# lab4d-org/lab4d

Hardware: AMD Instinct MI355X
Metric: rendered rays/sec (fwd+bwd) at 512² × 128 samples; PSNR vs ref (higher is better)
Workload: dtype bf16

## Files before the change

### include/lab4d_mlp.h

```cpp
#ifndef LAB4D_MLP_H
#define LAB4D_MLP_H

#include <stdint.h>

#define LAB4D_MLP_MAX_LAYERS 12

#define LAB4D_NET_FG_BASE 0
#define LAB4D_NET_FG_COLOR 1
#define LAB4D_NET_VIS 2
#define LAB4D_NET_FEAT 3
#define LAB4D_NET_SKIN 4
#define LAB4D_NET_DENSE 5
#define LAB4D_NET_BG_BASE 6
#define LAB4D_NET_BG_COLOR 7
#define LAB4D_NET_SKIN18 8
#define LAB4D_NET_HASH_GEO 9
#define LAB4D_NET_HASH_COLOR 10
#define LAB4D_NET_DENSE6 11
#define LAB4D_NET_SKIN_A 12
#define LAB4D_NET_SKIN18_A 13
#define LAB4D_NET_COUNT 14

#define LAB4D_PREC_F32 0
#define LAB4D_PREC_BF16 1

typedef struct {
  int ke;
  int kin;
  int mout;
  int mout_pad;
  int relu;
  int pf_bias;
  int add_ext;
  int ext_grad;
} lab4d_mlp_layer;

typedef struct {
  int n_layers;
  int emb_kind;
  int n_freq;
  int c_in;
  int emb_slots;
  int ke;
  int c_out;
  lab4d_mlp_layer layers[LAB4D_MLP_MAX_LAYERS];
} lab4d_mlp_desc;

int lab4d_mlp_describe(int net, lab4d_mlp_desc* out);

int64_t lab4d_mlp_packed_bytes(int net, int layer, int precision);

int lab4d_mlp_pack(int net, int layer, int precision, int transposed, const float* W_ref, int k_ref,
                   const int32_t* col_map, void* packed, void* stream);

typedef struct {
  int net, precision;
  int S;
  int S_pad;
  int ld;
  int spf;
  const float* x;
  const float* freq_w;
  const void* W[LAB4D_MLP_MAX_LAYERS];
  const float* bias[LAB4D_MLP_MAX_LAYERS];
  const float* pf_bias[LAB4D_MLP_MAX_LAYERS];
  void* act[LAB4D_MLP_MAX_LAYERS];
  void* mask[LAB4D_MLP_MAX_LAYERS];
  void* emb;
  const void* ext;
  float* out;
  const float* x2;
  const int32_t* S_dev;
  const int32_t* frame_idx;
  const float* aff;
} lab4d_mlp_fwd_args;
int lab4d_mlp_forward(const lab4d_mlp_fwd_args* a, void* stream);

typedef struct {
  int net, precision, S, spf;
  const float* x;
  const float* freq_w;
  const float* aff;
  const void* W[LAB4D_MLP_MAX_LAYERS];
  const void* WT[LAB4D_MLP_MAX_LAYERS];
  const float* bias[LAB4D_MLP_MAX_LAYERS];
  const float* pf_bias[LAB4D_MLP_MAX_LAYERS];
  const float* d_out;
  float* d_x;
  float* g_aff;
  float* dW[LAB4D_MLP_MAX_LAYERS];
  float* db[LAB4D_MLP_MAX_LAYERS];
  float* pf_db[LAB4D_MLP_MAX_LAYERS];
} lab4d_mlp_bwd_fused_args;
int lab4d_mlp_backward_fused(const lab4d_mlp_bwd_fused_args* a, void* stream);
int lab4d_mlp_fused_backward_supported(int net, int precision, int spf);

int lab4d_mlp_forward_tangent(const lab4d_mlp_fwd_args* a, void* stream);

typedef struct {
  int net, precision, S, S_pad, ld, spf;
  const void* WT[LAB4D_MLP_MAX_LAYERS];
  const void* act[LAB4D_MLP_MAX_LAYERS];
  const void* mask[LAB4D_MLP_MAX_LAYERS];
  const void* emb;
  const void* ext;
  const float* d_out;
  const void* ext_gin;
  void* ext_gout;
  void* dz[LAB4D_MLP_MAX_LAYERS];
  float* d_x;
  float* d_x2;
  const float* x;
  const float* aff;
  float* g_aff;
} lab4d_mlp_bwd_args;
int lab4d_mlp_backward(const lab4d_mlp_bwd_args* a, void* stream);

int lab4d_mlp_wgrad(int net, int layer, int precision, int S, int S_pad, int ld, int spf, const void* dz, const void* emb,
                    const void* act_prev, float* dW, float* db, float* pf_db, int M, void* stream);
int lab4d_mlp_wgrad_mapped(int net, int layer, int precision, int S, int S_pad, int ld, int spf, const void* dz, const void* emb,
                           const void* act_prev, float* dW_ref, int ld_ref, const int32_t* col_map, float* db, float* pf_db, int M,
                           void* stream);

#endif
```

### lab4d_amd/csrc/hd_math.hpp

```cpp
#pragma once
#include <math.h>
#include <stdint.h>

#if defined(__HIPCC__)
#define LAB4D_HD __host__ __device__ inline
#else
#define LAB4D_HD inline
#endif

namespace lab4d_rn {

#if defined(__HIP_DEVICE_COMPILE__)
template <typename T>
__device__ __forceinline__ void pin(T& v) { asm volatile("" : "+v"(v)); }
__device__ __forceinline__ float add_rn(float a, float b) { float p = a + b; asm volatile("" : "+v"(p)); return p; }
__device__ __forceinline__ float mul_rn(float a, float b) { float p = a * b; asm volatile("" : "+v"(p)); return p; }
__device__ __forceinline__ float div_rn(float a, float b) { return __fdiv_rn(a, b); }
__device__ __forceinline__ double dadd(double a, double b) { double p = a + b; asm volatile("" : "+v"(p)); return p; }
__device__ __forceinline__ double dmul(double a, double b) { double p = a * b; asm volatile("" : "+v"(p)); return p; }
#else
template <typename T>
LAB4D_HD void pin(T&) {}
LAB4D_HD float add_rn(float a, float b) { volatile float p = a + b; return p; }
LAB4D_HD float mul_rn(float a, float b) { volatile float p = a * b; return p; }
LAB4D_HD float div_rn(float a, float b) { volatile float p = a / b; return p; }
LAB4D_HD double dadd(double a, double b) { volatile double p = a + b; return p; }
LAB4D_HD double dmul(double a, double b) { volatile double p = a * b; return p; }
#endif

LAB4D_HD float sqrt_rn(float a) { return (float)sqrt((double)a); }
LAB4D_HD bool finite_f(float v) { return fabsf(v) <= 3.402823466e+38f; }
LAB4D_HD float inf_f() { return __builtin_huge_valf(); }
LAB4D_HD float nan_f() { return __builtin_nanf(""); }

}
```

### lab4d_amd/csrc/mlp.hip

```cpp
#include <cstdlib>
#include "mlp_kernels.hpp"
#include "mlp_fused_bwd.hpp"

namespace lab4d {

struct DwMap {
  const int* cmap;
  int ld, mout, db_rows;
};
__device__ __forceinline__ int dw_col(int k, const DwMap& wm) { return wm.cmap ? wm.cmap[k] : k; }
__device__ __forceinline__ void dw_add(float* dW, int o, int c, int K, const DwMap& wm, float v) {
  if (wm.cmap) {
    if (c >= 0 && o < wm.mout) atomicAdd(dW + (size_t)o * wm.ld + c, v);
  } else {
    atomicAdd(dW + (size_t)o * K + c, v);
  }
}

template <class P, int TM>
__global__ void __launch_bounds__(256) k_mlp_wgrad(const typename P::store_t* __restrict__ dz, const typename P::store_t* __restrict__ emb,
                                                    const typename P::store_t* __restrict__ actp, int mo_tiles, int ke, int kin,
                                                    int S_pad, int chunk, int spf, int cpf, float* __restrict__ dW, float* __restrict__ db, DwMap wm) {
  constexpr int TN = 4;
  constexpr int SPS = P::BF16 ? 16 : 8;
// ... 395 lines not shown
        });
      }
      __builtin_amdgcn_s_barrier();
      asm volatile("" ::: "memory");
      if (s + NSTAGE - 1 < N) issue(s + NSTAGE - 1, buf == 0 ? NSTAGE - 1 : buf - 1);
      compute(buf);
      buf = buf + 1 == NSTAGE ? 0 : buf + 1;
    }
  }
#pragma unroll
  for (int i = 0; i < TM; ++i) {
#pragma unroll
    for (int j = 0; j < TN; ++j) {
      if (!bv_[j]) continue;
      const int c = dw_col(k0 + 32 * (wc * TN + j) + row, wm);
#pragma unroll
      for (int r = 0; r < 16; ++r) {
        const int o = 32 * (wr * TM + i) + drow(r, h);
        dw_add(dW, o, c, K, wm, acc[i][j][r]);
      }
    }
    if (do_db) {
      const float v = rs[i] + __shfl_xor(rs[i], 32, 64);
      if (h == 0 && 32 * (wr * TM + i) + row < wm.db_rows) atomicAdd(db + 32 * (wr * TM + i) + row, v);
    }
  }
}

template <class P>
__global__ void __launch_bounds__(256) k_rowsum_pf(const typename P::store_t* __restrict__ dz, int mo_pad, int S, int ld, int spf,
                                                    int M, int nseg, float* __restrict__ pf_db) {
  constexpr int SEG = 4096;
  const int lane = threadIdx.x & 63;
  const long job = (long)blockIdx.x * 4 + (threadIdx.x >> 6);
  if (job >= (long)mo_pad * nseg) return;
  const int o = (int)(job / nseg), seg = (int)(job % nseg);
  const long b = (long)seg * SEG, e = min((long)S, b + SEG);
  const typename P::store_t* row = dz + (size_t)o * 64;
  long i = b;
  while (i < e) {
    const int m = (int)(i / spf);
    const long fe = min(e, (long)(m + 1) * spf);
    float s = 0.f;
    for (long k = i + lane; k < fe; k += 64) {
      const size_t idx = (size_t)(k >> 6) * block_stride(mo_pad) + (k & 63);
      if constexpr (P::BF16) s += bf2f(row[idx]);
      else s += row[idx];
    }
    s = wave_sum(s);
    if (lane == 0) atomicAdd(pf_db + (size_t)m * mo_pad + o, s);
    i = fe;
  }
}

template <class P>
__global__ void __launch_bounds__(256) k_pack(const float* __restrict__ Wref, int mout, int k_ref, const int32_t* __restrict__ col_map,
                                               int ke, int kin, int mo_pad, int transposed, typename P::store_t* __restrict__ out) {
  constexpr int EPL = P::BF16 ? 8 : 4;
  const int K = ke + kin;
  const int rows = transposed ? K : mo_pad;
  const int kdim = transposed ? mo_pad : K;
  const int G = kdim / P::FPG;
  const long total = (long)(rows / 32) * G * 64 * EPL;
  for (long e = (long)blockIdx.x * blockDim.x + threadIdx.x; e < total; e += (long)gridDim.x * blockDim.x) {
    const int j = (int)(e % EPL);
    const int lane = (int)((e / EPL) % 64);
    const int g = (int)((e / (EPL * 64)) % G);
    const int mt = (int)(e / ((long)EPL * 64 * G));
    const int row = 32 * mt + (lane & 31), h = lane >> 5;
    const int ge = transposed ? 0 : ke / P::FPG;
    int kk;
    if (g < ge) {
      kk = P::BF16 ? 16 * g + 8 * h + j : 2 * (4 * g + j) + h;
    } else {
      const int gg = g - ge;
      int b, r;
      if (P::BF16) { b = gg >> 1; r = 8 * (gg & 1) + j; }
      else { const int kap = 4 * gg + j; b = kap >> 4; r = kap & 15; }
      kk = (transposed ? 0 : ke) + 32 * b + drow(r, h);
    }
    const int o = transposed ? kk : row;
    const int c = transposed ? row : kk;
    float v = 0.f;
    if (o < mout && c < K) {
      const int cr = col_map[c];
      if (cr >= 0) v = Wref[(size_t)o * k_ref + cr];
    }
    if constexpr (P::BF16) out[e] = f2bf(v);
    else out[e] = v;
  }
}

}
using namespace lab4d;

namespace {

template <class F>
int with_net(int net, F&& f) {
  switch (net) {
    case LAB4D_NET_FG_BASE: return f(NetFgBase{});
    case LAB4D_NET_FG_COLOR: return f(NetFgColor{});
    case LAB4D_NET_VIS: return f(NetVis{});
    case LAB4D_NET_FEAT: return f(NetFeat{});
    case LAB4D_NET_SKIN: return f(NetSkin{});
    case LAB4D_NET_SKIN18: return f(NetSkin18{});
    case LAB4D_NET_SKIN_A: return f(NetSkinA{});
    case LAB4D_NET_SKIN18_A: return f(NetSkin18A{});
    case LAB4D_NET_DENSE: return f(NetDense{});
    case LAB4D_NET_DENSE6: return f(NetDense6{});
    case LAB4D_NET_BG_BASE: return f(NetBgBase{});
    case LAB4D_NET_BG_COLOR: return f(NetBgColor{});
    case LAB4D_NET_HASH_GEO: return f(NetHashGeo{});
    case LAB4D_NET_HASH_COLOR: return f(NetHashColor{});
    default: set_error("unknown net id %d", net); return LAB4D_EINVAL;
  }
}

}

extern "C" int lab4d_mlp_describe(int net, lab4d_mlp_desc* out) {
  LAB4D_REQUIRE(out, "mlp_describe: null out");
  memset(out, 0, sizeof(*out));
  return with_net(net, [&](auto n) { fill_desc<decltype(n)>(out); return LAB4D_OK; });
}

extern "C" int64_t lab4d_mlp_packed_bytes(int net, int layer, int precision) {
  lab4d_mlp_desc d;
  if (lab4d_mlp_describe(net, &d) != LAB4D_OK || layer < 0 || layer >= d.n_layers) return -1;
  const lab4d_mlp_layer& L = d.layers[layer];
  return (int64_t)L.mout_pad * (L.ke + L.kin) * (precision == LAB4D_PREC_BF16 ? 2 : 4);
}

extern "C" int lab4d_mlp_pack(int net, int layer, int precision, int transposed, const float* W_ref, int k_ref,
                              const int32_t* col_map, void* packed, void* stream) {
  lab4d_mlp_desc d;
  if (int e = lab4d_mlp_describe(net, &d)) return e;
  LAB4D_REQUIRE(layer >= 0 && layer < d.n_layers, "mlp_pack: bad layer %d", layer);
  LAB4D_REQUIRE(W_ref && col_map && packed, "mlp_pack: null pointer");
  const lab4d_mlp_layer& L = d.layers[layer];
  const long total = (long)L.mout_pad * (L.ke + L.kin);
  int grid = div_up(total, 256); if (grid > 2048) grid = 2048;
  if (precision == LAB4D_PREC_BF16)
    hipLaunchKernelGGL((k_pack<PBF16>), dim3(grid), dim3(256), 0, (hipStream_t)stream, W_ref, L.mout, k_ref, col_map, L.ke, L.kin,
                       L.mout_pad, transposed, (unsigned short*)packed);
  else if (precision == LAB4D_PREC_F32)
    hipLaunchKernelGGL((k_pack<PF32>), dim3(grid), dim3(256), 0, (hipStream_t)stream, W_ref, L.mout, k_ref, col_map, L.ke, L.kin,
                       L.mout_pad, transposed, (float*)packed);
  else { set_error("mlp_pack: bad precision %d", precision); return LAB4D_EINVAL; }
  return check_launch("mlp_pack");
}

extern "C" int lab4d_mlp_forward(const lab4d_mlp_fwd_args* a, void* stream) {
  LAB4D_REQUIRE(a, "mlp_forward: null args");
  LAB4D_REQUIRE(a->S >= 0 && a->S_pad >= a->S && a->S_pad % 256 == 0 && a->spf > 0 && a->ld >= a->S_pad && a->ld % 8 == 0,
                "mlp_forward: bad sizes (S_pad must be a multiple of 256) S=%d S_pad=%d ld=%d spf=%d", a->S, a->S_pad, a->ld, a->spf);
  LAB4D_REQUIRE(a->x && a->out, "mlp_forward: null x/out");
  if (a->S == 0) return LAB4D_OK;
  return with_net(a->net, [&](auto n) {
    using Net = decltype(n);
    FwdK k;
    memset(&k, 0, sizeof(k));
    k.S = a->S; k.S_pad = a->S_pad; k.ld = a->ld; k.spf = a->spf; k.x = a->x; k.freq_w = a->freq_w; k.emb = a->emb; k.ext = a->ext; k.out = a->out; k.x2 = a->x2;
    k.S_dev = a->S_dev; k.frame_idx = a->frame_idx; k.aff = a->aff;
    LAB4D_REQUIRE(!a->aff || Net::EMB != 0, "mlp_forward: aff is for the raw-input nets only");
    LAB4D_REQUIRE(Net::EMB != 2 || a->aff, "mlp_forward: this network needs the per-frame affine table aff (M, ke, 4)");
    LAB4D_REQUIRE(!Net::AUX3 || a->x2, "mlp_forward: this network needs the second input x2");
    LAB4D_REQUIRE(!(a->S_dev && a->emb), "mlp_forward: a device-side sample count is for the evaluation path (no stored activations)");
    for (int l = 0; l < Net::NL; ++l) {
      LAB4D_REQUIRE(a->W[l] && a->bias[l], "mlp_forward: layer %d weights/bias missing", l);
      LAB4D_REQUIRE(!Net::L[l].pf || a->pf_bias[l], "mlp_forward: layer %d needs a per-frame bias", l);
      LAB4D_REQUIRE(!Net::L[l].add_ext || a->ext, "mlp_forward: layer %d needs ext", l);
      if (a->emb && l + 1 < Net::NL) {
        LAB4D_REQUIRE(a->act[l] || (dx_only_ok<Net>() && !a->act[0]), "mlp_forward: training mode (emb != NULL) needs act[%d]", l);
        LAB4D_REQUIRE(!Net::L[l].relu || a->mask[l], "mlp_forward: training mode (emb != NULL) needs mask[%d]", l);
      }
      k.W[l] = a->W[l]; k.bias[l] = a->bias[l]; k.pf_bias[l] = a->pf_bias[l]; k.act[l] = a->act[l]; k.mask[l] = (unsigned int*)a->mask[l];
    }
    return launch_mlp_fwd<Net>(a->precision, k, a->S, (hipStream_t)stream);
  });
}

extern "C" int lab4d_mlp_backward(const lab4d_mlp_bwd_args* a, void* stream) {
  LAB4D_REQUIRE(a, "mlp_backward: null args");
  LAB4D_REQUIRE(a->S >= 0 && a->S_pad >= a->S && a->S_pad % 256 == 0 && a->spf > 0 && a->ld >= a->S_pad && a->ld % 8 == 0, "mlp_backward: bad sizes (S_pad must be a multiple of 256)");
  LAB4D_REQUIRE(a->d_out, "mlp_backward: null d_out");
  if (a->S == 0) return LAB4D_OK;
  return with_net(a->net, [&](auto n) {
    using Net = decltype(n);
    BwdK k;
    memset(&k, 0, sizeof(k));
    k.S = a->S; k.S_pad = a->S_pad; k.ld = a->ld; k.spf = a->spf; k.emb = a->emb; k.ext = a->ext; k.d_out = a->d_out; k.ext_gin = a->ext_gin;
    k.ext_gout = a->ext_gout; k.d_x = a->d_x; k.d_x2 = a->d_x2; k.x = a->x; k.aff = a->aff; k.g_aff = a->g_aff;
    if (Net::EMB == 2) {
      LAB4D_REQUIRE(a->x && a->aff && a->emb, "mlp_backward: this network needs x, aff and the stored embedding");
    } else {
      LAB4D_REQUIRE(!a->g_aff, "mlp_backward: g_aff is for the affine-first-layer nets only");
    }
    LAB4D_REQUIRE(!(a->d_x && Net::EMB == 0) || a->emb, "mlp_backward: d_x needs the stored embedding");
    for (int l = 0; l < Net::NL; ++l) {
      LAB4D_REQUIRE(a->WT[l], "mlp_backward: layer %d transposed weights missing", l);
      LAB4D_REQUIRE(!(Net::L[l].relu && l + 1 < Net::NL) || a->mask[l], "mlp_backward: layer %d ReLU mask missing", l);
      LAB4D_REQUIRE(!Net::L[l].ext_grad || a->ext_gin, "mlp_backward: layer %d needs ext_gin", l);
      LAB4D_REQUIRE(a->dz[l] || (dx_only_ok<Net>() && !a->dz[0] && a->d_x), "mlp_backward: dz[%d] missing (every layer's dZ is written, or none: point gradient only)", l);
      LAB4D_REQUIRE(!Net::L[l].add_ext || a->ext_gout, "mlp_backward: layer %d needs ext_gout", l);
      k.WT[l] = a->WT[l]; k.act[l] = a->act[l]; k.mask[l] = (const unsigned int*)a->mask[l]; k.dz[l] = a->dz[l];
    }
    return launch_mlp_bwd<Net>(a->precision, k, a->S, (hipStream_t)stream);
  });
}

extern "C" int lab4d_mlp_fused_backward_supported(int net, int precision, int spf) {
  if (precision != LAB4D_PREC_BF16 || spf <= 0 || spf % 64 != 0) return 0;
  static const int vis_env = getenv("LAB4D_FUSED_VIS") ? atoi(getenv("LAB4D_FUSED_VIS")) : 0;
  return net == LAB4D_NET_SKIN_A || net == LAB4D_NET_SKIN18_A || (net == LAB4D_NET_VIS && vis_env != 0);
}

extern "C" int lab4d_mlp_backward_fused(const lab4d_mlp_bwd_fused_args* a, void* stream) {
  LAB4D_REQUIRE(a, "mlp_backward_fused: null args");
  LAB4D_REQUIRE(lab4d_mlp_fused_backward_supported(a->net, a->precision, a->spf), "mlp_backward_fused: net %d / precision %d / spf %d not supported (bf16, narrow nets, spf %% 64 == 0)",
                a->net, a->precision, a->spf);
  LAB4D_REQUIRE(a->S >= 0 && a->x && a->d_out, "mlp_backward_fused: null x / d_out");
  if (a->S == 0) return LAB4D_OK;
  auto run = [&](auto n) {
    using Net = decltype(n);
    FusedK k;
    memset(&k, 0, sizeof(k));
    k.S = a->S; k.spf = a->spf; k.ntiles = (a->S + 63) / 64; k.x = a->x; k.freq_w = a->freq_w; k.aff = a->aff; k.d_out = a->d_out; k.d_x = a->d_x; k.g_aff = a->g_aff;
    LAB4D_REQUIRE(Net::EMB != 2 || a->aff, "mlp_backward_fused: this network needs the per-frame affine table aff");
    for (int l = 0; l < Net::NL; ++l) {
      LAB4D_REQUIRE(a->WT[l] && a->dW[l], "mlp_backward_fused: layer %d transposed weights / dW missing", l);
      LAB4D_REQUIRE(l + 1 == Net::NL || (a->W[l] && (Net::L[l].pf ? (const void*)a->pf_bias[l] : (const void*)a->bias[l])), "mlp_backward_fused: layer %d forward weights / bias missing", l);
      LAB4D_REQUIRE((((uintptr_t)a->W[l] | (uintptr_t)a->WT[l]) & 15) == 0, "mlp_backward_fused: packed weights must be 16-byte aligned");
      k.W[l] = a->W[l]; k.WT[l] = a->WT[l]; k.bias[l] = a->bias[l]; k.pf_bias[l] = a->pf_bias[l]; k.dW[l] = a->dW[l]; k.db[l] = a->db[l]; k.pf_db[l] = a->pf_db[l];
    }
    return launch_mlp_bwd_fused<Net>(k, (hipStream_t)stream);
  };
  switch (a->net) {
    case LAB4D_NET_VIS: return run(NetVis{});
    case LAB4D_NET_SKIN_A: return run(NetSkinA{});
    default: return run(NetSkin18A{});
  }
}

extern "C" int lab4d_mlp_wgrad(int net, int layer, int precision, int S, int S_pad, int ld, int spf, const void* dz, const void* emb,
                               const void* act_prev, float* dW, float* db, float* pf_db, int M, void* stream) {
  return lab4d_mlp_wgrad_mapped(net, layer, precision, S, S_pad, ld, spf, dz, emb, act_prev, dW, 0, nullptr, db, pf_db, M, stream);
}

extern "C" int lab4d_mlp_wgrad_mapped(int net, int layer, int precision, int S, int S_pad, int ld, int spf, const void* dz, const void* emb,
                                      const void* act_prev, float* dW, int ld_ref, const int32_t* col_map, float* db, float* pf_db, int M,
                                      void* stream) {
  lab4d_mlp_desc d;
  if (int e = lab4d_mlp_describe(net, &d)) return e;
  LAB4D_REQUIRE(layer >= 0 && layer < d.n_layers, "mlp_wgrad: bad layer %d", layer);
  const lab4d_mlp_layer& L = d.layers[layer];
  LAB4D_REQUIRE(dz && dW, "mlp_wgrad: null dz/dW");
  LAB4D_REQUIRE(col_map == nullptr || ld_ref > 0, "mlp_wgrad_mapped: a column map needs the reference row stride");
  LAB4D_REQUIRE(L.ke == 0 || emb, "mlp_wgrad: layer %d needs the stored embedding", layer);
  LAB4D_REQUIRE(L.kin == 0 || act_prev, "mlp_wgrad: layer %d needs the previous activation", layer);
  LAB4D_REQUIRE(S_pad % 64 == 0 && S_pad >= S && ld >= S_pad && ld % 8 == 0, "mlp_wgrad: bad S_pad/ld");
  if (S == 0) return LAB4D_OK;
  const int mo_tiles = L.mout_pad / 32, nk_tiles = (L.ke + L.kin) / 32;
  const bool big = mo_tiles >= 8;
  const int Kt = L.ke + L.kin;
  static const int head_dma = getenv("LAB4D_WGRAD_HEAD_DMA") ? atoi(getenv("LAB4D_WGRAD_HEAD_DMA")) : 1;
  const bool dma = precision == LAB4D_PREC_BF16 && (mo_tiles == 8 || mo_tiles == 4 || mo_tiles == 2 || (mo_tiles == 1 && head_dma && Kt <= 256));
  const int nbw = (dma && mo_tiles == 1) ? (Kt <= 128 ? 2 : 4)
                  : Kt <= 64 ? 1 : (Kt <= 128 ? 2 : (Kt <= 192 ? 3 : (Kt <= 256 ? 4 : (mo_tiles == 8 && Kt <= 320 ? 5 : 3))));
  const int TM = mo_tiles >= 4 ? 4 : (mo_tiles >= 2 ? 2 : 1);
  const int ob_n = dma ? 1 : (big ? div_up(mo_tiles, 8) : div_up(mo_tiles, TM));
  const int kb_n = dma ? div_up(Kt, 64 * nbw) : (big ? div_up(nk_tiles, 8) : div_up(nk_tiles, 4));
  static const int jobs_env = getenv("LAB4D_WGRAD_JOBS") ? atoi(getenv("LAB4D_WGRAD_JOBS")) : 0;
  const int jobs_target = jobs_env > 0 ? jobs_env : ((dma && mo_tiles < 8) ? 512 : 256);
  int nchunks = jobs_target / (ob_n * kb_n); if (nchunks < 1) nchunks = 1;
  int chunk = div_up(div_up(S_pad, nchunks), 256) * 256; if (chunk < 1024) chunk = 1024;
  const bool fold_pf = pf_db != nullptr && spf % 256 == 0 && M > 0 && (long)M * spf >= S;
  LAB4D_REQUIRE(pf_db == nullptr || fold_pf || (M > 0 && spf > 0 && (long)M * spf >= S), "mlp_wgrad: pf_db needs M and spf, with M * spf >= S");
  int cpf = 0;
  if (fold_pf) {
    if (chunk > spf) chunk = spf;
    cpf = div_up(spf, chunk);
    nchunks = cpf * M;
  } else {
    nchunks = div_up(S_pad, chunk);
  }
  const int jobs = ob_n * kb_n * nchunks;
  const dim3 grid(jobs), block(256), block8(512);
  float* db_arg = fold_pf ? pf_db : db;
  const DwMap wm = {col_map, ld_ref, L.mout, (col_map && !fold_pf) ? L.mout : L.mout_pad};
  hipStream_t st = (hipStream_t)stream;
#define WG(P, TMV) hipLaunchKernelGGL((k_mlp_wgrad<P, TMV>), grid, block, 0, st, (const typename P::store_t*)dz, (const typename P::store_t*)emb, \
                                      (const typename P::store_t*)act_prev, mo_tiles, L.ke, L.kin, S_pad, chunk, spf, cpf, dW, db_arg, wm)
#define WGB(P) hipLaunchKernelGGL((k_mlp_wgrad_big<P>), grid, block, 0, st, (const typename P::store_t*)dz, (const typename P::store_t*)emb, \
                                  (const typename P::store_t*)act_prev, mo_tiles, L.ke, L.kin, S_pad, chunk, spf, cpf, dW, db_arg, wm)
#define WGD(MTV, NBV) hipLaunchKernelGGL((k_mlp_wgrad_dma<MTV, NBV>), grid, block, 0, st, (const unsigned short*)dz, (const unsigned short*)emb, \
                                         (const unsigned short*)act_prev, L.ke, L.kin, S_pad, chunk, spf, cpf, dW, db_arg, wm)
#define WGD8(NBV) hipLaunchKernelGGL((k_mlp_wgrad_dma<8, NBV, 8>), grid, block8, 0, st, (const unsigned short*)dz, (const unsigned short*)emb, \
                                     (const unsigned short*)act_prev, L.ke, L.kin, S_pad, chunk, spf, cpf, dW, db_arg, wm)
#define WGD_NB(MTV) do { if (nbw == 1) WGD(MTV, 1); else if (nbw == 2) WGD(MTV, 2); else if (nbw == 3) WGD(MTV, 3); else WGD(MTV, 4); } while (0)
  if (dma) {
    if (mo_tiles == 8) {
      if (nbw == 1) WGD8(1); else if (nbw == 2) WGD8(2); else if (nbw == 3) WGD8(3); else if (nbw == 4) WGD8(4); else WGD8(5);
    } else if (mo_tiles == 4) WGD_NB(4); else if (mo_tiles == 2) WGD_NB(2);
    else if (nbw == 2) hipLaunchKernelGGL((k_mlp_wgrad_dma<1, 2, 4, 4>), grid, block, 0, st, (const unsigned short*)dz, (const unsigned short*)emb,
                                          (const unsigned short*)act_prev, L.ke, L.kin, S_pad, chunk, spf, cpf, dW, db_arg, wm);
    else hipLaunchKernelGGL((k_mlp_wgrad_dma<1, 4, 4, 4>), grid, block, 0, st, (const unsigned short*)dz, (const unsigned short*)emb,
                            (const unsigned short*)act_prev, L.ke, L.kin, S_pad, chunk, spf, cpf, dW, db_arg, wm);
  }
#undef WGD_NB
#undef WGD8
#undef WGD
  else if (precision == LAB4D_PREC_BF16) { if (big) WGB(PBF16); else if (TM == 4) WG(PBF16, 4); else if (TM == 2) WG(PBF16, 2); else WG(PBF16, 1); }
  else if (precision == LAB4D_PREC_F32) { if (big) WGB(PF32); else if (TM == 4) WG(PF32, 4); else if (TM == 2) WG(PF32, 2); else WG(PF32, 1); }
  else { set_error("mlp_wgrad: bad precision %d", precision); return LAB4D_EINVAL; }
#undef WGB
#undef WG
  if (int e = check_launch("mlp_wgrad")) return e;
  if (pf_db && !fold_pf) {
    const int nseg = div_up(S, 4096);
    const long jobs2 = (long)L.mout_pad * nseg;
    if (precision == LAB4D_PREC_BF16)
      hipLaunchKernelGGL((k_rowsum_pf<PBF16>), dim3(div_up(jobs2, 4)), dim3(256), 0, st, (const unsigned short*)dz, L.mout_pad, S, ld, spf, M, nseg, pf_db);
    else
      hipLaunchKernelGGL((k_rowsum_pf<PF32>), dim3(div_up(jobs2, 4)), dim3(256), 0, st, (const float*)dz, L.mout_pad, S, ld, spf, M, nseg, pf_db);
    return check_launch("mlp_rowsum_pf");
  }
  return LAB4D_OK;
}

namespace {
template <class Net>
int forward_tangent_impl(const lab4d_mlp_fwd_args* a, void* stream) {
  FwdK k;
  memset(&k, 0, sizeof(k));
  k.S = a->S; k.S_pad = a->S_pad; k.ld = a->ld; k.spf = a->spf; k.x = a->x; k.emb = a->emb; k.out = a->out;
  for (int l = 0; l < Net::NL; ++l) {
    LAB4D_REQUIRE(a->W[l], "mlp_forward_tangent: layer %d weights missing", l);
    LAB4D_REQUIRE(!(Net::L[l].relu) || a->mask[l], "mlp_forward_tangent: layer %d primal ReLU mask missing", l);
    LAB4D_REQUIRE(l + 1 == Net::NL || a->act[l], "mlp_forward_tangent: act[%d] missing", l);
    k.W[l] = a->W[l]; k.bias[l] = a->bias[l] ? a->bias[l] : (const float*)a->W[l]; k.act[l] = a->act[l]; k.mask[l] = (unsigned int*)a->mask[l];
  }
  return launch_mlp_fwd_tangent<Net>(a->precision, k, a->S, (hipStream_t)stream);
}
}

// ... 11 lines not shown
```

### lab4d_amd/csrc/mlp_kernels.hpp

```cpp
#pragma once
#include <cstddef>
#include <cstdlib>
#include <type_traits>

#include "common.hpp"
#include "mlp_nets.hpp"

namespace lab4d {

typedef __attribute__((ext_vector_type(8))) short bf16x8_t;
typedef __attribute__((ext_vector_type(16))) float f32x16_t;

struct PBF16 {
  static constexpr bool BF16 = true;
  static constexpr int NT = 2, TILE = 64, FPG = 16, UPT = 2;
  using store_t = unsigned short;
};
struct PF32 {
  static constexpr bool BF16 = false;
  static constexpr int NT = 1, TILE = 32, FPG = 8, UPT = 4;
  using store_t = float;
};

__device__ __forceinline__ unsigned short f2bf(float x) {
// ... 169 lines not shown
               "v_cndmask_b32_dpp %[t02], %[d21], %[d20], vcc" LAB4D_QP1 "v_cndmask_b32_dpp %[t22], %[d23], %[d22], vcc" LAB4D_QP1
               "v_cndmask_b32_dpp %[t03], %[d31], %[d30], vcc" LAB4D_QP1 "v_cndmask_b32_dpp %[t23], %[d33], %[d32], vcc quad_perm:[1,0,3,2] row_mask:0xf bank_mask:0xf"
               : [t00] "=&v"(t0[0]), [t01] "=&v"(t0[1]), [t02] "=&v"(t0[2]), [t03] "=&v"(t0[3]), [t20] "=&v"(t2[0]), [t21] "=&v"(t2[1]),
                 [t22] "=&v"(t2[2]), [t23] "=&v"(t2[3])
               : [m] "s"(mE), [d00] "v"(d[0][0]), [d01] "v"(d[0][1]), [d02] "v"(d[0][2]), [d03] "v"(d[0][3]), [d10] "v"(d[1][0]), [d11] "v"(d[1][1]),
                 [d12] "v"(d[1][2]), [d13] "v"(d[1][3]), [d20] "v"(d[2][0]), [d21] "v"(d[2][1]), [d22] "v"(d[2][2]), [d23] "v"(d[2][3]),
                 [d30] "v"(d[3][0]), [d31] "v"(d[3][1]), [d32] "v"(d[3][2]), [d33] "v"(d[3][3])
               : "vcc");
  asm volatile("s_mov_b64 vcc, %[m]\n\t"
               "v_cndmask_b32_dpp %[d01], %[d00], %[d01], vcc" LAB4D_QP1 "v_cndmask_b32_dpp %[d03], %[d02], %[d03], vcc" LAB4D_QP1
               "v_cndmask_b32_dpp %[d11], %[d10], %[d11], vcc" LAB4D_QP1 "v_cndmask_b32_dpp %[d13], %[d12], %[d13], vcc" LAB4D_QP1
               "v_cndmask_b32_dpp %[d21], %[d20], %[d21], vcc" LAB4D_QP1 "v_cndmask_b32_dpp %[d23], %[d22], %[d23], vcc" LAB4D_QP1
               "v_cndmask_b32_dpp %[d31], %[d30], %[d31], vcc" LAB4D_QP1 "v_cndmask_b32_dpp %[d33], %[d32], %[d33], vcc quad_perm:[1,0,3,2] row_mask:0xf bank_mask:0xf"
               : [d01] "+v"(d[0][1]), [d03] "+v"(d[0][3]), [d11] "+v"(d[1][1]), [d13] "+v"(d[1][3]), [d21] "+v"(d[2][1]), [d23] "+v"(d[2][3]),
                 [d31] "+v"(d[3][1]), [d33] "+v"(d[3][3])
               : [m] "s"(mO), [d00] "v"(d[0][0]), [d02] "v"(d[0][2]), [d10] "v"(d[1][0]), [d12] "v"(d[1][2]), [d20] "v"(d[2][0]), [d22] "v"(d[2][2]),
                 [d30] "v"(d[3][0]), [d32] "v"(d[3][2])
               : "vcc");
  unsigned int c0[4], c1[4];
  asm volatile("s_mov_b64 vcc, %[m]\n\t"
               "v_cndmask_b32_dpp %[c00], %[t20], %[t00], vcc" LAB4D_QP2 "v_cndmask_b32_dpp %[c10], %[d03], %[d01], vcc" LAB4D_QP2
               "v_cndmask_b32_dpp %[c01], %[t21], %[t01], vcc" LAB4D_QP2 "v_cndmask_b32_dpp %[c11], %[d13], %[d11], vcc" LAB4D_QP2
               "v_cndmask_b32_dpp %[c02], %[t22], %[t02], vcc" LAB4D_QP2 "v_cndmask_b32_dpp %[c12], %[d23], %[d21], vcc" LAB4D_QP2
               "v_cndmask_b32_dpp %[c03], %[t23], %[t03], vcc" LAB4D_QP2 "v_cndmask_b32_dpp %[c13], %[d33], %[d31], vcc quad_perm:[2,3,0,1] row_mask:0xf bank_mask:0xf"
               : [c00] "=&v"(c0[0]), [c01] "=&v"(c0[1]), [c02] "=&v"(c0[2]), [c03] "=&v"(c0[3]), [c10] "=&v"(c1[0]), [c11] "=&v"(c1[1]),
                 [c12] "=&v"(c1[2]), [c13] "=&v"(c1[3])
               : [m] "s"(mL), [t00] "v"(t0[0]), [t01] "v"(t0[1]), [t02] "v"(t0[2]), [t03] "v"(t0[3]), [t20] "v"(t2[0]), [t21] "v"(t2[1]), [t22] "v"(t2[2]),
                 [t23] "v"(t2[3]), [d01] "v"(d[0][1]), [d03] "v"(d[0][3]), [d11] "v"(d[1][1]), [d13] "v"(d[1][3]), [d21] "v"(d[2][1]), [d23] "v"(d[2][3]),
                 [d31] "v"(d[3][1]), [d33] "v"(d[3][3])
               : "vcc");
  asm volatile("s_mov_b64 vcc, %[m]\n\t"
               "v_cndmask_b32_dpp %[t20], %[t00], %[t20], vcc" LAB4D_QP2 "v_cndmask_b32_dpp %[d03], %[d01], %[d03], vcc" LAB4D_QP2
               "v_cndmask_b32_dpp %[t21], %[t01], %[t21], vcc" LAB4D_QP2 "v_cndmask_b32_dpp %[d13], %[d11], %[d13], vcc" LAB4D_QP2
               "v_cndmask_b32_dpp %[t22], %[t02], %[t22], vcc" LAB4D_QP2 "v_cndmask_b32_dpp %[d23], %[d21], %[d23], vcc" LAB4D_QP2
               "v_cndmask_b32_dpp %[t23], %[t03], %[t23], vcc" LAB4D_QP2 "v_cndmask_b32_dpp %[d33], %[d31], %[d33], vcc quad_perm:[2,3,0,1] row_mask:0xf bank_mask:0xf"
               : [t20] "+v"(t2[0]), [t21] "+v"(t2[1]), [t22] "+v"(t2[2]), [t23] "+v"(t2[3]), [d03] "+v"(d[0][3]), [d13] "+v"(d[1][3]), [d23] "+v"(d[2][3]),
                 [d33] "+v"(d[3][3])
               : [m] "s"(mH), [t00] "v"(t0[0]), [t01] "v"(t0[1]), [t02] "v"(t0[2]), [t03] "v"(t0[3]), [d01] "v"(d[0][1]), [d11] "v"(d[1][1]), [d21] "v"(d[2][1]),
                 [d31] "v"(d[3][1])
               : "vcc");
#undef LAB4D_QP1
#undef LAB4D_QP2
#pragma unroll
  for (int i = 0; i < 4; ++i) {
    out[i][0] = c0[i];
    out[i][1] = c1[i];
    out[i][2] = t2[i];
    out[i][3] = d[i][3];
  }
}

__device__ __forceinline__ void store_tile_packed(GLOBAL_AS void* buf, int F, int s0, int mt, int lane, const unsigned int (&w)[2][8]) {
  const int n = lane & 31, h = lane >> 5, q = n & 3, k = n >> 2;
  GLOBAL_AS char* base = (GLOBAL_AS char*)buf + tile_base_offset<PBF16>(F, s0, 32 * mt);
  const unsigned lo = tile_lane_offset<PBF16>(4 * h + q, k);
  unsigned int d[4][4], c[4][4];
#pragma unroll
  for (int i = 0; i < 4; ++i)
#pragma unroll
    for (int j = 0; j < 4; ++j) {
      const int r = 4 * i + j;
      d[i][j] = __builtin_amdgcn_perm(w[1][r >> 1], w[0][r >> 1], (r & 1) ? 0x07060302u : 0x05040100u);
    }
  quad_transpose4(d, c);
#pragma unroll
  for (int i = 0; i < 4; ++i) gst16(base + (lo + tile_lane_offset<PBF16>(8 * i, 0)), c[i][0], c[i][1], c[i][2], c[i][3]);
}


struct TrTile {
  unsigned long long a[4], b[4];
};
__device__ __forceinline__ void tr_wait(TrTile& r) {
  asm volatile("s_waitcnt lgkmcnt(0)"
               : "+v"(r.a[0]), "+v"(r.a[1]), "+v"(r.a[2]), "+v"(r.a[3]), "+v"(r.b[0]), "+v"(r.b[1]), "+v"(r.b[2]), "+v"(r.b[3]));
}
__device__ __forceinline__ void tr_store(GLOBAL_AS void* buf, int F, int s0, int mt, int lane, const TrTile& r) {
  const int i = lane & 15, G = lane >> 4, h = G & 1, S = G >> 1;
  GLOBAL_AS char* base = (GLOBAL_AS char*)buf + tile_base_offset<PBF16>(F, s0, 32 * mt);
  const unsigned lo = (unsigned)((4 * h + (i & 3)) * 128 + (32 * S + 8 * (i >> 2)) * 2);
#pragma unroll
  for (int qa = 0; qa < 4; ++qa) {
    const unsigned long long A = r.a[qa], B = r.b[qa];
    gst16(base + (lo + (unsigned)((16 * (qa >> 1) + 8 * (qa & 1)) * 128)), (unsigned)A, (unsigned)(A >> 32), (unsigned)B, (unsigned)(B >> 32));
  }
}

template <class P>
__device__ __forceinline__ void store_tile(GLOBAL_AS void* buf, int F, int s0, int mt, int lane, const f32x16_t* c ) {
  const int n = lane & 31, h = lane >> 5, q = n & 3, k = n >> 2;
  GLOBAL_AS char* base = (GLOBAL_AS char*)buf + tile_base_offset<P>(F, s0, 32 * mt);
  const unsigned lo = tile_lane_offset<P>(4 * h + q, k);
#pragma unroll
  for (int i = 0; i < 4; ++i) {
    unsigned int d[4];
#pragma unroll
    for (int j = 0; j < 4; ++j) {
      if constexpr (P::BF16) d[j] = pack2bf(c[0][4 * i + j], c[1][4 * i + j]);
      else d[j] = __float_as_uint(c[0][4 * i + j]);
    }
    quad_transpose(d, q);
    gst16(base + (lo + tile_lane_offset<P>(8 * i, 0)), d[0], d[1], d[2], d[3]);
  }
}
template <class P>
__device__ __forceinline__ void load_tile_raw(const GLOBAL_AS void* buf, int F, int s0, int mt, int lane, uint4 (&raw)[4]) {
  const int n = lane & 31, h = lane >> 5, q = n & 3, k = n >> 2;
  const GLOBAL_AS char* base = (const GLOBAL_AS char*)buf + tile_base_offset<P>(F, s0, 32 * mt);
  const unsigned lo = tile_lane_offset<P>(4 * h + q, k);
#pragma unroll
  for (int i = 0; i < 4; ++i) raw[i] = gld16(base + (lo + tile_lane_offset<P>(8 * i, 0)));
}
template <class P>
__device__ __forceinline__ void tile_from_raw(const uint4 (&raw)[4], int lane, f32x16_t* c ) {
  const int q = lane & 3;
#pragma unroll
  for (int i = 0; i < 4; ++i) {
    unsigned int d[4] = {raw[i].x, raw[i].y, raw[i].z, raw[i].w};
    quad_transpose(d, q);
#pragma unroll
    for (int j = 0; j < 4; ++j) {
      if constexpr (P::BF16) {
        c[0][4 * i + j] = bf2f((unsigned short)(d[j] & 0xffffu));
        c[1][4 * i + j] = bf2f((unsigned short)(d[j] >> 16));
      } else {
        c[0][4 * i + j] = __uint_as_float(d[j]);
      }
    }
  }
}
template <class P>
__device__ __forceinline__ void load_tile(const GLOBAL_AS void* buf, int F, int s0, int mt, int lane, f32x16_t* c ) {
  uint4 raw[4];
  load_tile_raw<P>(buf, F, s0, mt, lane, raw);
  tile_from_raw<P>(raw, lane, c);
}

struct FwdK {
  int S, S_pad, ld, spf, ntiles;
  const float* x;
  const float* freq_w;
  const void* W[LAB4D_MLP_MAX_LAYERS];
  const float* bias[LAB4D_MLP_MAX_LAYERS];
  const float* pf_bias[LAB4D_MLP_MAX_LAYERS];
  void* act[LAB4D_MLP_MAX_LAYERS];
  unsigned int* mask[LAB4D_MLP_MAX_LAYERS];
  void* emb;
  const void* ext;
  float* out;
  const float* x2;
  const int* S_dev;
  const int* frame_idx;
  const float* aff;
};
struct BwdK {
  int S, S_pad, ld, spf, ntiles;
  const void* WT[LAB4D_MLP_MAX_LAYERS];
  const void* act[LAB4D_MLP_MAX_LAYERS];
  const unsigned int* mask[LAB4D_MLP_MAX_LAYERS];
  const void* emb;
  const void* ext;
  const float* d_out;
  const void* ext_gin;
  void* ext_gout;
  void* dz[LAB4D_MLP_MAX_LAYERS];
  float* d_x;
  float* d_x2;
  const float* x;
  const float* aff;
  float* g_aff;
};

template <class Net>
__device__ __forceinline__ void emb_pair(int pair, const float* x , const float* freq_w, float& v0, float& v1) {
  constexpr int L = Net::NFREQ;
  if (pair < 3 * L) {
    const int f = pair / 3, a = pair - 3 * f;
    const float xa = a == 0 ? x[0] : (a == 1 ? x[1] : x[2]);
    const float ang = ldexpf(xa, f);
    float s, c;
    sincosf(ang, &s, &c);
    const float w = freq_w ? freq_w[f] : 1.0f;
    v0 = s * w;
    v1 = c * w;
  } else {
    const int s0 = 2 * pair - 6 * L;
    constexpr int NR = Net::AUX3 ? 6 : 3;
    v0 = s0 < NR ? x[s0 < NR ? s0 : 0] : 0.f;
    v1 = s0 + 1 < NR ? x[s0 + 1 < NR ? s0 + 1 : 0] : 0.f;
  }
}

constexpr int ACACHE_G = 14;
template <class Net, class P, bool BWD = false>
constexpr int want_occ() {
  return (P::BF16 && (Net::ID == LAB4D_NET_FEAT || Net::ID == LAB4D_NET_VIS)) ? 2 : 1;
}
template <class Net, class P>
constexpr int acache_g() {
  return want_occ<Net, P>() == 2 ? 7 : ACACHE_G;
}
__device__ __forceinline__ void wg_step_barrier() {
  asm volatile("s_waitcnt lgkmcnt(0)\n\ts_barrier" ::: "memory");
}

template <class Net>
constexpr bool fwd_same(int a, int b) {
  const LS x = Net::L[a], y = Net::L[b];
  return x.ke == y.ke && x.kin == y.kin && x.mout == y.mout && x.relu == y.relu && x.pf == y.pf && x.add_ext == y.add_ext &&
         ((a == Net::NL - 1) == (b == Net::NL - 1));
}
template <class Net>
constexpr int fwd_rep(int l) {
  for (int j = 0; j < l; ++j)
    if (fwd_same<Net>(j, l)) return j;
  return l;
}
template <class Net>
constexpr unsigned fwd_members(int r) {
  unsigned m = 0;
  for (int l = 0; l < Net::NL; ++l)
    if (fwd_rep<Net>(l) == r) m |= 1u << l;
  return m;
}
template <class Net>
constexpr bool fwd_any_export(int r) {
  for (int l = 0; l < Net::NL; ++l)
    if (fwd_rep<Net>(l) == r && Net::L[l].ext_grad) return true;
  return false;
}
template <class Net>
constexpr bool bwd_same(int a, int b) {
  if ((a == 0) != (b == 0)) return false;
  const LS x = Net::L[a], y = Net::L[b];
  if (!(x.ke == y.ke && x.kin == y.kin && x.mout == y.mout)) return false;
  if (a == 0) return true;
  const LS xp = Net::L[a - 1], yp = Net::L[b - 1];
  return xp.relu == yp.relu && xp.ext_grad == yp.ext_grad && xp.add_ext == yp.add_ext && xp.mout == yp.mout;
}
template <class Net>
constexpr int bwd_rep(int l) {
  for (int j = Net::NL - 1; j > l; --j)
    if (bwd_same<Net>(j, l)) return j;
  return l;
}
template <class Net>
constexpr unsigned bwd_members(int r) {
  unsigned m = 0;
  for (int l = 0; l < Net::NL; ++l)
    if (bwd_rep<Net>(l) == r) m |= 1u << l;
  return m;
}

template <class Net>
constexpr bool head_staged() { return Net::COUT > 16; }

template <class Net, class P>
struct Slab {
  static constexpr int W = net_wmax<Net>();
  static constexpr int UW = W / P::FPG;
  static constexpr int STAGE_C = Net::EMB == 1 ? Net::CIN : Net::KE;
  static constexpr bool STAGES = Net::EMB == 1 || Net::ID == LAB4D_NET_FG_BASE || Net::ID == LAB4D_NET_BG_BASE;
  static constexpr int UNITS_STAGE = STAGES ? (P::TILE * STAGE_C * 4 + 15) / 16 : 0;
  static constexpr int UNITS_LAYER = P::NT * UW * 64;
  static constexpr int UNITS_PER_WAVE = UNITS_LAYER > UNITS_STAGE ? UNITS_LAYER : UNITS_STAGE;
};

template <int COUNT>
__device__ __forceinline__ void stage_in(float* __restrict__ stage, const float* __restrict__ x, long e0, long e_last, int lane) {
  const GLOBAL_AS float* gx = (const GLOBAL_AS float*)x;
  if (e0 + COUNT - 1 <= e_last && (((size_t)(x + e0)) & 15) == 0 && (COUNT & 3) == 0) {
    constexpr int N4 = COUNT / 4, TRIPS = (N4 + 63) / 64;
    f32x4_t v[TRIPS];
#pragma unroll
    for (int i = 0; i < TRIPS; ++i) {
      const int e = lane + 64 * i;
      if (e < N4) v[i] = *(const GLOBAL_AS f32x4_t*)(gx + e0 + 4 * e);
    }
#pragma unroll
    for (int i = 0; i < TRIPS; ++i) {
      const int e = lane + 64 * i;
      if (e < N4) reinterpret_cast<float4*>(stage)[e] = make_float4(v[i].x, v[i].y, v[i].z, v[i].w);
    }
  } else {
    for (int e = lane; e < COUNT; e += 64) {
      const long ge = e0 + e;
      stage[e] = gx[ge <= e_last ? ge : e_last];
    }
  }
}
__device__ __forceinline__ void stage_out(const float* __restrict__ stage, float* __restrict__ y, long e0, int count, long e_last, int lane) {
  GLOBAL_AS float* gy = (GLOBAL_AS float*)y;
  if (e0 + count - 1 <= e_last && (((size_t)(y + e0)) & 15) == 0 && (count & 3) == 0) {
    for (int e = lane; e < count / 4; e += 64) {
      const float4 v = reinterpret_cast<const float4*>(stage)[e];
      f32x4_t o = {v.x, v.y, v.z, v.w};
      *(GLOBAL_AS f32x4_t*)(gy + e0 + 4 * e) = o;
    }
  } else {
    for (int e = lane; e < count; e += 64) {
      const long ge = e0 + e;
      if (ge <= e_last) gy[ge] = stage[e];
    }
  }
}

template <class Net, class P, bool TAN = false, bool ST = false, bool ACTS = true>
__global__ void __launch_bounds__(256, (want_occ<Net, P>())) k_mlp_fwd(FwdK a) {
  constexpr int NT = P::NT, TILE = P::TILE, KE = Net::KE, UE = KE / P::FPG, UW = Slab<Net, P>::UW;
  constexpr int ACG = acache_g<Net, P>();
  __shared__ uint4 slab_all[4 * Slab<Net, P>::UNITS_PER_WAVE];
  __shared__ uint4 abuf[2 * ACG * 64];
  __shared__ float4 afftab[(Net::EMB != 0 && !TAN) ? 4 * 96 : 1];
  const int lane = threadIdx.x & 63, n = lane & 31, h = lane >> 5;
  const int wid = __builtin_amdgcn_readfirstlane((int)(threadIdx.x >> 6));
  uint4* slab = slab_all + wid * Slab<Net, P>::UNITS_PER_WAVE + lane;
  const int wave = blockIdx.x * 4 + wid, nwaves = gridDim.x * 4;

  int S_eff = a.S, ntiles = a.ntiles;
  if (a.S_dev) {
    const int sd = *(const GLOBAL_AS int*)a.S_dev;
    S_eff = sd < a.S ? sd : a.S;
    const int nt = ((S_eff + TILE - 1) / TILE + 3) & ~3;
    ntiles = nt < a.ntiles ? nt : a.ntiles;
  }
  for (int tile = wave; tile < ntiles; tile += nwaves) {
    const int s0 = tile * TILE;
    int sidx[NT], frame[NT];
#pragma unroll
    for (int t = 0; t < NT; ++t) {
      const int s = s0 + NT * n + t;
      sidx[t] = s;
      const int sc = s < S_eff ? s : S_eff - 1;
      frame[t] = a.frame_idx ? ((const GLOBAL_AS int*)a.frame_idx)[sc] : sc / a.spf;
    }
    uint4 emb[NT][UE];
    constexpr bool RAW = (Net::EMB == 1) || TAN;
    constexpr int CINR = TAN ? KE : Net::CIN;
    float* stagef = reinterpret_cast<float*>(slab_all + wid * Slab<Net, P>::UNITS_PER_WAVE);
    if constexpr (RAW) {
      bool staged = false;
      if constexpr (Net::EMB == 1 && !TAN) {
        if (a.aff != nullptr) {
          static_assert(Net::CIN <= 96, "affine table");
          constexpr int HALF = (Net::CIN + 1) / 2;
          const GLOBAL_AS float4* tabg = (const GLOBAL_AS float4*)a.aff;
          float4* ltab = afftab + wid * 96;
          const bool uni = (a.spf % TILE) == 0 && a.frame_idx == nullptr;
          if (uni) {
            const int m = __builtin_amdgcn_readfirstlane(frame[0]);
            for (int e = lane; e < Net::CIN; e += 64) {
              const f32x4_t r = *(const GLOBAL_AS f32x4_t*)(tabg + (size_t)m * Net::CIN + e);
              ltab[e] = make_float4(r.x, r.y, r.z, r.w);
            }
          }
          __builtin_amdgcn_wave_barrier();
#pragma unroll
          for (int t = 0; t < NT; ++t) {
            const int s = sidx[t] < S_eff ? sidx[t] : S_eff - 1;
            const float x0 = a.x[(size_t)s * 3], x1 = a.x[(size_t)s * 3 + 1], x2_ = a.x[(size_t)s * 3 + 2];
            float* row = stagef + (NT * n + t) * Net::CIN;
            for (int i = 0; i < HALF; ++i) {
              const int c = i + h * HALF;
              if (c < Net::CIN) {
                float4 r;
                if (uni) r = ltab[c];
                else {
                  const f32x4_t g = *(const GLOBAL_AS f32x4_t*)(tabg + (size_t)frame[t] * Net::CIN + c);
                  r = make_float4(g.x, g.y, g.z, g.w);
                }
                row[c] = r.x * x0 + r.y * x1 + r.z * x2_ + r.w;
              }
            }
          }
          __builtin_amdgcn_wave_barrier();
          staged = true;
        }
      }
      if (!staged) stage_in<TILE * CINR>(stagef, a.x, (long)s0 * CINR, (long)S_eff * CINR - 1, lane);
    }
    if constexpr (Net::EMB == 2 && !TAN) {
      static_assert(KE <= 96, "affine table");
      const GLOBAL_AS float4* tabg = (const GLOBAL_AS float4*)a.aff;
      float4* ltab = afftab + wid * 96;
      const bool uni = (a.spf % TILE) == 0 && a.frame_idx == nullptr;
      if (uni) {
        const int m = __builtin_amdgcn_readfirstlane(frame[0]);
        for (int e = lane; e < KE; e += 64) {
          const f32x4_t r = *(const GLOBAL_AS f32x4_t*)(tabg + (size_t)m * KE + e);
          ltab[e] = make_float4(r.x, r.y, r.z, r.w);
        }
      }
      __builtin_amdgcn_wave_barrier();
#pragma unroll
      for (int t = 0; t < NT; ++t) {
        const int s = sidx[t] < S_eff ? sidx[t] : S_eff - 1;
        const float x0 = a.x[(size_t)s * 3], x1 = a.x[(size_t)s * 3 + 1], x2_ = a.x[(size_t)s * 3 + 2];
        auto slot_val = [&](int slot) {
          float4 r;
          if (uni) r = ltab[slot];
          else {
            const f32x4_t g4 = *(const GLOBAL_AS f32x4_t*)(tabg + (size_t)frame[t] * KE + slot);
            r = make_float4(g4.x, g4.y, g4.z, g4.w);
          }
          return relu1(r.x * x0 + r.y * x1 + r.z * x2_ + r.w);
        };
#pragma unroll
        for (int g = 0; g < UE; ++g) {
// ... 128 lines not shown
      if constexpr (fwd_rep<Net>(R) != R) return;
      constexpr unsigned MEMBERS = fwd_members<Net>(R);
      if (!((MEMBERS >> l) & 1u)) return;
      constexpr LS ls = Net::L[R];
      constexpr bool LAST = (R == Net::NL - 1);
      constexpr int MT = pad32(ls.mout) / 32;
      constexpr int GE = ls.ke / P::FPG, GA = ls.kin / P::FPG, G = GE + GA;
      constexpr int GL = G < ACG ? G : ACG, NQ = (GL + 3) / 4;
      const GLOBAL_AS void* Wl = KARG_PTR(FwdK, const void*, W, l);
      const GLOBAL_AS float* bl = KARG_PTR(FwdK, const float*, bias, l);
      const GLOBAL_AS float* pfl = KARG_PTR(FwdK, const float*, pf_bias, l);
      GLOBAL_AS unsigned int* maskl = KARG_PTR(FwdK, unsigned int*, mask, l);
      GLOBAL_AS void* actl = KARG_PTR(FwdK, void*, act, l);
      uint4 bin[NT][GA > 0 ? GA : 1];
#pragma unroll
      for (int t = 0; t < NT; ++t)
#pragma unroll
        for (int u = 0; u < GA; ++u) bin[t][u] = slab[(t * UW + u) * 64];
      constexpr int NB = (ls.pf != 0 && !TAN) ? NT : 1;
      auto load_bias = [&](int mt, f32x16_t (&bv)[NB]) {
        if constexpr (TAN) {
#pragma unroll
          for (int r = 0; r < 16; ++r) bv[0][r] = 0.f;
        } else {
#pragma unroll
          for (int t = 0; t < NB; ++t)
#pragma unroll
            for (int i = 0; i < 4; ++i) {
              const GLOBAL_AS float* src = (ls.pf != 0) ? pfl + (size_t)frame[t] * (32 * MT) : bl;
              const f32x4_t v = *(const GLOBAL_AS f32x4_t*)(src + 32 * mt + 8 * i + 4 * h);
              bv[t][4 * i + 0] = v.x; bv[t][4 * i + 1] = v.y; bv[t][4 * i + 2] = v.z; bv[t][4 * i + 3] = v.w;
            }
        }
      };
      auto mfma_tile = [&](auto has_pre, int pre, int rbuf, uint4 (&A)[G], f32x16_t (&bv)[NB], f32x16_t (&acc)[NT]) {
        constexpr bool PRE = decltype(has_pre)::value;
#pragma unroll
        for (int t = 0; t < NT; ++t) acc[t] = bv[NB == 1 ? 0 : t];
#pragma unroll
        for (int g = 0; g < G; ++g) {
#pragma unroll
          for (int t = 0; t < NT; ++t) mma_unit<P>(acc[t], A[g], g < GE ? emb[t][g < GE ? g : 0] : bin[t][g >= GE ? g - GE : 0]);
          if constexpr (PRE) {
            if (g >= GL) A[g] = load_a(Wl, G, pre, g, lane);
            else if (rbuf >= 0) A[g] = abuf[(rbuf * ACG + g) * 64 + lane];
          }
        }
        if constexpr (PRE) load_bias(pre, bv);
      };
      auto a_fetch = [&](int mt, uint4 (&stg)[NQ]) {
#pragma unroll
        for (int i = 0; i < NQ; ++i) {
          const int g = wid + 4 * i < GL ? wid + 4 * i : GL - 1;
          stg[i] = load_a(Wl, G, mt, g, lane);
        }
      };
      auto a_stash = [&](int buf, const uint4 (&stg)[NQ]) {
#pragma unroll
        for (int i = 0; i < NQ; ++i) {
          const int g = wid + 4 * i < GL ? wid + 4 * i : GL - 1;
          abuf[(buf * ACG + g) * 64 + lane] = stg[i];
        }
      };
      auto a_grab = [&](int buf, uint4 (&A)[G]) {
#pragma unroll
        for (int g = 0; g < GL; ++g) A[g] = abuf[(buf * ACG + g) * 64 + lane];
      };
      unsigned int tan_bits = 0;
      uint4 ext_raw[4];
      auto prefetch = [&](int mt) {
        if constexpr (TAN && ls.relu != 0) tan_bits = maskl[((size_t)tile * MT + mt) * 64 + lane];
        if constexpr (ls.add_ext != 0 && !TAN) load_tile_raw<P>((const GLOBAL_AS void*)a.ext, 32 * MT, s0, mt, lane, ext_raw);
      };
      constexpr bool PACKED = P::BF16 && !TAN && ls.add_ext == 0 && !LAST;
      auto epilogue = [&](int mt, f32x16_t (&acc)[NT], unsigned int (&w)[2][8], unsigned int& wbits) {
        if constexpr (PACKED) {
#pragma unroll
          for (int t = 0; t < NT; ++t) acc_fence_if<(want_occ<Net, P>() == 2)>(acc[t]);
#pragma unroll
          for (int t = 0; t < 2; ++t)
#pragma unroll
            for (int k = 0; k < 8; ++k) w[t][k] = pack2bf_op(acc[t][2 * k], acc[t][2 * k + 1]);
          if constexpr (ls.relu != 0) {
            if constexpr (ST) wbits = pk_alive_bits(w);
#pragma unroll
            for (int t = 0; t < 2; ++t)
#pragma unroll
              for (int k = 0; k < 8; ++k) w[t][k] = pk_relu_bf16(w[t][k]);
          }
#pragma unroll
          for (int t = 0; t < 2; ++t)
#pragma unroll
            for (int q = 0; q < 2; ++q) slab[(t * UW + 2 * mt + q) * 64] = make_uint4(w[t][4 * q], w[t][4 * q + 1], w[t][4 * q + 2], w[t][4 * q + 3]);
          return;
        }
        if constexpr (ls.relu != 0) {
          if constexpr (TAN) {
            const unsigned int bits = tan_bits;
#pragma unroll
            for (int t = 0; t < NT; ++t)
#pragma unroll
              for (int r = 0; r < 16; ++r)
                acc[t][r] = __uint_as_float(__float_as_uint(acc[t][r]) & (unsigned int)__builtin_amdgcn_sbfe((int)bits, mask_bit<P>(t, r), 1));
          } else {
            if constexpr (ST && !LAST) {
              unsigned int bits = 0;
#pragma unroll
              for (int t = 0; t < NT; ++t)
#pragma unroll
                for (int r = 0; r < 16; ++r) bits |= (acc[t][r] > 0.f ? 1u : 0u) << mask_bit<P>(t, r);
              maskl[((size_t)tile * MT + mt) * 64 + lane] = bits;
            }
#pragma unroll
            for (int t = 0; t < NT; ++t)
#pragma unroll
              for (int r = 0; r < 16; ++r) acc[t][r] = relu1(acc[t][r]);
          }
        }
        if constexpr (ls.add_ext != 0 && !TAN) {
          f32x16_t e[NT];
          tile_from_raw<P>(ext_raw, lane, e);
#pragma unroll
          for (int t = 0; t < NT; ++t)
#pragma unroll
            for (int r = 0; r < 16; ++r) acc[t][r] += e[t][r];
        }
        if constexpr (ST) {
          if constexpr (!LAST && ACTS) store_tile<P>(actl, 32 * MT, s0, mt, lane, acc);
        } else if constexpr (fwd_any_export<Net>(R)) {
          if (actl) store_tile<P>(actl, 32 * MT, s0, mt, lane, acc);
        }
        if constexpr (!LAST) {
#pragma unroll
          for (int t = 0; t < NT; ++t) {
            uint4 u[P::UPT];
            tile_to_units<P>(acc[t], u);
#pragma unroll
            for (int q = 0; q < P::UPT; ++q) slab[(t * UW + P::UPT * mt + q) * 64] = u[q];
          }
        } else if constexpr (head_staged<Net>() && !TAN) {
          static_assert(pad32(Net::COUT) == 32, "one row tile");
          __builtin_amdgcn_wave_barrier();
#pragma unroll
          for (int t = 0; t < NT; ++t)
#pragma unroll
            for (int r = 0; r < 16; ++r) {
              const int f = drow(r, h);
              if (f < Net::COUT) stagef[(NT * n + t) * Net::COUT + f] = acc[t][r];
            }
          __builtin_amdgcn_wave_barrier();
          if (a.out) stage_out(stagef, a.out, (long)s0 * Net::COUT, TILE * Net::COUT, (long)S_eff * Net::COUT - 1, lane);
          __builtin_amdgcn_wave_barrier();
        } else {
#pragma unroll
          for (int t = 0; t < NT; ++t)
#pragma unroll
            for (int r = 0; r < 16; ++r) {
              const int f = 32 * mt + drow(r, h);
              if (f < Net::COUT && sidx[t] < S_eff && a.out) a.out[(size_t)sidx[t] * Net::COUT + f] = acc[t][r];
            }
        }
      };
      auto flush = [&](int mt, const unsigned int (&w)[2][8], unsigned int wbits) {
        if constexpr (PACKED) {
          if constexpr (ST) {
            if constexpr (ls.relu != 0) maskl[((size_t)tile * MT + mt) * 64 + lane] = wbits;
            if constexpr (ACTS) store_tile_packed(actl, 32 * MT, s0, mt, lane, w);
          } else if constexpr (fwd_any_export<Net>(R)) {
            if (actl) store_tile_packed(actl, 32 * MT, s0, mt, lane, w);
          }
        }
      };
      uint4 A[G], stg[NQ];
      f32x16_t bv[NB];
      f32x16_t acc0[NT], acc1[NT];
      unsigned int pw[2][8], pbits = 0;
      wg_step_barrier();
      a_fetch(0, stg);
      a_stash(0, stg);
      if constexpr (MT > 1) {
        a_fetch(1, stg);
        a_stash(1, stg);
      }
      a_fetch(MT > 2 ? 2 : MT - 1, stg);
#pragma unroll
      for (int g = GL; g < G; ++g) A[g] = load_a(Wl, G, 0, g, lane);
      load_bias(0, bv);
      prefetch(0);
      wg_step_barrier();
      a_grab(0, A);
      constexpr int NSTEP = MT - 1, NPAIR = NSTEP / 2;
      mfma_tile(std::bool_constant<(MT > 1)>{}, 1, -1, A, bv, acc0);
      if constexpr (NPAIR > 0) {
#pragma nounroll
        for (int k = 0; k < 2 * NPAIR; k += 2) {
          wg_step_barrier();
          a_grab(1, A);
          mfma_tile(std::true_type{}, k + 2 < MT ? k + 2 : MT - 1, -1, A, bv, acc1);
          epilogue(k, acc0, pw, pbits);
          prefetch(k + 1);
          a_stash(0, stg);
          a_fetch(k + 3 < MT ? k + 3 : MT - 1, stg);
          flush(k, pw, pbits);
          wg_step_barrier();
          a_grab(0, A);
          mfma_tile(std::true_type{}, k + 3 < MT ? k + 3 : MT - 1, -1, A, bv, acc0);
          epilogue(k + 1, acc1, pw, pbits);
          prefetch(k + 2 < MT ? k + 2 : MT - 1);
          a_stash(1, stg);
          a_fetch(k + 4 < MT ? k + 4 : MT - 1, stg);
          flush(k + 1, pw, pbits);
        }
      }
      if constexpr (NSTEP % 2 == 1) {
        wg_step_barrier();
        a_grab(1, A);
        mfma_tile(std::false_type{}, 0, -1, A, bv, acc1);
        epilogue(MT - 2, acc0, pw, pbits);
        flush(MT - 2, pw, pbits);
        prefetch(MT - 1);
        epilogue(MT - 1, acc1, pw, pbits);
        flush(MT - 1, pw, pbits);
      } else {
        epilogue(MT - 1, acc0, pw, pbits);
        flush(MT - 1, pw, pbits);
      }
    });
  }
}

template <class Net>
constexpr int emb_layer_count() {
  int c = 0;
  for (int l = 0; l < Net::NL; ++l) c += Net::L[l].ke ? 1 : 0;
  return c;
}

template <class Net, class P, bool AU = true, bool DZ = true>
__global__ void __launch_bounds__(256, (want_occ<Net, P, true>())) k_mlp_bwd(BwdK a) {
  static_assert(Net::EMB == 0 || emb_layer_count<Net>() == 1, "raw-input nets may use the input in one layer only");
  constexpr int NT = P::NT, TILE = P::TILE, NL = Net::NL, UW = Slab<Net, P>::UW;
  constexpr int ACG = acache_g<Net, P>();
  __shared__ uint4 slab_all[4 * Slab<Net, P>::UNITS_PER_WAVE];
  __shared__ uint4 abuf0[ACG * 64];
  __shared__ uint4 abuf1[ACG * 64];
#define LAB4D_ABUF(buf) ((buf) ? abuf1 : abuf0)
  __shared__ float4 afftab[Net::EMB == 2 ? 4 * 96 : 1];
  constexpr int NGA = (Net::EMB == 2 && AU) ? (Net::KE / 32) * 16 * 4 : 1;
  float gacc[NGA];
#pragma unroll
  for (int i = 0; i < NGA; ++i) gacc[i] = 0.f;
  int gframe = -1;
  auto gram_flush = [&]() {
    if constexpr (Net::EMB == 2 && AU) {
      if (gframe >= 0 && a.g_aff != nullptr) {
#pragma unroll
        for (int i = 0; i < NGA; ++i) {
          float v = gacc[i];
#pragma unroll
          for (int off = 1; off < 32; off <<= 1) v += __shfl_xor(v, off, 64);
          const int mt = i / 64, r = (i >> 2) & 15, j = i & 3;
          if ((threadIdx.x & 31) == 0) atomicAdd(a.g_aff + ((size_t)gframe * Net::KE + 32 * mt + drow(r, (int)((threadIdx.x & 63) >> 5))) * 4 + j, v);
          gacc[i] = 0.f;
        }
      }
    }
  };
  const int lane = threadIdx.x & 63, n = lane & 31, h = lane >> 5;
  const int wid = __builtin_amdgcn_readfirstlane((int)(threadIdx.x >> 6));
  uint4* slab = slab_all + wid * Slab<Net, P>::UNITS_PER_WAVE + lane;
  float* stagef = reinterpret_cast<float*>(slab_all + wid * Slab<Net, P>::UNITS_PER_WAVE);
  const int wave = blockIdx.x * 4 + wid, nwaves = gridDim.x * 4;

  for (int tile = wave; tile < a.ntiles; tile += nwaves) {
    const int s0 = tile * TILE;
    int sidx[NT];
#pragma unroll
    for (int t = 0; t < NT; ++t) sidx[t] = s0 + NT * n + t;
    float dx[NT][3];
    float dx2[NT][3];
#pragma unroll
    for (int t = 0; t < NT; ++t) { dx[t][0] = dx[t][1] = dx[t][2] = 0.f; dx2[t][0] = dx2[t][1] = dx2[t][2] = 0.f; }
    float xs[NT][3];
    int frm[NT];
    float4* ltab = afftab + wid * 96;
    constexpr bool uni = AU;
    if constexpr (Net::EMB == 2) {
#pragma unroll
      for (int t = 0; t < NT; ++t) {
        const int sc = sidx[t] < a.S ? sidx[t] : a.S - 1;
        frm[t] = sc / a.spf;
#pragma unroll
        for (int k = 0; k < 3; ++k) xs[t][k] = ((const GLOBAL_AS float*)a.x)[(size_t)sc * 3 + k];
      }
      if constexpr (uni) {
        const int m = __builtin_amdgcn_readfirstlane(frm[0]);
        if (m != gframe) {
          gram_flush();
          gframe = m;
        }
        for (int e = lane; e < Net::KE; e += 64) {
          const f32x4_t r4 = *(const GLOBAL_AS f32x4_t*)((const GLOBAL_AS float4*)a.aff + (size_t)m * Net::KE + e);
          ltab[e] = make_float4(r4.x, r4.y, r4.z, r4.w);
        }
      }
      __builtin_amdgcn_wave_barrier();
    }

    {
      f32x16_t g[NT];
      if constexpr (head_staged<Net>()) {
        __builtin_amdgcn_wave_barrier();
        stage_in<TILE * Net::COUT>(stagef, a.d_out, (long)s0 * Net::COUT, (long)a.S * Net::COUT - 1, lane);
        __builtin_amdgcn_wave_barrier();
#pragma unroll
        for (int t = 0; t < NT; ++t)
#pragma unroll
          for (int r = 0; r < 16; ++r) {
            const int f = drow(r, h);
            g[t][r] = (f < Net::COUT && sidx[t] < a.S) ? stagef[(NT * n + t) * Net::COUT + (f < Net::COUT ? f : 0)] : 0.f;
          }
        __builtin_amdgcn_wave_barrier();
      } else {
#pragma unroll
      for (int t = 0; t < NT; ++t)
#pragma unroll
        for (int r = 0; r < 16; ++r) {
          const int f = drow(r, h);
          g[t][r] = (f < Net::COUT && sidx[t] < a.S) ? a.d_out[(size_t)sidx[t] * Net::COUT + f] : 0.f;
        }
      }
      if constexpr (DZ) store_tile<P>((GLOBAL_AS void*)a.dz[NL - 1], pad32(Net::L[NL - 1].mout), s0, 0, lane, g);
#pragma unroll
      for (int t = 0; t < NT; ++t) {
        uint4 u[P::UPT];
        tile_to_units<P>(g[t], u);
#pragma unroll
        for (int q = 0; q < P::UPT; ++q) slab[(t * UW + q) * 64] = u[q];
      }
    }

#pragma nounroll
    for (int l = NL - 1; l >= 0; --l)
    sfor<0, NL>([&](auto ri) {
      constexpr int R = NL - 1 - decltype(ri)::value;
      if constexpr (bwd_rep<Net>(R) != R) return;
      constexpr unsigned MEMBERS = bwd_members<Net>(R);
      if (!((MEMBERS >> l) & 1u)) return;
      constexpr LS ls = Net::L[R];
      constexpr LS lp = Net::L[R > 0 ? R - 1 : 0];
      constexpr int GK = pad32(ls.mout) / P::FPG;
      constexpr int GL = GK < ACG ? GK : ACG, NQ = (GL + 3) / 4;
      constexpr int MTE = ls.ke / 32, MTA = ls.kin / 32;
      constexpr bool DO_ACT = (R > 0 && MTA > 0);
      const int lm1 = l > 0 ? l - 1 : 0;
      const GLOBAL_AS void* Wt = KARG_PTR(BwdK, const void*, WT, l);
      const GLOBAL_AS unsigned int* maskp = KARG_PTR(BwdK, const unsigned int*, mask, lm1);
      GLOBAL_AS void* dzp = KARG_PTR(BwdK, void*, dz, lm1);
      uint4 bin[NT][GK];
#pragma unroll
      for (int t = 0; t < NT; ++t)
#pragma unroll
        for (int u = 0; u < GK; ++u) bin[t][u] = slab[(t * UW + u) * 64];

      auto mfma_tile = [&](auto has_pre, int pre, int rbuf, uint4 (&A)[GK], f32x16_t (&acc)[NT]) {
        constexpr bool PRE = decltype(has_pre)::value;
#pragma unroll
        for (int t = 0; t < NT; ++t)
#pragma unroll
          for (int r = 0; r < 16; ++r) acc[t][r] = 0.f;
        sfor<0, GK>([&](auto gc) {
          constexpr int g = decltype(gc)::value;
#pragma unroll
          for (int t = 0; t < NT; ++t) mma_unit<P>(acc[t], A[g], bin[t][g]);
          if constexpr (PRE) {
            if (g >= GL) A[g] = load_a(Wt, GK, pre, g, lane);
            else if (rbuf >= 0) A[g] = LAB4D_ABUF(rbuf)[g * 64 + lane];
          }
        });
      };
      auto a_fetch = [&](int mt, uint4 (&stg)[NQ]) {
#pragma unroll
        for (int i = 0; i < NQ; ++i) {
          const int g = wid + 4 * i < GL ? wid + 4 * i : GL - 1;
          stg[i] = load_a(Wt, GK, mt, g, lane);
        }
      };
      auto a_stash = [&](int buf, const uint4 (&stg)[NQ]) {
#pragma unroll
        for (int i = 0; i < NQ; ++i) {
          const int g = wid + 4 * i < GL ? wid + 4 * i : GL - 1;
          LAB4D_ABUF(buf)[g * 64 + lane] = stg[i];
        }
      };
      auto a_grab = [&](int buf, uint4 (&A)[GK]) {
#pragma unroll
        for (int g = 0; g < GL; ++g) A[g] = LAB4D_ABUF(buf)[g * 64 + lane];
      };
      auto pipeline = [&](auto n_c, int tile0, auto&& pre, auto&& epi, auto&& fl, auto&& prem) {
        constexpr int N = decltype(n_c)::value;
        if constexpr (N > 0) {
          uint4 A[GK], stg[NQ];
          f32x16_t acc0[NT], acc1[NT];
          unsigned int pw[2][8];
          wg_step_barrier();
          a_fetch(tile0, stg);
          a_stash(0, stg);
          if constexpr (N > 1) {
            a_fetch(tile0 + 1, stg);
            a_stash(1, stg);
          }
          a_fetch(tile0 + (N > 2 ? 2 : N - 1), stg);
#pragma unroll
          for (int g = GL; g < GK; ++g) A[g] = load_a(Wt, GK, tile0, g, lane);
          pre(0);
          prem(std::integral_constant<int, 0>{}, 0);
          prem(std::integral_constant<int, 1>{}, N > 1 ? 1 : 0);
          wg_step_barrier();
          a_grab(0, A);
          constexpr int NSTEP = N - 1, NPAIR = NSTEP / 2;
          mfma_tile(std::bool_constant<(N > 1)>{}, tile0 + 1, 1, A, acc0);
          if constexpr (N > 1) {
            wg_step_barrier();
            a_stash(0, stg);
            a_fetch(tile0 + (N > 3 ? 3 : N - 1), stg);
          }
          if constexpr (NPAIR > 0) {
#pragma nounroll
            for (int k = 0; k < 2 * NPAIR; k += 2) {
              wg_step_barrier();
              mfma_tile(std::true_type{}, tile0 + (k + 2 < N ? k + 2 : N - 1), 0, A, acc1);
              epi(k, acc0, pw);
              pre(k + 1);
              prem(std::integral_constant<int, 0>{}, k + 2 < N ? k + 2 : N - 1);
              a_stash(1, stg);
              a_fetch(tile0 + (k + 4 < N ? k + 4 : N - 1), stg);
              fl(k, pw);
              wg_step_barrier();
              mfma_tile(std::true_type{}, tile0 + (k + 3 < N ? k + 3 : N - 1), 1, A, acc0);
              epi(k + 1, acc1, pw);
              pre(k + 2 < N ? k + 2 : N - 1);
              prem(std::integral_constant<int, 1>{}, k + 3 < N ? k + 3 : N - 1);
              a_stash(0, stg);
              a_fetch(tile0 + (k + 5 < N ? k + 5 : N - 1), stg);
              fl(k + 1, pw);
            }
          }
          if constexpr (NSTEP % 2 == 1) {
            wg_step_barrier();
            mfma_tile(std::false_type{}, 0, -1, A, acc1);
            epi(N - 2, acc0, pw);
            fl(N - 2, pw);
            pre(N - 1);
            epi(N - 1, acc1, pw);
            fl(N - 1, pw);
          } else {
            epi(N - 1, acc0, pw);
            fl(N - 1, pw);
          }
        }
      };
      uint4 raw[4];
      unsigned int mb0 = 0, mb1 = 0;
      auto no_prem = [&](auto, int) {};
      auto pre_mask = [&](auto par_c, int j) {
        if constexpr (lp.relu != 0) {
          const unsigned int v = maskp[((size_t)tile * (pad32(lp.mout) / 32) + j) * 64 + lane];
          if constexpr (decltype(par_c)::value == 0) mb0 = v; else mb1 = v;
        }
      };
      auto pre_emb = [&](int mt) {
        if constexpr (Net::EMB != 1) load_tile_raw<P>((const GLOBAL_AS void*)a.emb, Net::KE, s0, mt, lane, raw);
      };
      auto pre_act = [&](int j) {
        if constexpr (lp.ext_grad != 0) load_tile_raw<P>((const GLOBAL_AS void*)a.ext_gin, pad32(lp.mout), s0, j, lane, raw);
      };
      auto no_flush = [&](int, const unsigned int (&)[2][8]) {};
      auto epi_emb = [&](int mt, f32x16_t (&acc)[NT], unsigned int (&)[2][8]) {
        if constexpr (Net::EMB == 0) {
          f32x16_t e[NT];
          tile_from_raw<P>(raw, lane, e);
          constexpr int L = Net::NFREQ;
#pragma unroll
// ... 297 lines not shown
```

### lab4d_amd/csrc/mlp_kernels_ws.hpp

```cpp
#pragma once
#include "mlp_kernels.hpp"

namespace lab4d {

template <class Net>
constexpr bool ws_ok() {
  if (!(Net::EMB == 0 && Net::AUX3 == 0 && net_wmax<Net>() == 256 && Net::KE % 32 == 0)) return false;
  for (int l = 0; l < Net::NL; ++l) {
    const int mt = pad32(Net::L[l].mout) / 32;
    if (!(mt == 1 || mt == 2 || mt == 4 || mt == 8)) return false;
    if (Net::L[l].kin % 32 != 0 || Net::L[l].kin > 256) return false;
    if (Net::L[l].ke != 0 && Net::L[l].ke != Net::KE) return false;
  }
  return true;
}
template <class Net>
constexpr int ws_g(int l) { return (Net::L[l].ke + Net::L[l].kin) / 16; }
template <class Net>
constexpr int ws_mt(int l) { return pad32(Net::L[l].mout) / 32; }
template <class Net>
constexpr int ws_gmax() {
  int g = 0;
  for (int l = 0; l < Net::NL; ++l) g = ws_g<Net>(l) > g ? ws_g<Net>(l) : g;
  return g;
// ... 396 lines not shown
      GLOBAL_AS void* actp = act_c;
      GLOBAL_AS unsigned int* maskp = mask_c;
      const GLOBAL_AS void* Wn_n = KARG_PTR(FwdK, const void*, W, (ln + 1 < NL ? ln + 1 : 0));
      GLOBAL_AS void* act_n = KARG_PTR(FwdK, void*, act, l);
      GLOBAL_AS unsigned int* mask_n = KARG_PTR(FwdK, unsigned int*, mask, l);
      const int mtp = ITp::mt(w);
      if constexpr (R > 0 && !SPREAD) {
        auto flush_prev = [&]() {
#pragma unroll
          for (int k = 0; k < ITp::IPW; ++k) {
            const int b = ITp::blk(w, k);
            if constexpr (ACTS) {
              {
                const unsigned tb_ = xbuf_lds + (unsigned)(ib * WS_BUF * 16 + b * 2 * 16 * 1024 + mtp * 2048);
                ws_tr_issue(tb_ + trl, tb_ + trl2, trt);
              }
              tr_wait(trt);
              tr_store(actp, 32 * MTp, s0 + 64 * b, mtp, lane, trt);
            }
            if constexpr (ST && !TAN && Net::L[R > 0 ? R - 1 : 0].relu != 0) maskp[((size_t)(2 * tile + b) * MTp + mtp) * 64 + lane] = pbits[k];
          }
        };
        if constexpr (ST) {
          if (ITp::active(w)) flush_prev();
        } else {
          if (actp != nullptr && ITp::active(w)) flush_prev();
        }
      }
      WsPiece tp;

      if (active) {
        sfor<0, IT::IPW>([&](auto kc) {
          constexpr int k = decltype(kc)::value;
          const int b = IT::blk(w, k);
          constexpr int KL = IT::IPW - 1;
          f32x16_t acc[2];
          constexpr int BD = G < WS_BD ? G : WS_BD;
          u32x4_t bq[BD][2];
          const unsigned pe_a = ebuf_lds + (unsigned)((2 * b * UE) * 1024 + lane * 16), px_a = xbuf_lds + (unsigned)(ib * WS_BUF * 16 + (2 * b * 16) * 1024 + lane_s * 16);
          auto b_read = [&](auto gc, u32x4_t (&dst)[2]) {
            constexpr int g = decltype(gc)::value;
            if constexpr (g < GE) {
              ws_lds_read<g * 1024>(dst[0], pe_a);
              ws_lds_read<(UE + g) * 1024>(dst[1], pe_a);
            } else {
              ws_lds_read<(g - GE) * 1024>(dst[0], px_a);
              ws_lds_read<(16 + g - GE) * 1024>(dst[1], px_a);
            }
          };
          sfor<0, BD>([&](auto gc) { b_read(gc, bq[decltype(gc)::value]); });
          if constexpr (k == 0) {
            if (bias_lds_path) {
              ws_lds_wait4<2 * BD>(br);
#pragma unroll
              for (int i = 0; i < 4; ++i) {
                bv[0][4 * i + 0] = __uint_as_float(br[i].x); bv[0][4 * i + 1] = __uint_as_float(br[i].y);
                bv[0][4 * i + 2] = __uint_as_float(br[i].z); bv[0][4 * i + 3] = __uint_as_float(br[i].w);
              }
              bv[1] = bv[0];
            }
          }
          acc[0] = bv[0];
          acc[1] = bv[1];
          sfor<0, G>([&](auto gc) {
            constexpr int g = decltype(gc)::value;
            constexpr int NEWER = 2 * ((G - 1 - g) < (BD - 1) ? (G - 1 - g) : (BD - 1));
            ws_lds_wait<NEWER>(bq[g % BD][0], bq[g % BD][1]);
            mma_b(acc[0], A[g], bq[g % BD][0]);
            mma_b(acc[1], A[g], bq[g % BD][1]);
            if constexpr (SPREAD && k < NHOST) {
              using SP = WsSpread<G, (NPI > 0 ? NPI : 1)>;
              sfor<0, (SPREAD ? NPI : 0)>([&](auto ic) {
                constexpr int i = decltype(ic)::value, pi = k * NPI + i, kp = pi / 4, qa = pi % 4;
                if constexpr (SP::issue_at(i) == g) {
                  const unsigned tb_ = xbuf_lds + (unsigned)(ib * WS_BUF * 16 + ITp::blk(w, kp) * 2 * 16 * 1024 + mtp * 2048);
                  ws_trp_issue<qa>(tb_ + trl, tb_ + trl2, tp);
                }
              });
            }
            if constexpr (g + BD < G) b_read(std::integral_constant<int, g + BD>{}, bq[g % BD]);
            if constexpr (SPREAD && k < NHOST) {
              using SP = WsSpread<G, (NPI > 0 ? NPI : 1)>;
              sfor<0, (SPREAD ? NPI : 0)>([&](auto ic) {
                constexpr int i = decltype(ic)::value, pi = k * NPI + i, kp = pi / 4, qa = pi % 4;
                if constexpr (SP::perm_at(i) == g) ws_trp_perm<SP::newer(SP::issue_at(i), true, g, BD)>(tp);
                if constexpr (SP::store_at(i) == g) {
                  ws_trp_store<qa, SP::newer(SP::perm_at(i), false, g, BD)>(actp, 32 * MTp, s0 + 64 * ITp::blk(w, kp), mtp, lane, tp);
                  if constexpr (!TAN && qa == 3 && Net::L[R > 0 ? R - 1 : 0].relu != 0) maskp[((size_t)(2 * tile + ITp::blk(w, kp)) * MTp + mtp) * 64 + lane] = pbits[kp];
                }
              });
            }
            if (k == KL && g < Gn) A[g] = load_a(Wn, Gn, mtn, g, lane);
          });
          if (k < KL) {
            if constexpr (ls.pf != 0) load_bias(IT::blk(w, k + 1), bv);
          }
          if constexpr (!LAST && ls.add_ext == 0) {
#pragma unroll
            for (int t = 0; t < 2; ++t) acc_fence(acc[t]);
            unsigned int pw[2][8];
#pragma unroll
            for (int t = 0; t < 2; ++t)
#pragma unroll
              for (int kk = 0; kk < 8; ++kk) pw[t][kk] = pack2bf_op(acc[t][2 * kk], acc[t][2 * kk + 1]);
            if constexpr (ls.relu != 0 && TAN) {
#pragma unroll
              for (int t = 0; t < 2; ++t)
#pragma unroll
                for (int kk = 0; kk < 8; ++kk) pw[t][kk] = pk_mask_bf16(pw[t][kk], pk_m01(tbits[k], t, kk));
            } else if constexpr (ls.relu != 0) {
              if constexpr (ST) pbits[k] = pk_alive_bits(pw);
#pragma unroll
              for (int t = 0; t < 2; ++t)
#pragma unroll
                for (int kk = 0; kk < 8; ++kk) pw[t][kk] = pk_relu_bf16(pw[t][kk]);
            }
#pragma unroll
            for (int t = 0; t < 2; ++t)
#pragma unroll
              for (int q = 0; q < 2; ++q)
                xout[((2 * b + t) * 16 + 2 * mt + q) * 64 + lane_s] = make_uint4(pw[t][4 * q], pw[t][4 * q + 1], pw[t][4 * q + 2], pw[t][4 * q + 3]);
          } else if constexpr (!LAST) {
            if constexpr (ls.relu != 0) {
              if constexpr (ST) {
                unsigned int bits = 0;
#pragma unroll
                for (int t = 0; t < 2; ++t)
#pragma unroll
                  for (int r = 0; r < 16; ++r) bits |= (acc[t][r] > 0.f ? 1u : 0u) << mask_bit<P>(t, r);
                pbits[k] = bits;
              }
#pragma unroll
              for (int t = 0; t < 2; ++t)
#pragma unroll
                for (int r = 0; r < 16; ++r) acc[t][r] = relu1(acc[t][r]);
            }
            {
              f32x16_t e[2];
              tile_from_raw<P>(ext_raw, lane, e);
#pragma unroll
              for (int t = 0; t < 2; ++t)
#pragma unroll
                for (int r = 0; r < 16; ++r) acc[t][r] += e[t][r];
            }
            if (k < KL) load_ext(IT::blk(w, k + 1));
#pragma unroll
            for (int t = 0; t < 2; ++t) {
              uint4 u[2];
              tile_to_units<P>(acc[t], u);
#pragma unroll
              for (int q = 0; q < 2; ++q) xout[((2 * b + t) * 16 + 2 * mt + q) * 64 + lane_s] = u[q];
            }
          } else {
#pragma unroll
            for (int t = 0; t < 2; ++t) {
              const int s = s0 + 64 * b + 2 * n + t;
#pragma unroll
              for (int r = 0; r < 16; ++r) {
                const int f = 32 * mt + drow(r, h);
                if (f < Net::COUT && s < S_eff && a.out) a.out[(size_t)s * Net::COUT + f] = acc[t][r];
              }
            }
          }
        });
      } else {
        a_load(std::integral_constant<int, 0>{}, std::integral_constant<int, (Gn < G ? Gn : G)>{}, Wn, Gn, mtn);
      }
      ws_layer_barrier();
      Wn_c = Wn_n;
      act_c = act_n;
      mask_c = mask_n;
      ws_pin_sgpr(Wn_c);
      ws_pin_sgpr(act_c);
      ws_pin_sgpr(mask_c);
    });
    xcur = xnext;
  }
}

template <class Net>
constexpr int wsb_gk(int l) { return pad32(Net::L[l].mout) / 16; }
template <class Net>
constexpr bool wsb_same(int a, int b) {
  if (!bwd_same<Net>(a, b)) return false;
  if ((a == Net::NL - 1) != (b == Net::NL - 1)) return false;
  const int an = a > 0 ? a - 1 : Net::NL - 1, bn = b > 0 ? b - 1 : Net::NL - 1;
  return wsb_gk<Net>(an) == wsb_gk<Net>(bn);
}
template <class Net>
constexpr int wsb_rep(int l) {
  for (int j = Net::NL - 1; j > l; --j)
    if (wsb_same<Net>(j, l)) return j;
  return l;
}
template <class Net>
constexpr unsigned wsb_members(int r) {
  unsigned m = 0;
  for (int l = 0; l < Net::NL; ++l)
    if (wsb_rep<Net>(l) == r) m |= 1u << l;
  return m;
}
template <class Net>
__device__ __forceinline__ int wsb_first_tile(int l, int w, bool want_dx) {
  int v = 0;
  sfor<0, Net::NL>([&](auto ic) {
    constexpr int i = decltype(ic)::value;
    constexpr int MTE = Net::L[i].ke / 32, MTA = Net::L[i].kin / 32;
    if (l == i) {
      if (MTE > 0 && want_dx && w < 2 * MTE) v = w % (MTE > 0 ? MTE : 1);
      else v = (i > 0 && MTA > 0) ? MTE + (w & ((MTA > 0 ? MTA : 1) - 1)) : 0;
    }
  });
  return v;
}
template <class Net>
__device__ __forceinline__ int wsb_mta_rt(int l) {
  int v = 0;
  sfor<0, Net::NL>([&](auto ic) {
    constexpr int i = decltype(ic)::value;
    if (l == i) v = i > 0 ? Net::L[i].kin / 32 : 0;
  });
  return v;
}

template <class Net, bool DZ = true>
__global__ void __launch_bounds__(512) k_mlp_bwd_ws(BwdK a) {
  static_assert(ws_ok<Net>(), "weights-stationary chain: 256-wide posenc nets only");
  using P = PBF16;
  constexpr int NL = Net::NL, KE = Net::KE, GMAX = 16;
  constexpr int MTE_ANY = KE / 32;
  __shared__ uint4 xbuf[2 * WS_BUF];
  __shared__ float red[8 * 2 * 3 * 32];
  const int tid = threadIdx.x, lane = tid & 63, n = lane & 31, h = lane >> 5;
  const int w = __builtin_amdgcn_readfirstlane((int)(threadIdx.x >> 6));
  const unsigned xbuf_lds = lds_addr(xbuf);
  const unsigned trl = ws_tr_lane(lane), trl2 = trl ^ 32u;
  const int lane_s = ws_slot(lane);
  const int ntw = a.S_pad / WS_TILE;
  const bool want_dx = a.d_x != nullptr;

  uint4 A[GMAX];
  auto a_load = [&](auto g1c, const GLOBAL_AS void* Wp, int G, int rt) {
    constexpr int G1 = decltype(g1c)::value;
#pragma unroll
    for (int g = 0; g < G1; ++g) A[g] = load_a(Wp, G, rt, g, lane);
  };
  if ((int)blockIdx.x < ntw) {
    constexpr int GK0 = wsb_gk<Net>(NL - 1);
    a_load(std::integral_constant<int, GK0>{}, KARG_PTR(BwdK, const void*, WT, NL - 1), GK0, wsb_first_tile<Net>(NL - 1, w, want_dx));
  }
  TrTile trt;
  auto mask_slot_after = [](int ln_) { const int q = ln_ > 0 ? ln_ - 1 : 0; return q >= 1 ? q - 1 : 0; };
  const GLOBAL_AS void* Wn_c = KARG_PTR(BwdK, const void*, WT, (NL >= 2 ? NL - 2 : 0));
  GLOBAL_AS void* dz_c = KARG_PTR(BwdK, void*, dz, NL - 1);
  const GLOBAL_AS unsigned int* maskq_c = KARG_PTR(BwdK, const unsigned int*, mask, mask_slot_after(NL - 1));
  auto mask_req = [&](int lq , int tile, unsigned int (&m)[2], const GLOBAL_AS unsigned int* mp) {
    int mta = wsb_mta_rt<Net>(lq >= 1 ? lq : 1);
    mta = mta > 0 ? mta : 8;
    const int j = w & (mta - 1);
#pragma unroll
    for (int k = 0; k < 2; ++k) {
      const int b = mta >= 8 ? k : ((w / mta) & 1);
      m[k] = mp[((size_t)(2 * tile + b) * mta + j) * 64 + lane];
    }
  };

  constexpr bool DPRE = Net::COUT <= 4;
  constexpr int DN = DPRE ? Net::COUT : 1;
  auto d_fetch = [&](int tile_, float (&d)[2][DN]) {
    if constexpr (DPRE) {
      if (w < 2 && tile_ < ntw) {
#pragma unroll
        for (int t = 0; t < 2; ++t) {
          const int s = tile_ * WS_TILE + 64 * w + 2 * n + t;
#pragma unroll
          for (int r = 0; r < DN; ++r) {
            const int f = drow(r, h);
            d[t][r] = (f < Net::COUT && s < a.S) ? a.d_out[(size_t)s * Net::COUT + f] : 0.f;
          }
        }
      }
    }
  };
  float dcur[2][DN], dnext[2][DN];
#pragma unroll
  for (int t = 0; t < 2; ++t)
#pragma unroll
    for (int r = 0; r < DN; ++r) dcur[t][r] = dnext[t][r] = 0.f;
  d_fetch((int)blockIdx.x, dcur);
  for (int tile = blockIdx.x; tile < ntw; tile += gridDim.x) {
    const int s0 = tile * WS_TILE;
    d_fetch(tile + (int)gridDim.x, dnext);
    float dx[2][3];
#pragma unroll
    for (int t = 0; t < 2; ++t) dx[t][0] = dx[t][1] = dx[t][2] = 0.f;
    unsigned int mcur[2], mnext[2];
    mask_req(NL - 1, tile, mcur, KARG_PTR(BwdK, const unsigned int*, mask, (NL >= 2 ? NL - 2 : 0)));

    if (w < 2) {
      const int b = w;
      f32x16_t g[2];
#pragma unroll
      for (int t = 0; t < 2; ++t) {
        const int s = s0 + 64 * b + 2 * n + t;
#pragma unroll
        for (int r = 0; r < 16; ++r) {
          const int f = drow(r, h);
          if constexpr (DPRE) g[t][r] = r < DN ? dcur[t][r < DN ? r : 0] : 0.f;
          else g[t][r] = (f < Net::COUT && s < a.S) ? a.d_out[(size_t)s * Net::COUT + f] : 0.f;
        }
      }
      if constexpr (DZ) store_tile<P>((GLOBAL_AS void*)a.dz[NL - 1], pad32(Net::L[NL - 1].mout), s0 + 64 * b, 0, lane, g);
#pragma unroll
      for (int t = 0; t < 2; ++t) {
        uint4 u[2];
        tile_to_units<P>(g[t], u);
#pragma unroll
        for (int q = 0; q < 2; ++q) xbuf[((2 * b + t) * 16 + q) * 64 + lane_s] = u[q];
      }
    }
    wg_step_barrier();

#pragma nounroll
    for (int l = NL - 1; l >= 0; --l)
    sfor<0, NL>([&](auto ri) {
      constexpr int R = NL - 1 - decltype(ri)::value;
      if constexpr (wsb_rep<Net>(R) != R) return;
      constexpr unsigned MEMBERS = wsb_members<Net>(R);
      if (!((MEMBERS >> l) & 1u)) return;
      constexpr LS ls = Net::L[R];
      constexpr LS lp = Net::L[R > 0 ? R - 1 : 0];
      constexpr int GK = wsb_gk<Net>(R);
      constexpr int MTE = ls.ke / 32, MTA = ls.kin / 32;
      constexpr bool DO_ACT = (R > 0 && MTA > 0);
      constexpr int GKn = wsb_gk<Net>(R > 0 ? R - 1 : NL - 1);
      using IT = WsItems<(DO_ACT ? MTA : 1)>;
      const int lm1 = l > 0 ? l - 1 : 0;
      const int ln = l > 0 ? l - 1 : NL - 1;
      const GLOBAL_AS void* Wn = Wn_c;
      const GLOBAL_AS void* Wn_n = KARG_PTR(BwdK, const void*, WT, (ln > 0 ? ln - 1 : NL - 1));
      GLOBAL_AS void* dz_n = KARG_PTR(BwdK, void*, dz, ln);
      const GLOBAL_AS unsigned int* maskq_n = KARG_PTR(BwdK, const unsigned int*, mask, mask_slot_after(ln));
      const int rtn = wsb_first_tile<Net>(ln, w, want_dx);
      const int ib = (NL - 1 - l) & 1;
      uint4* xout = xbuf + (ib ^ 1) * WS_BUF;
      const bool act_on = DO_ACT && IT::active(w);
      const bool emb_on = MTE > 0 && want_dx && w < 2 * MTE;
      const int j = IT::mt(w);
      const int me = MTE > 0 ? w % (MTE > 0 ? MTE : 1) : 0, be = MTE > 0 ? (w / (MTE > 0 ? MTE : 1)) & 1 : 0;

#pragma unroll
      for (int g = GK; g < GKn; ++g) A[g] = load_a(Wn, GKn, rtn, g, lane);
      mask_req(lm1, tile, mnext, maskq_c);
      uint4 raw[4];
      if constexpr (MTE > 0) {
        if (emb_on) load_tile_raw<P>((const GLOBAL_AS void*)a.emb, KE, s0 + 64 * be, me, lane, raw);
      }
      if constexpr (DO_ACT && lp.ext_grad != 0) {
        if (act_on && !emb_on) load_tile_raw<P>((const GLOBAL_AS void*)a.ext_gin, pad32(lp.mout), s0 + 64 * IT::blk(w, 0), j, lane, raw);
      }
      static_assert(!(MTE > 0 && DO_ACT && lp.ext_grad != 0), "one prefetched tile per layer");
      constexpr int MTp = GK / 2;
      using ITp = WsItems<MTp>;
      constexpr int NP = (DZ && R < NL - 1) ? 4 * ITp::IPW : 0;
      constexpr int NHOST = IT::IPW;
      constexpr int NPI = NP / NHOST;
      constexpr bool SPREAD = NP > 0 && DO_ACT && IT::ITEMS >= 8 && ITp::ITEMS >= 8 && NP % NHOST == 0 && WsSpread<GK, (NPI > 0 ? NPI : 1)>::OK;
      GLOBAL_AS void* dzl = dz_c;
      const int jp = ITp::mt(w);
      if constexpr (NP > 0 && !SPREAD) {
        if (ITp::active(w)) {
#pragma unroll
          for (int k = 0; k < ITp::IPW; ++k) {
            const int b = ITp::blk(w, k);
            {
              const unsigned tb_ = xbuf_lds + (unsigned)(ib * WS_BUF * 16 + b * 2 * 16 * 1024 + jp * 2048);
              ws_tr_issue(tb_ + trl, tb_ + trl2, trt);
            }
            tr_wait(trt);
            tr_store(dzl, 32 * MTp, s0 + 64 * b, jp, lane, trt);
          }
        }
      }
      WsPiece tp;

      auto mfma_item = [&](int b, f32x16_t (&acc)[2], auto pf_c, auto gp_c, const GLOBAL_AS void* Wp, int rt, auto host_c) {
        constexpr bool PF = decltype(pf_c)::value;
        constexpr int GP = decltype(gp_c)::value;
        constexpr int HK = decltype(host_c)::value;
#pragma unroll
        for (int t = 0; t < 2; ++t)
#pragma unroll
          for (int r = 0; r < 16; ++r) acc[t][r] = 0.f;
        constexpr int BD = GK < WS_BD ? GK : WS_BD;
        u32x4_t bq[BD][2];
        const unsigned px_a = xbuf_lds + (unsigned)(ib * WS_BUF * 16 + (2 * b * 16) * 1024 + lane_s * 16);
        auto b_read = [&](auto gc, u32x4_t (&dst)[2]) {
          constexpr int g = decltype(gc)::value;
          ws_lds_read<g * 1024>(dst[0], px_a);
          ws_lds_read<(16 + g) * 1024>(dst[1], px_a);
        };
        sfor<0, BD>([&](auto gc) { b_read(gc, bq[decltype(gc)::value]); });
        sfor<0, GK>([&](auto gc) {
          constexpr int g = decltype(gc)::value;
          constexpr int NEWER = 2 * ((GK - 1 - g) < (BD - 1) ? (GK - 1 - g) : (BD - 1));
          ws_lds_wait<NEWER>(bq[g % BD][0], bq[g % BD][1]);
          mma_b(acc[0], A[g], bq[g % BD][0]);
          mma_b(acc[1], A[g], bq[g % BD][1]);
          if constexpr (SPREAD && HK >= 0 && HK < NHOST) {
            using SP = WsSpread<GK, (NPI > 0 ? NPI : 1)>;
            sfor<0, (SPREAD ? NPI : 0)>([&](auto ic) {
              constexpr int i = decltype(ic)::value, pi = (HK >= 0 ? HK : 0) * NPI + i, kp = pi / 4, qa = pi % 4;
              if constexpr (SP::issue_at(i) == g) {
                const unsigned tb_ = xbuf_lds + (unsigned)(ib * WS_BUF * 16 + ITp::blk(w, kp) * 2 * 16 * 1024 + jp * 2048);
                ws_trp_issue<qa>(tb_ + trl, tb_ + trl2, tp);
              }
            });
          }
          if constexpr (g + BD < GK) b_read(std::integral_constant<int, g + BD>{}, bq[g % BD]);
          if constexpr (SPREAD && HK >= 0 && HK < NHOST) {
            using SP = WsSpread<GK, (NPI > 0 ? NPI : 1)>;
            sfor<0, (SPREAD ? NPI : 0)>([&](auto ic) {
              constexpr int i = decltype(ic)::value, pi = (HK >= 0 ? HK : 0) * NPI + i, kp = pi / 4, qa = pi % 4;
              if constexpr (SP::perm_at(i) == g) ws_trp_perm<SP::newer(SP::issue_at(i), true, g, BD)>(tp);
              if constexpr (SP::store_at(i) == g) ws_trp_store<qa, SP::newer(SP::perm_at(i), false, g, BD)>(dzl, 32 * MTp, s0 + 64 * ITp::blk(w, kp), jp, lane, tp);
            });
          }
          if constexpr (PF && g < GP) A[g] = load_a(Wp, GP, rt, g, lane);
        });
      };

      bool loaded_next = false;
      if constexpr (MTE > 0) {
        if (emb_on) {
          f32x16_t acc[2];
          if constexpr (DO_ACT) mfma_item(be, acc, std::true_type{}, std::integral_constant<int, GK>{}, KARG_PTR(BwdK, const void*, WT, l), MTE + j, std::integral_constant<int, -1>{});
          else { mfma_item(be, acc, std::true_type{}, std::integral_constant<int, GKn>{}, Wn, rtn, std::integral_constant<int, -1>{}); loaded_next = true; }
          f32x16_t e[2];
          tile_from_raw<P>(raw, lane, e);
          constexpr int L = Net::NFREQ;
          sfor<0, (MTE > 0 ? MTE : 1)>([&](auto mc) {
            constexpr int MEc = decltype(mc)::value;
            if (me != MEc) return;
            sfor<0, 16>([&](auto rc) {
              constexpr int r = decltype(rc)::value;
              constexpr int S0 = 32 * MEc + (r & 3) + 8 * (r >> 2), S1 = S0 + 4;
              constexpr int K0 = S0 < 6 * L ? 1 : (S0 < 6 * L + 3 ? 2 : 0), K1 = S1 < 6 * L ? 1 : (S1 < 6 * L + 3 ? 2 : 0);
              if constexpr (K0 != 0 || K1 != 0) {
                constexpr int F0 = (S0 >> 1) / 3, F1 = (S1 >> 1) / 3;
                constexpr int A0 = K0 == 1 ? (S0 >> 1) % 3 : (K0 == 2 ? S0 - 6 * L : -1), A1 = K1 == 1 ? (S1 >> 1) % 3 : (K1 == 2 ? S1 - 6 * L : -1);
#pragma unroll
                for (int t = 0; t < 2; ++t) {
                  const float gv = acc[t][r];
                  const float partner = e[t][r ^ 1];
                  const float sp = (r & 1) ? -partner : partner;
                  float c;
                  if constexpr (K0 == 1 && K1 == 1) {
                    c = ldexpf(sp, h ? F1 : F0) * gv;
                  } else {
                    const float c0 = K0 == 1 ? ldexpf(sp, F0) * gv : (K0 == 2 ? gv : 0.f);
                    const float c1 = K1 == 1 ? ldexpf(sp, F1) * gv : (K1 == 2 ? gv : 0.f);
                    c = h ? c1 : c0;
                  }
#pragma unroll
                  for (int k = 0; k < 3; ++k) {
                    if (A0 == k && A1 == k) dx[t][k] += c;
                    else if (A0 == k) dx[t][k] += h ? 0.f : c;
                    else if (A1 == k) dx[t][k] += h ? c : 0.f;
                  }
                }
              }
            });
          });
        }
      }
      if constexpr (DO_ACT) {
        if (act_on) {
          sfor<0, IT::IPW>([&](auto kc) {
            constexpr int k = decltype(kc)::value;
            const int b = IT::blk(w, k);
            constexpr int KL = IT::IPW - 1;
              f32x16_t acc[2];
            if constexpr (k == KL) mfma_item(b, acc, std::true_type{}, std::integral_constant<int, GKn>{}, Wn, rtn, kc);
            else mfma_item(b, acc, std::false_type{}, std::integral_constant<int, 0>{}, Wn, rtn, kc);
            if constexpr (lp.ext_grad != 0) {
              f32x16_t eg[2];
              tile_from_raw<P>(raw, lane, eg);
#pragma unroll
              for (int t = 0; t < 2; ++t)
#pragma unroll
                for (int r = 0; r < 16; ++r) acc[t][r] += eg[t][r];
              if (k < KL) load_tile_raw<P>((const GLOBAL_AS void*)a.ext_gin, pad32(lp.mout), s0 + 64 * IT::blk(w, k + 1), j, lane, raw);
            }
            if constexpr (lp.add_ext != 0) store_tile<P>((GLOBAL_AS void*)a.ext_gout, pad32(lp.mout), s0 + 64 * b, j, lane, acc);
#pragma unroll
            for (int t = 0; t < 2; ++t) acc_fence(acc[t]);
            unsigned int pw[2][8];
#pragma unroll
            for (int t = 0; t < 2; ++t)
#pragma unroll
              for (int kk = 0; kk < 8; ++kk) pw[t][kk] = pack2bf_op(acc[t][2 * kk], acc[t][2 * kk + 1]);
            {
              unsigned int alive = lp.relu != 0 ? mcur[k] : 0xffffffffu;
#pragma unroll
              for (int t = 0; t < 2; ++t)
                if (s0 + 64 * b + 2 * n + t >= a.S) alive &= ~(0x00ff00ffu << (8 * t));
#pragma unroll
              for (int t = 0; t < 2; ++t)
#pragma unroll
                for (int kk = 0; kk < 8; ++kk) pw[t][kk] = pk_mask_bf16(pw[t][kk], pk_m01(alive, t, kk));
            }
#pragma unroll
            for (int t = 0; t < 2; ++t)
#pragma unroll
              for (int q = 0; q < 2; ++q)
                xout[((2 * b + t) * 16 + 2 * j + q) * 64 + lane_s] = make_uint4(pw[t][4 * q], pw[t][4 * q + 1], pw[t][4 * q + 2], pw[t][4 * q + 3]);
          });
          loaded_next = true;
        }
      }
      if (!loaded_next) a_load(std::integral_constant<int, (GKn < GK ? GKn : GK)>{}, Wn, GKn, rtn);
      mcur[0] = mnext[0];
      mcur[1] = mnext[1];
      ws_layer_barrier();
      Wn_c = Wn_n;
      dz_c = dz_n;
      maskq_c = maskq_n;
      ws_pin_sgpr(Wn_c);
      ws_pin_sgpr(dz_c);
      ws_pin_sgpr(maskq_c);
    });

#pragma unroll
    for (int t = 0; t < 2; ++t)
#pragma unroll
      for (int r = 0; r < DN; ++r) dcur[t][r] = dnext[t][r];
    if (want_dx) {
      if (w < 2 * MTE_ANY) {
#pragma unroll
        for (int t = 0; t < 2; ++t)
#pragma unroll
          for (int k = 0; k < 3; ++k) {
            const float v = dx[t][k] + __shfl_xor(dx[t][k], 32, 64);
            if (h == 0) red[((w * 2 + t) * 3 + k) * 32 + n] = v;
          }
      }
      wg_step_barrier();
      if (w < 2 && h == 0) {
        const int b = w;
#pragma unroll
        for (int t = 0; t < 2; ++t) {
          const int s = s0 + 64 * b + 2 * n + t;
          float v[3] = {0.f, 0.f, 0.f};
#pragma unroll
          for (int m = 0; m < MTE_ANY; ++m)
#pragma unroll
            for (int k = 0; k < 3; ++k) v[k] += red[(((b * MTE_ANY + m) * 2 + t) * 3 + k) * 32 + n];
          if (s < a.S) {
            a.d_x[(size_t)s * 3 + 0] = v[0];
            a.d_x[(size_t)s * 3 + 1] = v[1];
            a.d_x[(size_t)s * 3 + 2] = v[2];
          }
        }
      }
    }
  }
}

inline int mlp_grid_ws(int ntiles) {
  static int n_cu = 0;
  if (n_cu == 0) {
    int dev = 0;
    hipDeviceProp_t prop;
    if (hipGetDevice(&dev) != hipSuccess || hipGetDeviceProperties(&prop, dev) != hipSuccess) prop.multiProcessorCount = 256;
    n_cu = prop.multiProcessorCount > 0 ? prop.multiProcessorCount : 256;
  }
  const char* ge = getenv("LAB4D_CHAIN_GRID");
  const int grid_env = ge ? atoi(ge) : 0;
  int g = ntiles < n_cu ? ntiles : n_cu;
  if (grid_env > 0 && g > grid_env) g = grid_env;
  return g < 1 ? 1 : g;
}

inline bool ws_enabled() {
  const char* e = getenv("LAB4D_WS");
  return e == nullptr || atoi(e) != 0;
}

}
```

### lab4d_amd/csrc/pointwise.hip

```cpp
#include "common.hpp"

namespace lab4d {

template <int C>
__global__ void __launch_bounds__(256) k_l2norm_fwd(const float* __restrict__ x, long S, float* __restrict__ y) {
  for (long s = (long)blockIdx.x * blockDim.x + threadIdx.x; s < S; s += (long)gridDim.x * blockDim.x) {
    float v[C];
    float q = 0.f;
#pragma unroll
    for (int c = 0; c < C; ++c) { v[c] = x[s * C + c]; q += v[c] * v[c]; }
    const float inv = 1.f / sqrtf(q);
#pragma unroll
    for (int c = 0; c < C; ++c) y[s * C + c] = v[c] * inv;
  }
}
template <int C>
__global__ void __launch_bounds__(256) k_l2norm_bwd(const float* __restrict__ x, const float* __restrict__ g, long S, float* __restrict__ gx) {
  for (long s = (long)blockIdx.x * blockDim.x + threadIdx.x; s < S; s += (long)gridDim.x * blockDim.x) {
    float v[C], gv[C];
    float q = 0.f, d = 0.f;
#pragma unroll
    for (int c = 0; c < C; ++c) { v[c] = x[s * C + c]; gv[c] = g[s * C + c]; q += v[c] * v[c]; d += v[c] * gv[c]; }
    const float inv = 1.f / sqrtf(q);
    const float k = d * inv * inv;
#pragma unroll
    for (int c = 0; c < C; ++c) gx[s * C + c] = (gv[c] - v[c] * k) * inv;
  }
}

__global__ void __launch_bounds__(256) k_eik_tangent_input(const float* __restrict__ x, const float* __restrict__ g, const float* __restrict__ ge,
                                                           const float* __restrict__ freq_w, long S, int L, int KE, float* __restrict__ u) {
  for (long s = (long)blockIdx.x * blockDim.x + threadIdx.x; s < S; s += (long)gridDim.x * blockDim.x) {
    const float g0 = g[s * 3], g1 = g[s * 3 + 1], g2 = g[s * 3 + 2];
    const float gn = sqrtf(g0 * g0 + g1 * g1 + g2 * g2);
    const float k = gn > 0.f ? ge[s] * (2.f * (gn - 1.f) / fmaxf(gn, 1e-38f)) : 0.f;
    const float d[3] = {k * g0, k * g1, k * g2};
    const float xv[3] = {x[s * 3], x[s * 3 + 1], x[s * 3 + 2]};
    float* row = u + s * KE;
    for (int f = 0; f < L; ++f) {
      const float fr = ldexpf(1.f, f);
      const float wf = freq_w ? fr * freq_w[f] : fr;
#pragma unroll
      for (int a = 0; a < 3; ++a) {
        float sn, cs;
        sincosf(xv[a] * fr, &sn, &cs);
        row[2 * (3 * f + a)] = wf * cs * d[a];
        row[2 * (3 * f + a) + 1] = -wf * sn * d[a];
      }
    }
    row[6 * L] = d[0]; row[6 * L + 1] = d[1]; row[6 * L + 2] = d[2];
    for (int c = 6 * L + 3; c < KE; ++c) row[c] = 0.f;
  }
}

}
using namespace lab4d;

extern "C" int lab4d_l2_normalize_forward(const float* x, int S, int C, float* y, void* stream) {
  LAB4D_REQUIRE(x && y, "l2_normalize_forward: null pointer");
  LAB4D_REQUIRE(C == 16 || C == 3, "l2_normalize_forward: C must be 16 (feature field) or 3 (got %d)", C);
  if (S == 0) return LAB4D_OK;
  if (C == 16) hipLaunchKernelGGL((k_l2norm_fwd<16>), dim3(grid_1d(S, 256, 16384)), dim3(256), 0, (hipStream_t)stream, x, (long)S, y);
  else hipLaunchKernelGGL((k_l2norm_fwd<3>), dim3(grid_1d(S, 256, 16384)), dim3(256), 0, (hipStream_t)stream, x, (long)S, y);
  return check_launch("l2_normalize_forward");
}

extern "C" int lab4d_l2_normalize_backward(const float* x, const float* g, int S, int C, float* g_x, void* stream) {
  LAB4D_REQUIRE(x && g && g_x, "l2_normalize_backward: null pointer");
  LAB4D_REQUIRE(C == 16 || C == 3, "l2_normalize_backward: C must be 16 or 3 (got %d)", C);
  if (S == 0) return LAB4D_OK;
  if (C == 16) hipLaunchKernelGGL((k_l2norm_bwd<16>), dim3(grid_1d(S, 256, 16384)), dim3(256), 0, (hipStream_t)stream, x, g, (long)S, g_x);
  else hipLaunchKernelGGL((k_l2norm_bwd<3>), dim3(grid_1d(S, 256, 16384)), dim3(256), 0, (hipStream_t)stream, x, g, (long)S, g_x);
  return check_launch("l2_normalize_backward");
}

extern "C" int lab4d_eikonal_tangent_input(const float* x, const float* g, const float* ge, const float* freq_w, int S, int L, int KE, float* u,
                                           void* stream) {
  LAB4D_REQUIRE(x && g && ge && u, "eikonal_tangent_input: null pointer");
  LAB4D_REQUIRE(L >= 0 && KE >= 6 * L + 3, "eikonal_tangent_input: KE = %d is too small for %d bands", KE, L);
  if (S == 0) return LAB4D_OK;
  hipLaunchKernelGGL(k_eik_tangent_input, dim3(grid_1d(S, 256, 16384)), dim3(256), 0, (hipStream_t)stream, x, g, ge, freq_w, (long)S, L, KE, u);
  return check_launch("eikonal_tangent_input");
}
```

### lab4d_amd/deformable.py

```python
import ctypes
import os

import torch
import torch.nn.functional as F
from torch.autograd import Function
from torch.autograd.function import once_differentiable

from . import _lib, mlp
from . import quat_utils as Q
from . import render_utils as RU
from .warping import composed_warp, dense_warp, skinning_warp, skinning_warp_forward_multi

vp, ci, cf = ctypes.c_void_p, ctypes.c_int, ctypes.c_float


def flip_pair(x):
    if torch.is_tensor(x):
        if len(x) < 2:
            return x
        return x.view(x.shape[0] // 2, 2, -1).flip(1).view(x.shape)
    if isinstance(x, tuple):
        return tuple(flip_pair(t) for t in x)
    if isinstance(x, dict):
        return {k: flip_pair(v) for k, v in x.items()}
    return x


def _spf(x):
    n = 1
    for d in x.shape[1:-1]:
        n *= d
    return n


def rigid_apply(q, t, x):
    shp = (x.shape[0],) + (1,) * (x.dim() - 2)
    w = q[:, 0].view(shp + (1,))
    v = q[:, 1:].view(shp + (3,))
    out = (w * w - (v * v).sum(-1, keepdim=True)) * x + 2 * (v * x).sum(-1, keepdim=True) * v + 2 * w * torch.linalg.cross(v.expand_as(x), x)
    return out + t.view(shp + (3,))


def pinhole_projection(Kmat, xyz_cam):
    shp = (xyz_cam.shape[0],) + (1,) * (xyz_cam.dim() - 2)
    K = Kmat.view(shp + (3, 3))
    hxy = (K * xyz_cam.unsqueeze(-2)).sum(-1)
    return hxy / (hxy[..., -1:] + 1e-6)


class GaussDensity(Function):
    @staticmethod
    def forward(ctx, xyz, centres, ibeta):
        xyz, centres = xyz.contiguous(), centres.contiguous()
        _lib.require_device(xyz, centres)
        S, B = xyz.shape[0], centres.shape[0]
        out = torch.empty(S, 1, device=xyz.device)
        best = torch.empty(S, dtype=torch.int32, device=xyz.device)
        ib = ibeta.detach().reshape(1).float().contiguous()
        _lib.call("gauss_density_forward", xyz, centres, B, ib, S, out, best)
        ctx.save_for_backward(xyz, centres, best, ib)
        return out

    @staticmethod
    @once_differentiable
    def backward(ctx, g):
        xyz, centres, best, ib = ctx.saved_tensors
        g = g.contiguous()
        gx = torch.empty_like(xyz)
        gc = torch.zeros_like(centres)
        gi = torch.zeros(1, device=xyz.device)
        _lib.call("gauss_density_backward", xyz, centres, centres.shape[0], ib, best, g, xyz.shape[0], gx, gc, gi)
        return gx, gc, gi


def gauss_density(P, xyz, rest_articulation, ft=None):
    if ft is not None:
        centre, ibeta = ft["gauss_centre"], ft["gauss_ibeta"]
    else:
        _, centre = Q.dual_quaternion_to_quaternion_translation((rest_articulation[0][:1], rest_articulation[1][:1]))
        ibeta = P["warp.logibeta"].exp()
    out = GaussDensity.apply(xyz.reshape(-1, 3), centre[0], ibeta)
    return out.view(xyz.shape[:-1] + (1,))


def _flip_yz(n):
    return torch.cat([n[..., :1], -n[..., 1:]], -1)


class FlowCyc(Function):

    @staticmethod
    def forward(ctx, xyz_next, q, t, Kmat, hxy, xyz_cyc, xyz_t, flow_thresh):
        xyz_next, q, t, Kmat, hxy = [x.contiguous().float() for x in (xyz_next, q, t, Kmat, hxy)]
        has_cyc = xyz_cyc is not None
        if has_cyc:
            xyz_cyc, xyz_t = xyz_cyc.contiguous().float(), xyz_t.contiguous().float()
        _lib.require_device(xyz_next, q, t, Kmat, hxy, xyz_cyc, xyz_t)
        M, N, D = xyz_next.shape[:3]
        S = M * N * D
        flow = torch.empty(M, N, D, 3, device=xyz_next.device)
        cyc = torch.empty(M, N, D, 1, device=xyz_next.device) if has_cyc else None
        _lib.call("flow_cyc_forward", xyz_next, q, t, Kmat, hxy, xyz_cyc, xyz_t, S, N * D, D, -1.0 if flow_thresh is None else float(flow_thresh), flow, cyc)
        ctx.save_for_backward(xyz_next, q, t, Kmat, xyz_cyc, xyz_t)
        ctx.dims = (M, N, D)
        return (flow, cyc) if has_cyc else (flow, None)

    @staticmethod
    @once_differentiable
    def backward(ctx, g_flow, g_cyc):
        xyz_next, q, t, Kmat, xyz_cyc, xyz_t = ctx.saved_tensors
        M, N, D = ctx.dims
        S = M * N * D
        has_cyc = xyz_cyc is not None
        g_flow = g_flow.contiguous()
        if has_cyc:
            g_cyc = torch.zeros(M, N, D, 1, device=g_flow.device) if g_cyc is None else g_cyc.contiguous()
        g_next = torch.empty_like(xyz_next)
        g_pf = torch.empty(M, 16, device=g_flow.device)
        g_xc = torch.empty_like(xyz_cyc) if has_cyc else None
        g_xt = torch.empty_like(xyz_t) if has_cyc else None
        _lib.call("flow_cyc_backward", xyz_next, q, t, Kmat, xyz_cyc, xyz_t, g_flow, g_cyc if has_cyc else None, S, N * D, M, g_next, g_pf, g_xc, g_xt)
        return g_next, g_pf[:, :4], g_pf[:, 4:7], g_pf[:, 7:].reshape(M, 3, 3), None, g_xc, g_xt, None


class VolSdfDensity(Function):

    @staticmethod
    def forward(ctx, sdf, ibeta):
        sdf_c, ib = sdf.contiguous().float(), ibeta.reshape(1).contiguous().float()
        _lib.require_device(sdf_c, ib)
        out = torch.empty_like(sdf_c)
        _lib.call("volsdf_forward", sdf_c, ib, sdf_c.numel(), out)
        ctx.save_for_backward(sdf_c, ib)
        ctx.ib_shape = ibeta.shape
        return out

    @staticmethod
    @once_differentiable
    def backward(ctx, g):
        sdf, ib = ctx.saved_tensors
        g = g.contiguous()
        g_sdf = torch.empty_like(sdf)
        g_ib = torch.empty(1, device=sdf.device) if ctx.needs_input_grad[1] else None
        _lib.call("volsdf_backward", sdf, ib, g, sdf.numel(), g_sdf, g_ib)
        return g_sdf, None if g_ib is None else g_ib.view(ctx.ib_shape)


def volsdf_density(sdf, logibeta):
    return VolSdfDensity.apply(sdf, logibeta.exp())


EIK_REUSE = os.environ.get("LAB4D_EIK_REUSE", "1") != "0"


def posenc_window(alpha, n_freq, device):
    if alpha is None:
        return None
    w = torch.clamp(alpha * n_freq - torch.arange(n_freq, dtype=torch.float32, device=device), 0.0, 1.0)
    return 0.5 * (1 + torch.cos(torch.pi * w + torch.pi))


def nerf_forward(P, xyz, fr, prec, with_color=True, get_density=True, alpha=None, ft=None, tap=None):
    shape = xyz.shape
    spf = _spf(xyz)
    x = xyz.reshape(-1, 3)
    dev = x.device
    r = mlp.run_chain(mlp.NET_FG_BASE, prec, P, x, spf, conds={0: fr["code_base"], 4: fr["code_base"]}, export_layer=8 if with_color else None,
                      freq_w=posenc_window(alpha, 10, dev), pfs_pre=None if ft is None else {0: ft["pf.base0"], 4: ft["pf.base4"]}, tap=tap)
    sdf, feat = r if with_color else (r, None)
    sdf = sdf.view(shape[:-1] + (1,))
    if get_density:
        out = volsdf_density(sdf, P["logibeta"])
    else:
        out = sdf
    if not with_color:
        return out
    rgb = mlp.run_chain(mlp.NET_FG_COLOR, prec, P, x, spf, conds={0: fr["code_color"], 3: fr["appr_code"]}, ext=feat,
                        freq_w=posenc_window(alpha, 12, dev), pfs_pre=None if ft is None else {0: ft["pf.color0"], 3: ft["pf.color3"]})
    return torch.sigmoid(rgb).view(shape[:-1] + (3,)), out


def nerf_forward_bg(P, xyz, dir, codes, prec, get_density=True, alpha=None, prefix="", tap=None):
    shape = xyz.shape
    spf = _spf(xyz)
    x = xyz.reshape(-1, 3)
    dev = x.device
    r = mlp.run_chain(mlp.NET_BG_BASE, prec, P, x, spf, conds={0: codes["basefield"], 4: codes["basefield"]}, export_layer=5 if dir is not None else None,
                      freq_w=posenc_window(alpha, 6, dev), prefix=prefix, tap=tap)
    sdf, feat = r if dir is not None else (r, None)
    sdf = sdf.view(shape[:-1] + (1,))
    if get_density:
        out = volsdf_density(sdf, P[prefix + "logibeta"])
    else:
        out = sdf
    if dir is None:
        return out
    rgb = mlp.run_chain(mlp.NET_BG_COLOR, prec, P, x, spf, conds={0: codes["colorfield"]}, ext=feat, freq_w=posenc_window(alpha, 8, dev),
                        prefix=prefix, x2=dir.reshape(-1, 3))
    return torch.sigmoid(rgb).view(shape[:-1] + (3,)), out


def vis_field(P, xyz, fr, prec, ft=None):
    out = mlp.run_chain(mlp.NET_VIS, prec, P, xyz.reshape(-1, 3), _spf(xyz), conds={0: fr["code_vis"]},
                        pfs_pre=None if ft is None else {0: ft["pf.vis0"]})
    return out.view(xyz.shape[:-1] + (1,))


class L2Normalize(Function):

    @staticmethod
    def forward(ctx, x):
        x = x.contiguous()
        _lib.require_device(x)
        S, C = x.shape
        y = torch.empty_like(x)
        _lib.call("l2_normalize_forward", x, S, C, y)
        ctx.save_for_backward(x)
        return y

    @staticmethod
    @once_differentiable
    def backward(ctx, g):
        (x,) = ctx.saved_tensors
        g = g.contiguous()
        gx = torch.empty_like(x)
        _lib.call("l2_normalize_backward", x, g, x.shape[0], x.shape[1], gx)
        return gx


def compute_feat(P, xyz, prec):
    f = mlp.run_chain(mlp.NET_FEAT, prec, P, xyz.reshape(-1, 3), _spf(xyz))
    return L2Normalize.apply(f).view(xyz.shape[:-1] + (16,))


class GlobalMatch(Function):

    @staticmethod
    def forward(ctx, feat_px, feat_c, xyz_c, logsigma):
        feat_px, feat_c, xyz_c, logsigma = [t.detach().contiguous().float() for t in (feat_px, feat_c, xyz_c, logsigma)]
        _lib.require_device(feat_px, feat_c, xyz_c, logsigma)
        R, C = feat_px.shape
        K = feat_c.shape[0]
        out = torch.empty(R, 3, device=feat_px.device)
        stats = torch.empty(R, 2, device=feat_px.device)
        with _lib.timed("k_match_fwd", (2.0 * R * K * (C + 3), 4.0 * (R * (C + 5) + K * (C + 3)))):
            _lib.call("global_match_forward", feat_px, feat_c, xyz_c, logsigma, R, C, K, out, stats)
        ctx.save_for_backward(feat_px, feat_c, xyz_c, logsigma, out, stats)
        return out

    @staticmethod
    @once_differentiable
    def backward(ctx, g):
        if ctx.needs_input_grad[0]:
            raise NotImplementedError("GlobalMatch: the pixel features are data (samples_dict['feature'], feature.py:127): no gradient path")
        feat_px, feat_c, xyz_c, logsigma, out, stats = ctx.saved_tensors
        R, C = feat_px.shape
        K = feat_c.shape[0]
        g = g.contiguous().float()
        g_fc, g_xc, g_ls = torch.empty_like(feat_c), torch.empty_like(xyz_c), torch.empty_like(logsigma)
        work = torch.empty(_lib.lib().lab4d_global_match_workspace_floats(K), device=g.device)
        with _lib.timed("k_match_bwd", (2.0 * R * K * (2 * C + 8), 4.0 * (R * (C + 8) + 2 * K * (C + 3)))):
            _lib.call("global_match_backward", feat_px, feat_c, xyz_c, logsigma, out, stats, g, R, C, K, g_fc, g_xc, g_ls, work)
        return None, g_fc, g_xc, g_ls


class RowTap(Function):

    @staticmethod
    def forward(ctx, x, idx):
        ctx.save_for_backward(idx)
        ctx.x_shape = x.shape
        return x.view_as(x), x.detach()[idx]

    @staticmethod
    @once_differentiable
    def backward(ctx, g_dense, g_rows):
        (idx,) = ctx.saved_tensors
        if g_dense is None:
            g_dense = torch.zeros(ctx.x_shape, device=idx.device)
        elif not g_dense.is_contiguous():
            g_dense = g_dense.contiguous()
        elif g_rows is not None and (g_dense._use_count() > 2 or g_dense._is_view()):
            g_dense = g_dense.clone()
        if g_rows is not None:
            g_dense.index_add_(0, idx, g_rows.to(g_dense.dtype))
        return g_dense, None


def global_match(P, feat_px, feat_rows, xyz_rows):
    shape = feat_px.shape
    out = GlobalMatch.apply(feat_px.reshape(-1, shape[-1]), feat_rows, xyz_rows, P["logsigma"].reshape(1))
    return out.view(shape[:-1] + (3,))


def eikonal_subsample(P, xyz, code, rand_inds, alpha=None, prec=mlp.PREC_F32, net=mlp.NET_FG_BASE, prefix="", pf_tables=None, tap=None):
    M, N, D, _ = xyz.shape
    pts = xyz.reshape(M * N, D, 3)
    out = torch.zeros(M * N, D, device=xyz.device)
    if rand_inds is None:
        rand_inds = torch.arange(M * N, device=xyz.device)
    ray_frame = torch.div(rand_inds, N, rounding_mode="floor")
    x = pts[rand_inds].detach().reshape(-1, 3)
    if pf_tables is not None:
        ray_code, pf_rows = None, (pf_tables[0].index_select(0, ray_frame), pf_tables[1].index_select(0, ray_frame))
    else:
        ray_code, pf_rows = code[ray_frame], None
    eik_tap = None
    if tap and D % 64 == 0:
        eik_tap = (tap, (rand_inds[:, None] * (D // 64) + torch.arange(D // 64, device=xyz.device)).reshape(-1))
    e = mlp.eikonal_sdf(P, x, ray_code, D, prec, freq_w=posenc_window(alpha, mlp.describe(net).n_freq, xyz.device), prefix=prefix, net=net,
                        pf_rows=pf_rows, tap=eik_tap)
    out = out.index_put((rand_inds,), e.view(-1, D))
    return out.reshape(M, N, D, 1)


def frame_terms(P, fr):
    from .warping import SKIN_AFFINE, get_gauss, skin_affine_table, skin_cond
    ft = {}
    M = fr["field2cam"][0].shape[0]
    ft["cam2field.q"], ft["cam2field.t"] = Q.quaternion_translation_inverse(fr["field2cam"][0], fr["field2cam"][1])
    nxt = flip_pair({k: fr.get(k) for k in ["Kinv", "field2cam", "t_articulation"]})
    ft["Kmat"], ft["Kmat_next"] = Q.kmatinv(fr["Kinv"]), Q.kmatinv(nxt["Kinv"])
    ft["field2cam_next.q"], ft["field2cam_next.t"] = nxt["field2cam"][0].contiguous(), nxt["field2cam"][1].contiguous()
    ft["scale"] = P["logscale"].exp()
    motion = fr.get("motion", "skinning")
    if motion not in ("rigid", "dense"):
        _, centre = Q.dual_quaternion_to_quaternion_translation((fr["rest_articulation"][0][:1], fr["rest_articulation"][1][:1]))
        ft["gauss_centre"], ft["gauss_ibeta"] = centre, P["warp.logibeta"].exp()
    W = lambda net, l: P[mlp.bindings(net)[l].wname]
    ft["pf.base0"] = mlp.pf_bias_of(mlp.NET_FG_BASE, 0, W(mlp.NET_FG_BASE, 0), fr["code_base"])
    ft["pf.base4"] = mlp.pf_bias_of(mlp.NET_FG_BASE, 4, W(mlp.NET_FG_BASE, 4), fr["code_base"])
    ft["pf.color0"] = mlp.pf_bias_of(mlp.NET_FG_COLOR, 0, W(mlp.NET_FG_COLOR, 0), fr["code_color"])
    ft["pf.color3"] = mlp.pf_bias_of(mlp.NET_FG_COLOR, 3, W(mlp.NET_FG_COLOR, 3), fr["appr_code"])
    ft["pf.vis0"] = mlp.pf_bias_of(mlp.NET_VIS, 0, W(mlp.NET_VIS, 0), fr["code_vis"])
    if fr.get("dense") is None and motion == "skinning":
        t_art, rest = fr["t_articulation"], fr["rest_articulation"]
        skin = mlp.skin_net_for(t_art[0].shape[1])
        ft["gauss"] = get_gauss(P)
        ft["se3_bw.r"], ft["se3_bw.d"] = Q.dual_quaternion_mul(rest, Q.dual_quaternion_inverse(t_art))
        rest_inv = Q.dual_quaternion_inverse(rest)
        ft["se3_next.r"], ft["se3_next.d"] = Q.dual_quaternion_mul(nxt["t_articulation"], rest_inv)
        ft["se3_own.r"], ft["se3_own.d"] = Q.dual_quaternion_mul(t_art, rest_inv)
        ft["pf.skin_bw"] = mlp.pf_bias_of(skin, 0, W(skin, 0), skin_cond(fr["t_embed"], fr["code_skin"], M))
        ft["pf.skin_fw"] = mlp.pf_bias_of(skin, 0, W(skin, 0), skin_cond(fr["t_embed_mean"], fr["code_skin"], M))
        if SKIN_AFFINE:
            B = t_art[0].shape[1]
            ft["skinA.bw"] = skin_affine_table(P, t_art, ft["gauss"], ft["pf.skin_bw"], B)
            ft["skinA.fw"] = skin_affine_table(P, rest, ft["gauss"], ft["pf.skin_fw"], B)
    return ft


class FramePrologue:

    def __init__(self, P, fr):
        self.P, self.fr = P, fr
        self.outs, self.leaves = None, None

    def refresh(self):
        self.outs = frame_terms(self.P, self.fr)
        if self.leaves is None:
            self.leaves = {}
            for k, v in self.outs.items():
                leaf = v.detach().clone().contiguous()
                if v.requires_grad:
                    leaf.requires_grad_(True)
                    leaf.grad = torch.zeros_like(leaf)
                self.leaves[k] = leaf
        else:
            with torch.no_grad():
                for k, v in self.outs.items():
                    self.leaves[k].copy_(v)
        return dict(self.fr, frame_terms=self.leaves)

    def zero_grad(self):
        for leaf in (self.leaves or {}).values():
            if leaf.grad is not None:
                leaf.grad.zero_()

    def backward(self):
        ks = [k for k, v in self.outs.items() if v.requires_grad]
        if ks:
            torch.autograd.backward([self.outs[k] for k in ks], [self.leaves[k].grad for k in ks])
            for k in ks:
                self.leaves[k].grad.zero_()
        self.outs = None
# ... 523 lines not shown
```

### lab4d_amd/mlp.py

```python
import ctypes
import os
import weakref
from typing import NamedTuple

import torch
from torch.autograd import Function
from torch.autograd.function import once_differentiable

from . import _lib

MAXL = 12
PREC_F32, PREC_BF16 = 0, 1
vp, ci = ctypes.c_void_p, ctypes.c_int


@_lib.mirrors("lab4d_mlp_layer")
class LayerDesc(ctypes.Structure):
    _fields_ = [(n, ci) for n in ("ke", "kin", "mout", "mout_pad", "relu", "pf_bias", "add_ext", "ext_grad")]


@_lib.mirrors("lab4d_mlp_desc")
class NetDesc(ctypes.Structure):
    _fields_ = [(n, ci) for n in ("n_layers", "emb_kind", "n_freq", "c_in", "emb_slots", "ke", "c_out")] + [("layers", LayerDesc * MAXL)]


@_lib.mirrors("lab4d_mlp_fwd_args")
class FwdArgs(ctypes.Structure):
    _fields_ = [("net", ci), ("precision", ci), ("S", ci), ("S_pad", ci), ("ld", ci), ("spf", ci), ("x", vp), ("freq_w", vp),
                ("W", vp * MAXL), ("bias", vp * MAXL), ("pf_bias", vp * MAXL), ("act", vp * MAXL), ("mask", vp * MAXL), ("emb", vp),
                ("ext", vp), ("out", vp), ("x2", vp), ("S_dev", vp), ("frame_idx", vp), ("aff", vp)]


@_lib.mirrors("lab4d_mlp_bwd_args")
class BwdArgs(ctypes.Structure):
    _fields_ = [("net", ci), ("precision", ci), ("S", ci), ("S_pad", ci), ("ld", ci), ("spf", ci), ("WT", vp * MAXL), ("act", vp * MAXL),
                ("mask", vp * MAXL), ("emb", vp), ("ext", vp), ("d_out", vp), ("ext_gin", vp), ("ext_gout", vp), ("dz", vp * MAXL), ("d_x", vp),
                ("d_x2", vp), ("x", vp), ("aff", vp), ("g_aff", vp)]


@_lib.mirrors("lab4d_mlp_bwd_fused_args")
class BwdFusedArgs(ctypes.Structure):
    _fields_ = [("net", ci), ("precision", ci), ("S", ci), ("spf", ci), ("x", vp), ("freq_w", vp), ("aff", vp), ("W", vp * MAXL), ("WT", vp * MAXL),
                ("bias", vp * MAXL), ("pf_bias", vp * MAXL), ("d_out", vp), ("d_x", vp), ("g_aff", vp), ("dW", vp * MAXL), ("db", vp * MAXL),
                ("pf_db", vp * MAXL)]


class NetInfo(NamedTuple):
    id: int
    name: str
    kernel: str
    macs: int
    ws: bool


NETS = (
    NetInfo(0, "fg_base", "FgBase", 572928 + 256, True),
    NetInfo(1, "fg_color", "FgColor", 158464 + 37248, True),
    NetInfo(2, "vis", "Vis", 10240, False),
    NetInfo(3, "feat", "Feat", 77568, False),
    NetInfo(4, "skin", "Skin", 20736, False),
    NetInfo(5, "dense", "Dense", 39 * 256 + 256 * 256 + 256 * 3, True),
    NetInfo(6, "bg_base", "BgBase", 100096 + 128, False),
    NetInfo(7, "bg_color", "BgColor", 43392 + 8576, False),
    NetInfo(8, "skin18", "Skin18", (54 + 160) * 64 + 64 * 64 + 64 * 18, False),
    NetInfo(9, "hash_geo", "HashGeo", 32 * 64 + 64 * 16, False),
    NetInfo(10, "hash_color", "HashColor", 19 * 64 + 64 * 64 + 64 * 3, False),
    NetInfo(11, "dense6", "Dense6", 199 * 256 + 3 * 256 * 256 + 455 * 256 + 256 * 256 + 256 * 3, True),
    NetInfo(12, "skin_a", "SkinA", 4 * 64 + 64 * 64 + 64 * 25, False),
    NetInfo(13, "skin18_a", "Skin18A", 4 * 64 + 64 * 64 + 64 * 18, False),
)
(NET_FG_BASE, NET_FG_COLOR, NET_VIS, NET_FEAT, NET_SKIN, NET_DENSE, NET_BG_BASE, NET_BG_COLOR, NET_SKIN18, NET_HASH_GEO, NET_HASH_COLOR, NET_DENSE6,
 NET_SKIN_A, NET_SKIN18_A) = (n.id for n in NETS)
NET_NAMES = {n.id: n.name for n in NETS}
KERNEL_NET = {n.id: n.kernel for n in NETS}
NET_MACS = {n.id: n.macs for n in NETS}
WS_NETS = tuple(n.id for n in NETS if n.ws)


def ws_active(net, prec, dx_only=False):
    e = os.environ.get("LAB4D_WS")
    try:
        on = e is None or int(e.strip() or "0") != 0
    except ValueError:
        on = False
    return bool(on and prec == PREC_BF16 and net in WS_NETS)


def chain_kernel_name(kind, net, prec, dx_only=False):
    return "k_mlp_%s%s<%s>" % (kind, "_ws" if ws_active(net, prec, dx_only) else "", KERNEL_NET[net])


def wgrad_kernel_name(L, prec):
    if prec == PREC_BF16 and L.mout_pad == 32 and os.environ.get("LAB4D_WGRAD_HEAD_DMA", "1") not in ("", "0") and L.ke + L.kin <= 256:
        return "k_mlp_wgrad_dma<1,%d>" % (2 if L.ke + L.kin <= 128 else 4)
    if prec == PREC_BF16 and L.mout_pad in (64, 128, 256):
        K = L.ke + L.kin
        nbw = 1 if K <= 64 else (2 if K <= 128 else (3 if K <= 192 else (4 if K <= 256 else (5 if (L.mout_pad == 256 and K <= 320) else 3))))
        return "k_mlp_wgrad_dma<%d,%d>" % (L.mout_pad // 32, nbw)
    if L.mout_pad >= 256:
        return "k_mlp_wgrad_big"
    return "k_mlp_wgrad<%d>" % (4 if L.mout_pad >= 128 else (2 if L.mout_pad >= 64 else 1))


def wgrad_work(L, S_pad, prec):
    K = L.ke + L.kin
    esize = 2 if prec == PREC_BF16 else 4
    return (2.0 * S_pad * L.mout * K, float((L.mout_pad + K) * S_pad * esize + L.mout_pad * K * 4))


_DESC = {}


def describe(net):
    if net not in _DESC:
        d = NetDesc()
        _lib.call("mlp_describe", net, ctypes.byref(d))
        _DESC[net] = d
    return _DESC[net]


def store_dtype(prec):
    return torch.bfloat16 if prec == PREC_BF16 else torch.float32


def posenc_slot_to_ref_channel(n_freq, ke):
    out = []
    for slot in range(ke):
        if slot < 6 * n_freq:
            pair, t = slot >> 1, slot & 1
            f, a = pair // 3, pair % 3
            out.append(3 + f * 6 + t * 3 + a)
        elif slot < 6 * n_freq + 3:
            out.append(slot - 6 * n_freq)
        else:
            out.append(-1)
    return out


class LayerBinding:

    def __init__(self, wname, bname, emb0=None, cond=None, prev0=None, aux0=None):
        self.wname, self.bname = wname, bname
        self.aux0 = aux0
        self.emb0 = emb0
        self.cond = cond
        self.prev0 = prev0


def _lb(q, name, **blocks):
    return LayerBinding(q + name + ".weight", q + name + ".bias", **blocks)


def _hidden(q, D, n_emb, n_cond=0, skip=None):
    cond = (n_emb, n_cond) if n_cond else None
    out = [_lb(q, "linear_1.0", emb0=0, cond=cond)]
    for i in range(2, D + 1):
        out.append(_lb(q, "linear_%d.0" % i, emb0=0, cond=cond, prev0=n_emb + n_cond) if i == (skip or 0) + 1 else _lb(q, "linear_%d.0" % i, prev0=0))
    return out


def _mlp(q, D, n_emb, n_cond=0, skip=None):
    return _hidden(q, D, n_emb, n_cond, skip) + [_lb(q, "linear_final", prev0=0)]


def bindings(net, prefix=""):
# ... 112 lines not shown
    out = _pack_into(net, layer, prec, W, transposed, hit[1] if (hit is not None and hit[1].device == W.device) else None)
    if not ALWAYS_PACK:
        per[key] = (ver, out)
    return out


def _pack_into(net, layer, prec, W, transposed, out=None):
    d = describe(net)
    L = d.layers[layer]
    Wc = W.detach().contiguous()
    _lib.require_device(Wc)
    if out is None or ALWAYS_PACK:
        out = torch.empty(L.mout_pad * (L.ke + L.kin), dtype=store_dtype(prec), device=W.device)
    cm = col_map(net, layer, W.device)
    _lib.call("mlp_pack", net, layer, prec, 1 if transposed else 0, Wc, Wc.shape[1], cm, out)
    return out


def repack_all(force=False):
    n = 0
    for ref, per in list(_PACK_CACHE.values()):
        W = ref()
        if W is None:
            continue
        for key, (ver, buf) in list(per.items()):
            if force or ver != W._version:
                per[key] = (W._version, _pack_into(key[0], key[1], key[2], W, key[3], buf))
                n += 1
    return n


def clear_caches():
    _PACK_CACHE.clear()
    _COLMAP.clear()
    _COLIDX.clear()


def pf_bias_of(net, layer, W, cond):
    c0, n = bindings(net)[layer].cond
    return cond @ W[:, c0:c0 + n].t()


def s_pad_of(S):
    return (S + 255) // 256 * 256


def buf_numel(F, S_pad):
    return (S_pad // 64) * (F * 64 + 128)


def mask_numel(L, S_pad, prec):
    return (S_pad // (64 if prec == PREC_BF16 else 32)) * (L.mout_pad // 32) * 64


def bind_forward(net, prec, S, S_pad, spf, Ws, bs, pfs):
    d = describe(net)
    a = FwdArgs()
    a.net, a.precision, a.S, a.S_pad, a.ld, a.spf = net, prec, S, S_pad, S_pad, spf
    pfs = iter(pfs)
    packed, biases, tables = [], [], []
    for l in range(d.n_layers):
        L = d.layers[l]
        pw = packed_weights(net, l, prec, Ws[l], False)
        b = bs[l].detach().float()
        if b.numel() != L.mout_pad:
            b = torch.nn.functional.pad(b, (0, L.mout_pad - b.numel()))
        b = b.contiguous()
        a.W[l], a.bias[l] = _lib.dp(pw), _lib.dp(b)
        pf = None
        if L.pf_bias:
            pf = (next(pfs).detach().float() + b[None]).contiguous()
            if pf.shape[1] != L.mout_pad:
                raise RuntimeError("per-frame bias of layer %d must have %d columns" % (l, L.mout_pad))
            a.pf_bias[l] = _lib.dp(pf)
        packed.append(pw)
        biases.append(b)
        tables.append(pf)
    return a, packed, biases, tables


def bind_backward(net, prec, S, S_pad, spf, Ws, masks, with_dz=True, ext_gin=None):
    d = describe(net)
    dev, sdt = Ws[0].device, store_dtype(prec)
    a = BwdArgs()
    a.net, a.precision, a.S, a.S_pad, a.ld, a.spf = net, prec, S, S_pad, S_pad, spf
    packed_t, dz = [], [None] * d.n_layers
    for l in range(d.n_layers):
        L = d.layers[l]
        pw = packed_weights(net, l, prec, Ws[l], True)
        a.WT[l] = _lib.dp(pw)
        packed_t.append(pw)
        if masks[l] is not None:
            a.mask[l] = _lib.dp(masks[l])
        if with_dz:
            dz[l] = torch.empty(buf_numel(L.mout_pad, S_pad), dtype=sdt, device=dev)
            a.dz[l] = _lib.dp(dz[l])
        if L.ext_grad:
            if ext_gin is None:
                ext_gin = torch.zeros(buf_numel(L.mout_pad, S_pad), dtype=sdt, device=dev)
            ext_gin = ext_gin.contiguous()
            a.ext_gin = _lib.dp(ext_gin)
    return a, packed_t, dz, ext_gin


def _to_reference(net, l, W, dWk, sink=None):
    kcols, rcols = col_index(net, l, W.device)
    mout = describe(net).layers[l].mout
    if sink is not None:
        sink.index_add_(1, rcols, dWk[:mout].index_select(1, kcols))
        return None
    gW = torch.zeros_like(W, dtype=torch.float32)
    gW[:, rcols] = dWk[:mout][:, kcols]
    return gW


def collect_wgrads(net, prec, S, S_pad, spf, M, Ws, bs, emb, layers, eikonal=False):
    d = describe(net)
    bias_out, tag, what = (False, "@eik", "(eikonal)") if eikonal else (True, "", "")
    dev = emb.device
    sinks, sizes = [], []
    for l, (_, _, need_w, need_b, _) in enumerate(layers):
        L = d.layers[l]
        sw = _grad_sink(Ws[l]) if need_w else None
        sb = _grad_sink(bs[l]) if (need_b and sw is not None and not L.pf_bias) else None
        sinks.append((sw, sb))
        sizes.append((0 if sw is not None else L.mout_pad * (L.ke + L.kin), L.mout_pad if (bias_out and sb is None) else 0,
                      M * L.mout_pad if L.pf_bias else 0))
    arena = torch.zeros(sum(sum(t) for t in sizes), device=dev)
    aoff = 0
    out = []
    for l, (dz, prev, need_w, need_b, need_pf) in enumerate(layers):
        L = d.layers[l]
        gW = gb = pfd = None
        if need_w or need_b or need_pf:
            (n0, n1, n2), (sw, sb) = sizes[l], sinks[l]
            dWk = arena[aoff:aoff + n0].view(L.mout_pad, L.ke + L.kin) if sw is None else None
            dbk = arena[aoff + n0:aoff + n0 + n1] if (bias_out and sb is None) else None
            pfd = arena[aoff + n0 + n1:aoff + n0 + n1 + n2].view(M, L.mout_pad) if need_pf else None
            with _lib.timed(wgrad_kernel_name(L, prec) + tag, wgrad_work(L, S_pad, prec)):
                if sw is not None:
                    _lib.call("mlp_wgrad_mapped", net, l, prec, S, S_pad, S_pad, spf, dz, emb, prev, sw, sw.shape[1], col_map(net, l, dev),
                              sb if sb is not None else dbk, pfd, M, what="mlp_wgrad_mapped" + what)
                else:
                    _lib.call("mlp_wgrad", net, l, prec, S, S_pad, S_pad, spf, dz, emb, prev, dWk, dbk, pfd, M, what="mlp_wgrad" + what)
            if need_w and sw is None:
                gW = _to_reference(net, l, Ws[l], dWk)
            if need_b and sb is None:
                gb = (pfd.sum(0) if need_pf else dbk)[:L.mout].reshape(bs[l].shape)
        aoff += sum(sizes[l])
        out.append((gW, gb, pfd))
    return out


CHAIN_LEAD = ("net", "prec", "spf", "x", "ext", "freq_w", "export_layer", "n_pf", "x2", "tap")


class Wants:

    def __init__(self, x=False, ext=False, freq_w=False, x2=False, pfs=(), params=()):
        self.x, self.ext, self.freq_w, self.x2, self.pfs, self.params = bool(x), bool(ext), bool(freq_w), bool(x2), tuple(pfs), tuple(params)

    @property
    def beyond_x(self):
        return self.ext or self.freq_w or self.x2 or any(self.pfs) or any(self.params)

    @property
    def any(self):
        return self.x or self.beyond_x


class ChainState:
    __slots__ = ("net", "prec", "spf", "S", "S_pad",
                 "want",
                 "params",
                 "pf_used",
                 "acts", "masks", "emb", "ext",
                 "dx_only",
                 "fused",
                 "x_shape", "has_x2",
                 "aff_in",
                 "g_aff")

    def __init__(self, **kw):
        for k in self.__slots__:
            setattr(self, k, kw.pop(k))
        assert not kw, kw


def chain_forward(net, prec, spf, x, pfs, params, want, ext=None, freq_w=None, export_layer=-1, x2=None, aff=None, tap=None):
    d = describe(net)
    NL = d.n_layers
    pfs, params = list(pfs), list(params)
    assert len(params) == 2 * NL
    Ws, bs = params[0::2], params[1::2]
    spf = int(spf)
    x = x.contiguous()
    _lib.require_device(x)
    if x.dtype != torch.float32:
        raise RuntimeError("MlpChain: x must be fp32")
    S = x.shape[0]
    S_pad = s_pad_of(S)
    dev = x.device
    sdt = store_dtype(prec)
    need_grad = want.any
    fused = bool(need_grad and FUSED_NARROW_BWD and export_layer < 0 and ext is None and x2 is None and tap is None
                 and _lib.lib().lab4d_mlp_fused_backward_supported(net, prec, spf))
    store = need_grad and not fused
    dx_only = bool(store and net in (NET_FG_BASE, NET_BG_BASE) and export_layer < 0 and ext is None and tap is None and not want.beyond_x)
    if d.emb_kind == 2 and aff is None:
        raise RuntimeError("MlpChain: net %d needs the per-frame affine table aff" % net)
    if aff is not None:
        rows = d.ke if d.emb_kind == 2 else d.c_in
        if tuple(aff.shape[1:]) != (rows, 4) or x.shape[1] != 3 or aff.dtype != torch.float32 or not aff.is_contiguous():
            raise RuntimeError("MlpChain: aff must be a contiguous fp32 (M, %d, 4) table and x the (S,3) points" % rows)
        _lib.require_device(aff)
    a, pw_used, bias_used, pf_used = bind_forward(net, prec, S, S_pad, spf, Ws, bs, pfs)
    a.x = _lib.dp(x)
    if aff is not None:
        a.aff = _lib.dp(aff)
    if x2 is not None:
        x2 = x2.contiguous().float()
        _lib.require_device(x2)
        a.x2 = _lib.dp(x2)
    if freq_w is not None:
        freq_w = freq_w.contiguous().float()
        a.freq_w = _lib.dp(freq_w)
    acts = [None] * NL
    masks = [None] * NL
    for l in range(NL):
        L = d.layers[l]
        if (store and not dx_only and l + 1 < NL) or l == export_layer:
            acts[l] = torch.empty(buf_numel(L.mout_pad, S_pad), dtype=sdt, device=dev)
            a.act[l] = _lib.dp(acts[l])
        if store and L.relu and l + 1 < NL:
            masks[l] = torch.empty(mask_numel(L, S_pad, prec), dtype=torch.int32, device=dev)
            a.mask[l] = _lib.dp(masks[l])
    emb = None
    if store:
        emb = torch.empty(buf_numel(d.ke, S_pad), dtype=sdt, device=dev)
        a.emb = _lib.dp(emb)
    if ext is not None:
        ext = ext.contiguous()
        if ext.dtype != sdt:
            raise RuntimeError("ext must be stored as %s" % sdt)
        a.ext = _lib.dp(ext)
    out = torch.empty(S, d.c_out, device=dev)
    a.out = _lib.dp(out)
    nbytes = sum(t.numel() * t.element_size() for t in acts + masks + [emb, ext, out, x] if t is not None)
    with _lib.timed(chain_kernel_name("fwd", net, prec, dx_only) + ("" if store else " inference"), (2.0 * S * NET_MACS[net], float(nbytes))):
        _lib.call("mlp_forward", ctypes.byref(a))
    if tap is not None and need_grad:
        tap.update(net=net, prec=prec, S=S, S_pad=S_pad, masks=list(masks), emb=emb)
    st = ChainState(net=net, prec=prec, spf=spf, S=S, S_pad=S_pad, want=want, params=params, pf_used=pf_used, acts=acts, masks=masks, emb=emb,
                    ext=ext, dx_only=dx_only, g_aff=None,
                    fused={"x": x, "freq_w": freq_w, "aff": aff, "W": pw_used, "bias": bias_used} if fused else None,
                    x_shape=x.shape if aff is None else (S, d.c_in),
                    has_x2=x2 is not None,
                    aff_in=(x, aff) if (d.emb_kind == 2 and need_grad) else None)
    return out, (acts[export_layer].view(-1) if export_layer >= 0 else None), st


def chain_backward(st, d_out, d_export=None):
    if st.params is None:
        raise RuntimeError("MlpChain: backward a second time through a chain whose stored activations have been released")
    if st.fused is not None:
        return chain_backward_fused(st, d_out)
    net, prec, spf, S, S_pad, want = st.net, st.prec, st.spf, st.S, st.S_pad, st.want
    d = describe(net)
    NL = d.n_layers
    Ws, bs = st.params[0::2], st.params[1::2]
    dev = d_out.device
    a, packed_t, dz, d_export = bind_backward(net, prec, S, S_pad, spf, Ws, st.masks, with_dz=not st.dx_only, ext_gin=d_export)
    for l in range(NL):
        if st.acts[l] is not None:
            a.act[l] = _lib.dp(st.acts[l])
    if st.emb is not None:
        a.emb = _lib.dp(st.emb)
    ext_g = None
    if st.ext is not None:
        a.ext = _lib.dp(st.ext)
        ext_g = torch.empty_like(st.ext)
        a.ext_gout = _lib.dp(ext_g)
    d_out = d_out.contiguous().float()
    a.d_out = _lib.dp(d_out)
    d_x = d_x2 = g_aff = None
    if st.aff_in is not None:
        xin, aff = st.aff_in
        a.x, a.aff = _lib.dp(xin), _lib.dp(aff)
        g_aff = torch.zeros_like(aff)
        a.g_aff = _lib.dp(g_aff)
    if want.x or want.x2 or g_aff is not None:
        d_x = torch.empty(st.x_shape, device=dev)
        a.d_x = _lib.dp(d_x)
        if st.has_x2:
            d_x2 = torch.empty(st.x_shape, device=dev)
            a.d_x2 = _lib.dp(d_x2)
    nbytes = sum(t.numel() * t.element_size() for t in list(dz) + list(st.masks) + [d_out, d_x, ext_g, st.emb if d_x is not None else None, d_export]
                 if t is not None)
    with _lib.timed(chain_kernel_name("bwd", net, prec, st.dx_only), (2.0 * S * NET_MACS[net], float(nbytes))):
        _lib.call("mlp_backward", ctypes.byref(a))
    need_pf = iter(want.pfs)
    layers = [(dz[l], st.acts[l - 1] if d.layers[l].kin else None, want.params[2 * l], want.params[2 * l + 1],
               bool(d.layers[l].pf_bias) and bool(next(need_pf))) for l in range(NL)]
    grads = collect_wgrads(net, prec, S, S_pad, spf, (S + spf - 1) // spf, Ws, bs, st.emb, layers)
    _release(st, g_aff)
    return d_x, ext_g, d_x2, [g[2] for l, g in enumerate(grads) if d.layers[l].pf_bias], [t for g in grads for t in g[:2]]


def _release(st, g_aff):
    st.acts = st.masks = st.emb = st.ext = st.params = st.aff_in = st.fused = None
    st.g_aff = g_aff


def chain_backward_fused(st, d_out):
    net, prec, spf, S, want = st.net, st.prec, st.spf, st.S, st.want
    d = describe(net)
    NL = d.n_layers
    Ws, bs = st.params[0::2], st.params[1::2]
    f = st.fused
    dev = d_out.device
    M = (S + spf - 1) // spf
    a = BwdFusedArgs()
    a.net, a.precision, a.S, a.spf = net, prec, S, spf
    a.x = _lib.dp(f["x"])
    if f["freq_w"] is not None:
        a.freq_w = _lib.dp(f["freq_w"])
    g_aff = None
    if f["aff"] is not None:
        a.aff = _lib.dp(f["aff"])
        g_aff = torch.zeros_like(f["aff"])
        a.g_aff = _lib.dp(g_aff)
    d_out = d_out.contiguous().float()
    a.d_out = _lib.dp(d_out)
    d_x = None
    if want.x or g_aff is not None:
        d_x = torch.empty(st.x_shape, device=dev)
        a.d_x = _lib.dp(d_x)
    sizes = [(L.mout_pad * (L.ke + L.kin), L.mout_pad, M * L.mout_pad if L.pf_bias else 0) for L in (d.layers[l] for l in range(NL))]
    arena = torch.zeros(sum(sum(t) for t in sizes), device=dev)
    keep, views, aoff = [], [], 0
    for l in range(NL):
        L = d.layers[l]
        n0, n1, n2 = sizes[l]
        dWk, dbk = arena[aoff:aoff + n0].view(L.mout_pad, L.ke + L.kin), arena[aoff + n0:aoff + n0 + n1]
        pfd = arena[aoff + n0 + n1:aoff + n0 + n1 + n2].view(M, L.mout_pad) if L.pf_bias else None
        aoff += n0 + n1 + n2
        views.append((dWk, dbk, pfd))
        pwt = packed_weights(net, l, prec, Ws[l], True)
        keep.append(pwt)
        a.WT[l], a.dW[l] = _lib.dp(pwt), _lib.dp(dWk)
        if l + 1 < NL:
            a.W[l] = _lib.dp(f["W"][l])
        if L.pf_bias:
            a.pf_bias[l], a.pf_db[l] = _lib.dp(st.pf_used[l]), _lib.dp(pfd)
        else:
            a.bias[l], a.db[l] = _lib.dp(f["bias"][l]), _lib.dp(dbk)
    nbytes = 4.0 * S * (3 + d.c_out + (3 if d_x is not None else 0))
    with _lib.timed("k_mlp_bwd_fused<%s>" % KERNEL_NET[net], (2.0 * S * NET_MACS[net] * 3, nbytes)):
        _lib.call("mlp_backward_fused", ctypes.byref(a))
    grads_pf, grads_params = [], []
    need_pf = iter(want.pfs)
    for l in range(NL):
        L = d.layers[l]
        dWk, dbk, pfd = views[l]
        need_w, need_b = want.params[2 * l], want.params[2 * l + 1]
        sw = _grad_sink(Ws[l]) if need_w else None
        gW = _to_reference(net, l, Ws[l], dWk, sw) if need_w else None
        gb = None
        if need_b:
            gb = (pfd.sum(0) if L.pf_bias else dbk)[:L.mout].reshape(bs[l].shape)
            sb = _grad_sink(bs[l]) if sw is not None else None
            if sb is not None:
                sb.add_(gb)
                gb = None
        if L.pf_bias:
            grads_pf.append(pfd if next(need_pf) else None)
        grads_params += [gW, gb]
    _release(st, g_aff)
    return d_x, None, None, grads_pf, grads_params


class MlpChain(Function):

    @staticmethod
    def forward(ctx, *args):
        lead, rest = dict(zip(CHAIN_LEAD, args)), args[len(CHAIN_LEAD):]
        need = dict(zip(CHAIN_LEAD, ctx.needs_input_grad))
        n_pf = lead["n_pf"]
        want = Wants(need["x"], need["ext"], need["freq_w"], need["x2"], ctx.needs_input_grad[len(CHAIN_LEAD):][:n_pf],
                     ctx.needs_input_grad[len(CHAIN_LEAD):][n_pf:])
        out, exported, ctx.state = chain_forward(lead["net"], lead["prec"], lead["spf"], lead["x"], rest[:n_pf], rest[n_pf:], want, ext=lead["ext"],
                                                 freq_w=lead["freq_w"], export_layer=lead["export_layer"], x2=lead["x2"], tap=lead["tap"])
        return out if exported is None else (out, exported)

    @staticmethod
    @once_differentiable
    def backward(ctx, d_out, d_export=None):
        d_x, d_ext, d_x2, g_pfs, g_params = chain_backward(ctx.state, d_out, d_export)
        lead = dict.fromkeys(CHAIN_LEAD)
        lead.update(x=d_x, ext=d_ext, x2=d_x2)
        return (*lead.values(), *g_pfs, *g_params)


def chain_params(net, P, prefix=""):
    return [P[n] for bd in bindings(net, prefix) for n in (bd.wname, bd.bname)]


def run_chain(net, prec, P, x, spf, conds=None, ext=None, freq_w=None, export_layer=None, prefix="", x2=None, pfs_pre=None, tap=None):
    d = describe(net)
    bd = bindings(net, prefix)
    pfs = []
    for l in range(d.n_layers):
        if d.layers[l].pf_bias:
            pfs.append(pfs_pre[l] if pfs_pre is not None and l in pfs_pre else pf_bias_of(net, l, P[bd[l].wname], conds[l]))
    return MlpChain.apply(net, prec, spf, x, ext, freq_w, -1 if export_layer is None else export_layer, len(pfs), x2, tap, *pfs,
                          *chain_params(net, P, prefix))


@torch.no_grad()
def run_chain_compacted(net, prec, P, x, frame_idx, count, conds=None, ext=None, freq_w=None, export_layer=None, prefix=""):
    d = describe(net)
    x = x.contiguous()
    _lib.require_device(x, frame_idx, count)
    if frame_idx.dtype != torch.int32 or count.dtype != torch.int32:
        raise RuntimeError("run_chain_compacted: frame_idx and count must be int32")
    S = x.shape[0]
    S_pad = s_pad_of(S)
    dev, sdt = x.device, store_dtype(prec)
    params = chain_params(net, P, prefix)
    pfs = [pf_bias_of(net, l, params[2 * l], conds[l]) for l in range(d.n_layers) if d.layers[l].pf_bias]
    a, *keep = bind_forward(net, prec, S, S_pad, 1, params[0::2], params[1::2], pfs)
    a.x, a.S_dev, a.frame_idx = _lib.dp(x), _lib.dp(count), _lib.dp(frame_idx)
    if freq_w is not None:
        freq_w = freq_w.contiguous().float()
        a.freq_w = _lib.dp(freq_w)
    exported = None
    if export_layer is not None and export_layer >= 0:
        exported = torch.empty(buf_numel(d.layers[export_layer].mout_pad, S_pad), dtype=sdt, device=dev)
        a.act[export_layer] = _lib.dp(exported)
    if ext is not None:
        if ext.dtype != sdt:
            raise RuntimeError("ext must be stored as %s" % sdt)
        a.ext = _lib.dp(ext)
    out = torch.empty(S, d.c_out, device=dev)
    a.out = _lib.dp(out)
    with _lib.timed(chain_kernel_name("fwd", net, prec) + " inference", (2.0 * S * NET_MACS[net], 0.0)):
        _lib.call("mlp_forward", ctypes.byref(a), what="mlp_forward(compacted)")
    return (out, exported) if exported is not None else out


class EikonalSdf(Function):

    @staticmethod
    def forward(ctx, net, prec, spf, x, freq_w, pf0, pf4, tap, *params):
        if net not in (NET_FG_BASE, NET_BG_BASE):
            raise RuntimeError("EikonalSdf: the eikonal term exists for the basefield / sdf networks only (net %d)" % net)
        d = describe(net)
        NL = d.n_layers
        Ws, bs = params[0::2], params[1::2]
        x = x.detach().contiguous()
        _lib.require_device(x)
        S = x.shape[0]
        S_pad = s_pad_of(S)
        spf = int(spf)
        dev, sdt = x.device, store_dtype(prec)
        a, packed, *keep = bind_forward(net, prec, S, S_pad, spf, Ws, bs, [pf0, pf4])
        a.x = _lib.dp(x)
        fw = None
        if freq_w is not None:
            fw = freq_w.detach().contiguous().float()
            a.freq_w = _lib.dp(fw)
        masks, tact = [None] * NL, [None] * NL
        for l in range(NL - 1):
            L = d.layers[l]
            if L.relu:
                masks[l] = torch.empty(mask_numel(L, S_pad, prec), dtype=torch.int32, device=dev)
                a.mask[l] = _lib.dp(masks[l])
            tact[l] = torch.empty(buf_numel(L.mout_pad, S_pad), dtype=sdt, device=dev)
            a.act[l] = _lib.dp(tact[l])
        emb = torch.empty(buf_numel(d.ke, S_pad), dtype=sdt, device=dev)
        a.emb = _lib.dp(emb)
        sdf = torch.empty(S, 1, device=dev)
        a.out = _lib.dp(sdf)
        reused = False
        if tap is not None:
            src, blk_map = tap
            ok = (src.get("net") == net and src.get("prec") == prec and S % 64 == 0 and S_pad == S and blk_map.numel() == S // 64
                  and src.get("emb") is not None and all((masks[l] is None) == (src["masks"][l] is None) for l in range(NL)))
            if ok:
                nb_src = src["S_pad"] // 64
                tpb = 2 if prec == PREC_F32 else 1
                tile_map = blk_map if tpb == 1 else (blk_map[:, None] * tpb + torch.arange(tpb, device=dev)).reshape(-1)
                for l in range(NL):
                    if masks[l] is not None:
                        masks[l] = src["masks"][l].view(nb_src * tpb, -1).index_select(0, tile_map).reshape(-1)
                emb = src["emb"].view(nb_src, -1).index_select(0, blk_map).reshape(-1)
                reused = True
        if not reused:
            with _lib.timed(chain_kernel_name("fwd", net, prec) + "@eik"):
                _lib.call("mlp_forward", ctypes.byref(a), what="mlp_forward(eikonal primal)")
        bk, packed_t, dz, zero_gin = bind_backward(net, prec, S, S_pad, spf, Ws, masks)
        bk.emb = _lib.dp(emb)
        ones = torch.ones(S, 1, device=dev)
        bk.d_out = _lib.dp(ones)
        g = torch.empty(S, 3, device=dev)
        bk.d_x = _lib.dp(g)
        with _lib.timed(chain_kernel_name("bwd", net, prec) + "@eik"):
            _lib.call("mlp_backward", ctypes.byref(bk), what="mlp_backward(eikonal primal)")
        gn = g.norm(2, dim=-1, keepdim=True)
        ctx.meta = (net, prec, spf, S, S_pad)
        ctx.saved = (x, fw, g, gn, dz, masks, packed, tact)
        ctx.params = params
        return (gn - 1) ** 2

    @staticmethod
    @once_differentiable
    def backward(ctx, ge):
        net, prec, spf, S, S_pad = ctx.meta
        x, fw, g, gn, dz, masks, packed, tact = ctx.saved
        d = describe(net)
        NL, L0 = d.n_layers, d.n_freq
        Ws, bs = ctx.params[0::2], ctx.params[1::2]
        dev, sdt = x.device, store_dtype(prec)
        u = torch.empty(S, d.ke, device=dev)
        _lib.call("eikonal_tangent_input", x, g, ge.contiguous().float(), fw, S, L0, d.ke, u)
        a = FwdArgs()
        a.net, a.precision, a.S, a.S_pad, a.ld, a.spf = net, prec, S, S_pad, S_pad, spf
        a.x = _lib.dp(u)
        for l in range(NL):
            a.W[l] = _lib.dp(packed[l])
            if masks[l] is not None:
                a.mask[l] = _lib.dp(masks[l])
            if l + 1 < NL:
                a.act[l] = _lib.dp(tact[l])
        temb = torch.empty(buf_numel(d.ke, S_pad), dtype=sdt, device=dev)
        a.emb = _lib.dp(temb)
        with _lib.timed(("k_mlp_fwd_ws_tangent<%s>@eik" if (ws_active(net, prec) and net == NET_FG_BASE) else "k_mlp_fwd_tangent<%s>@eik") % KERNEL_NET[net]):
            _lib.call("mlp_forward_tangent", ctypes.byref(a))
        need_w = ctx.needs_input_grad[-2 * NL:][0::2]
        layers = [(dz[l], tact[l - 1] if d.layers[l].kin else None, need_w[l], False, False) for l in range(NL)]
        grads = collect_wgrads(net, prec, S, S_pad, spf, 0, Ws, bs, temb, layers, eikonal=True)
        ctx.saved = None
        return (None,) * (len(ctx.needs_input_grad) - 2 * NL) + tuple(t for gr in grads for t in (gr[0], None))


def eikonal_sdf(P, x, ray_code, spf, prec, freq_w=None, prefix="", net=NET_FG_BASE, pf_rows=None, tap=None):
    bd = bindings(net, prefix)
    if pf_rows is not None:
        pf0, pf4 = pf_rows
    else:
        pf0 = pf_bias_of(net, 0, P[bd[0].wname], ray_code)
        pf4 = pf_bias_of(net, 4, P[bd[4].wname], ray_code)
    return EikonalSdf.apply(net, prec, spf, x, freq_w, pf0, pf4, tap, *chain_params(net, P, prefix))
```

### lab4d_amd/warping.py

```python
import os

import torch
from torch.autograd import Function
from torch.autograd.function import once_differentiable

from . import _lib, mlp
from . import quat_utils as Q


def _blend_bwd_work(S, spf, M, B, device):
    n = int(_lib.lib().lab4d_skin_blend_backward_workspace_floats(S, spf, M, B, 1))
    return torch.empty(n, device=device), n == M * B * 34


FUSE_BONE_COORDS = os.environ.get("LAB4D_FUSE_BONE", "1") != "0"


class BoneCoords(Function):

    @staticmethod
    def forward(ctx, xyz, art_r, art_d, gauss, spf):
        xyz, art_r, art_d, gauss = xyz.contiguous(), art_r.contiguous(), art_d.contiguous(), gauss.contiguous()
        _lib.require_device(xyz, art_r, art_d, gauss)
        S, (M, B) = xyz.shape[0], art_r.shape[:2]
# ... 104 lines not shown

    @staticmethod
    def forward(ctx, net, prec, spf, xyz, tab, *params):
        want = mlp.Wants(x=any(ctx.needs_input_grad), params=ctx.needs_input_grad[SkinChainA.N_LEAD:])
        out, _, ctx.chain = mlp.chain_forward(net, prec, spf, xyz.contiguous(), (), params, want, aff=tab.detach().contiguous())
        return out

    @staticmethod
    @once_differentiable
    def backward(ctx, d_out):
        d_x, _, _, _, g_params = mlp.chain_backward(ctx.chain, d_out)
        return (None, None, None, d_x, ctx.chain.g_aff, *g_params)


SKIN_AFFINE = os.environ.get("LAB4D_SKIN_AFFINE", "1") != "0"


class SkinBlend(Function):

    @staticmethod
    def forward(ctx, xyz, raw, art_r, art_d, gauss, se3_r, se3_d, spf):
        xyz, raw, art_r, art_d, gauss, se3_r, se3_d = [t.contiguous() for t in (xyz, raw, art_r, art_d, gauss, se3_r, se3_d)]
        _lib.require_device(xyz, raw, art_r, art_d, gauss, se3_r, se3_d)
        S, (M, B) = xyz.shape[0], se3_r.shape[:2]
        out = torch.empty(S, 3, device=xyz.device)
        ent = torch.empty(S, 1, device=xyz.device)
        dsk = torch.empty(S, 1, device=xyz.device)
        work = torch.empty(M * B * 12, device=xyz.device)
        with _lib.timed("k_blend_fwd", (0.0, 4.0 * S * (3 + B + 3 + 2))):
            _lib.call("skin_blend_forward", xyz, art_r, art_d, gauss, raw, se3_r, se3_d, S, spf, M, B, out, ent, dsk, work)
        ctx.save_for_backward(xyz, raw, art_r, art_d, gauss, se3_r, se3_d)
        ctx.spf = spf
        return out, ent, dsk

    @staticmethod
    @once_differentiable
    def backward(ctx, g_out, g_ent, g_dsk):
        xyz, raw, art_r, art_d, gauss, se3_r, se3_d = ctx.saved_tensors
        S, (M, B) = xyz.shape[0], se3_r.shape[:2]
        g_out = g_out.contiguous()
        g_ent = g_ent.contiguous() if g_ent is not None else None
        g_dsk = g_dsk.contiguous() if g_dsk is not None else None
        gx, gr = torch.empty_like(xyz), torch.empty_like(raw)
        gse3 = torch.zeros(M, B, 8, device=xyz.device)
        need_p = any(ctx.needs_input_grad[2:5])
        gar = torch.empty_like(art_r) if need_p else None
        gad = torch.empty_like(art_d) if need_p else None
        gg = torch.zeros_like(gauss) if need_p else None
        work, fused = _blend_bwd_work(S, ctx.spf, M, B, xyz.device)
        with _lib.timed("k_blend_bwd+gram", (0.0, 4.0 * S * ((3 + B + 3 + 2) + (3 + B) + (0 if fused else 2 * (2 * B + 18))))):
            _lib.call("skin_blend_backward", xyz, art_r, art_d, gauss, raw, se3_r, se3_d, g_out, g_ent, g_dsk, S, ctx.spf, M, B, gx, gr, gse3, gar, gad, gg,
                      work)
        return gx, gr, gar, gad, gg, gse3[..., :4].contiguous(), gse3[..., 4:].contiguous(), None


class SkinBlendMulti(Function):

    @staticmethod
    def forward(ctx, xyz, raw, art_r, art_d, gauss, spf, *se3s):
        xyz, raw, art_r, art_d, gauss = [t.contiguous() for t in (xyz, raw, art_r, art_d, gauss)]
        se3s = [t.contiguous() for t in se3s]
        _lib.require_device(xyz, raw, art_r, art_d, gauss, *se3s)
        S, (M, B) = xyz.shape[0], art_r.shape[:2]
        outs = []
        for i in range(0, len(se3s), 2):
            out = torch.empty(S, 3, device=xyz.device)
            ent = torch.empty(S, 1, device=xyz.device)
            dsk = torch.empty(S, 1, device=xyz.device)
            work = torch.empty(M * B * 12, device=xyz.device)
            with _lib.timed("k_blend_fwd", (0.0, 4.0 * S * (3 + B + 3 + 2))):
                _lib.call("skin_blend_forward", xyz, art_r, art_d, gauss, raw, se3s[i], se3s[i + 1], S, spf, M, B, out, ent, dsk, work)
            outs += [out, ent, dsk]
        ctx.save_for_backward(xyz, raw, art_r, art_d, gauss, *se3s)
        ctx.spf = spf
        return tuple(outs)

    @staticmethod
    @once_differentiable
    def backward(ctx, *grads):
        xyz, raw, art_r, art_d, gauss, *se3s = ctx.saved_tensors
        S, (M, B) = xyz.shape[0], art_r.shape[:2]
        gx, gr = torch.empty_like(xyz), torch.empty_like(raw)
        need_p = any(ctx.needs_input_grad[2:5])
        work0, fused = _blend_bwd_work(S, ctx.spf, M, B, xyz.device)
        gar = gad = gg = None
        gse3s = []
        first = True
        for i in range(0, len(se3s), 2):
            g_out, g_ent, g_dsk = grads[3 * (i // 2):3 * (i // 2) + 3]
            if g_out is None and g_ent is None and g_dsk is None:
                gse3s += [None, None]
                continue
            g_out = torch.zeros_like(xyz) if g_out is None else g_out.contiguous()
            g_ent = g_ent.contiguous() if g_ent is not None else None
            g_dsk = g_dsk.contiguous() if g_dsk is not None else None
            gse3 = torch.zeros(M, B, 8, device=xyz.device)
            par = torch.empty_like(art_r) if need_p else None
            pad = torch.empty_like(art_d) if need_p else None
            pg = torch.zeros_like(gauss) if need_p else None
            work = work0 if first else _blend_bwd_work(S, ctx.spf, M, B, xyz.device)[0]
            with _lib.timed("k_blend_bwd+gram", (0.0, 4.0 * S * ((3 + B + 3 + 2) + (3 + B) * (1 if first else 2) + (0 if fused else 2 * (2 * B + 18))))):
                _lib.call("skin_blend_backward_acc", xyz, art_r, art_d, gauss, raw, se3s[i], se3s[i + 1], g_out, g_ent, g_dsk, S, ctx.spf, M, B, gx, gr, gse3,
                          par, pad, pg, work, 0 if first else 1)
            first = False
            if need_p:
                gar, gad, gg = (par, pad, pg) if gar is None else (gar + par, gad + pad, gg + pg)
            gse3s += [gse3[..., :4].contiguous(), gse3[..., 4:].contiguous()]
        if first:
            return (None,) * (6 + len(se3s))
        return (gx, gr, gar, gad, gg, None) + tuple(gse3s)


def get_gauss(P):
    lg = P["warp.skinning_model.log_gauss"]
    symm = P.get("warp.skinning_model.symm_idx")
    if symm is not None:
        lg = (lg[symm] + lg) / 2
    return lg.exp()


def _spf(shape):
    spf = 1
    for d in shape[1:-1]:
        spf *= d
    return spf


def skin_cond(t_embed, code, M):
    return torch.cat([t_embed.expand(M, -1), code], -1)


def skin_logits(P, x, art, t_embed, code, M, spf, prec, pre=None):
    gauss = pre["gauss"] if pre is not None else get_gauss(P)
    B = art[0].shape[1]
    net = mlp.skin_net_for(B)
    d, bd = mlp.describe(net), mlp.bindings(net, "")
    if SKIN_AFFINE and FUSE_BONE_COORDS:
        tab = pre.get("tab") if pre is not None else None
        if tab is None:
            pf = pre["pf"] if pre is not None else mlp.pf_bias_of(net, 0, P[bd[0].wname], skin_cond(t_embed, code, M))
            tab = skin_affine_table(P, art, gauss, pf, B)
        net_a = mlp.skin_net_for(B, affine=True)
        bda = mlp.bindings(net_a, "")
        params = []
        for l in range(mlp.describe(net_a).n_layers):
            params += [P[bda[l].wname], P[bda[l].bname]]
        return SkinChainA.apply(net_a, prec, spf, x, tab, *params), gauss
    pf = pre["pf"] if pre is not None else mlp.pf_bias_of(net, 0, P[bd[0].wname], skin_cond(t_embed, code, M))
    params = []
    for l in range(d.n_layers):
        params += [P[bd[l].wname], P[bd[l].bname]]
    if not FUSE_BONE_COORDS:
        bone = BoneCoords.apply(x, art[0], art[1], gauss, spf)
        return mlp.MlpChain.apply(net, prec, spf, bone, None, None, -1, 1, None, None, pf, *params), gauss
    return SkinChain.apply(net, prec, spf, x, art[0], art[1], gauss, 1, pf, *params), gauss


def skinning_warp(P, xyz, t_articulation, rest_articulation, t_embed, code, backward, prec=mlp.PREC_F32, pre=None):
    shape = xyz.shape
    M, spf = shape[0], _spf(shape)
    if pre is not None:
        se3 = pre["se3"]
        art = t_articulation if backward else rest_articulation
    elif backward:
        se3 = Q.dual_quaternion_mul(rest_articulation, Q.dual_quaternion_inverse(t_articulation))
        art = t_articulation
    else:
        se3 = Q.dual_quaternion_mul(t_articulation, Q.dual_quaternion_inverse(rest_articulation))
        art = rest_articulation
    x = xyz.reshape(-1, 3)
    raw, gauss = skin_logits(P, x, art, t_embed, code, M, spf, prec, pre)
    out, ent, dsk = SkinBlend.apply(x, raw, art[0], art[1], gauss, se3[0], se3[1], spf)
    return out.view(shape), {"skin_entropy": ent.view(shape[:-1] + (1,)), "delta_skin": dsk.view(shape[:-1] + (1,))}


def skinning_warp_forward_multi(P, xyz, t_articulations, rest_articulation, t_embed_mean, code, prec=mlp.PREC_F32, pre=None):
    shape = xyz.shape
    M, spf = shape[0], _spf(shape)
    x = xyz.reshape(-1, 3)
    raw, gauss = skin_logits(P, x, rest_articulation, t_embed_mean, code, M, spf, prec, pre)
    rest_inv = None if pre is not None else Q.dual_quaternion_inverse(rest_articulation)
    se3s = [pre["se3s"][i] if pre is not None else Q.dual_quaternion_mul(t_art, rest_inv) for i, t_art in enumerate(t_articulations)]
    flat = SkinBlendMulti.apply(x, raw, rest_articulation[0], rest_articulation[1], gauss, spf, *[t for se3 in se3s for t in se3])
    outs = []
    for i in range(len(se3s)):
        out, ent, dsk = flat[3 * i:3 * i + 3]
        outs.append((out.view(shape), {"skin_entropy": ent.view(shape[:-1] + (1,)), "delta_skin": dsk.view(shape[:-1] + (1,))}))
    return outs


def dense_warp(P, xyz, t_embed, code, backward, prec=mlp.PREC_F32, prefix="warp.post_warp.", net=mlp.NET_DENSE):
    shape = xyz.shape
    spf = 1
    for d in shape[1:-1]:
        spf *= d
    which = "backward_map." if backward else "forward_map."
    cond = torch.cat([t_embed, code], -1)
    conds = {0: cond, 4: cond} if net == mlp.NET_DENSE6 else {0: cond}
    motion = mlp.run_chain(net, prec, P, xyz.reshape(-1, 3), spf, conds=conds, prefix=prefix + which)
    return xyz + 0.1 * motion.view(shape)


def composed_warp(P, xyz, t_articulation, rest_articulation, t_embed, code, backward, prec=mlp.PREC_F32, dense=None):
    if not backward and dense is not None:
        xyz = dense_warp(P, xyz, dense["t_embed"], dense["code_fw"], False, prec)
    out, aux = skinning_warp(P, xyz, t_articulation, rest_articulation, t_embed, code, backward, prec)
    if backward and dense is not None:
        out = dense_warp(P, out, dense["t_embed"], dense["code_bw"], True, prec)
    return out, aux
```

Measured before the change: 757,800.

## Fuse sigmoid and L2-normalize output heads into MLP forward/backward kernels

Adds a head activation option to the MLP forward and backward kernels, so the colour nets apply sigmoid and the feature net applies L2 normalisation in the kernel epilogue and prologue. This replaces the separate torch.sigmoid and L2Normalize pointwise launches and the extra memory round trips they cost. The backward pass now reads the stored forward output (and inv_norm for L2NORM), and any head disables the fused narrow backward path, which may push those nets onto a slower backward route.

```diff
diff --git a/include/lab4d_mlp.h b/include/lab4d_mlp.h
--- a/include/lab4d_mlp.h
+++ b/include/lab4d_mlp.h
@@ -23,6 +23,10 @@
 
 #define LAB4D_PREC_F32 0
 #define LAB4D_PREC_BF16 1
+
+#define LAB4D_HEAD_NONE 0
+#define LAB4D_HEAD_SIGMOID 1
+#define LAB4D_HEAD_L2NORM 2
 
 typedef struct {
   int ke;
@@ -75,6 +79,7 @@
   const float* aff;
 } lab4d_mlp_fwd_args;
 int lab4d_mlp_forward(const lab4d_mlp_fwd_args* a, void* stream);
+int lab4d_mlp_forward_head(const lab4d_mlp_fwd_args* a, int head_act, float* inv_norm, void* stream);
 
 typedef struct {
   int net, precision, S, spf;
@@ -115,6 +120,7 @@
   float* g_aff;
 } lab4d_mlp_bwd_args;
 int lab4d_mlp_backward(const lab4d_mlp_bwd_args* a, void* stream);
+int lab4d_mlp_backward_head(const lab4d_mlp_bwd_args* a, int head_act, const float* y, const float* inv_norm, void* stream);
 
 int lab4d_mlp_wgrad(int net, int layer, int precision, int S, int S_pad, int ld, int spf, const void* dz, const void* emb,
                     const void* act_prev, float* dW, float* db, float* pf_db, int M, void* stream);
diff --git a/lab4d_amd/csrc/hd_math.hpp b/lab4d_amd/csrc/hd_math.hpp
--- a/lab4d_amd/csrc/hd_math.hpp
+++ b/lab4d_amd/csrc/hd_math.hpp
@@ -34,3 +34,22 @@
 LAB4D_HD float nan_f() { return __builtin_nanf(""); }
 
 }
+
+namespace lab4d_head {
+
+LAB4D_HD float exp_t(float v) { return expf(v); }
+LAB4D_HD double exp_t(double v) { return exp(v); }
+LAB4D_HD float sqrt_t(float v) { return sqrtf(v); }
+LAB4D_HD double sqrt_t(double v) { return sqrt(v); }
+
+template <typename T>
+LAB4D_HD T sigmoid_fwd(T z) { return T(1) / (T(1) + exp_t(-z)); }
+template <typename T>
+LAB4D_HD T sigmoid_bwd(T g, T y) { return g * y * (T(1) - y); }
+
+template <typename T>
+LAB4D_HD T l2_inv_norm(T sumsq) { return T(1) / sqrt_t(sumsq); }
+template <typename T>
+LAB4D_HD T l2_bwd(T g, T y, T g_dot_y, T inv) { return (g - y * g_dot_y) * inv; }
+
+}
diff --git a/lab4d_amd/csrc/mlp.hip b/lab4d_amd/csrc/mlp.hip
--- a/lab4d_amd/csrc/mlp.hip
+++ b/lab4d_amd/csrc/mlp.hip
@@ -571,6 +571,10 @@
 }
 
 extern "C" int lab4d_mlp_forward(const lab4d_mlp_fwd_args* a, void* stream) {
+  return lab4d_mlp_forward_head(a, LAB4D_HEAD_NONE, nullptr, stream);
+}
+
+extern "C" int lab4d_mlp_forward_head(const lab4d_mlp_fwd_args* a, int head_act, float* inv_norm, void* stream) {
   LAB4D_REQUIRE(a, "mlp_forward: null args");
   LAB4D_REQUIRE(a->S >= 0 && a->S_pad >= a->S && a->S_pad % 256 == 0 && a->spf > 0 && a->ld >= a->S_pad && a->ld % 8 == 0,
                 "mlp_forward: bad sizes (S_pad must be a multiple of 256) S=%d S_pad=%d ld=%d spf=%d", a->S, a->S_pad, a->ld, a->spf);
@@ -581,7 +585,9 @@
     FwdK k;
     memset(&k, 0, sizeof(k));
     k.S = a->S; k.S_pad = a->S_pad; k.ld = a->ld; k.spf = a->spf; k.x = a->x; k.freq_w = a->freq_w; k.emb = a->emb; k.ext = a->ext; k.out = a->out; k.x2 = a->x2;
-    k.S_dev = a->S_dev; k.frame_idx = a->frame_idx; k.aff = a->aff;
+    k.S_dev = a->S_dev; k.frame_idx = a->frame_idx; k.aff = a->aff; k.head_act = head_act; k.inv_norm = inv_norm;
+    LAB4D_REQUIRE(head_act_ok<Net>(head_act), "mlp_forward: head_act %d is not built for net %d (SIGMOID: the colour nets, L2NORM: the feature net)", head_act, a->net);
+    LAB4D_REQUIRE(!inv_norm || head_act == LAB4D_HEAD_L2NORM, "mlp_forward: inv_norm is written by the L2NORM head only");
     LAB4D_REQUIRE(!a->aff || Net::EMB != 0, "mlp_forward: aff is for the raw-input nets only");
     LAB4D_REQUIRE(Net::EMB != 2 || a->aff, "mlp_forward: this network needs the per-frame affine table aff (M, ke, 4)");
     LAB4D_REQUIRE(!Net::AUX3 || a->x2, "mlp_forward: this network needs the second input x2");
@@ -601,6 +607,10 @@
 }
 
 extern "C" int lab4d_mlp_backward(const lab4d_mlp_bwd_args* a, void* stream) {
+  return lab4d_mlp_backward_head(a, LAB4D_HEAD_NONE, nullptr, nullptr, stream);
+}
+
+extern "C" int lab4d_mlp_backward_head(const lab4d_mlp_bwd_args* a, int head_act, const float* y, const float* inv_norm, void* stream) {
   LAB4D_REQUIRE(a, "mlp_backward: null args");
   LAB4D_REQUIRE(a->S >= 0 && a->S_pad >= a->S && a->S_pad % 256 == 0 && a->spf > 0 && a->ld >= a->S_pad && a->ld % 8 == 0, "mlp_backward: bad sizes (S_pad must be a multiple of 256)");
   LAB4D_REQUIRE(a->d_out, "mlp_backward: null d_out");
@@ -611,6 +621,10 @@
     memset(&k, 0, sizeof(k));
     k.S = a->S; k.S_pad = a->S_pad; k.ld = a->ld; k.spf = a->spf; k.emb = a->emb; k.ext = a->ext; k.d_out = a->d_out; k.ext_gin = a->ext_gin;
     k.ext_gout = a->ext_gout; k.d_x = a->d_x; k.d_x2 = a->d_x2; k.x = a->x; k.aff = a->aff; k.g_aff = a->g_aff;
+    k.head_act = head_act; k.y = y; k.inv_norm = inv_norm;
+    LAB4D_REQUIRE(head_act_ok<Net>(head_act), "mlp_backward: head_act %d is not built for net %d", head_act, a->net);
+    LAB4D_REQUIRE(head_act == LAB4D_HEAD_NONE || y, "mlp_backward: head_act %d needs y, the forward's output", head_act);
+    LAB4D_REQUIRE(head_act != LAB4D_HEAD_L2NORM || inv_norm, "mlp_backward: the L2NORM head needs the forward's inv_norm");
     if (Net::EMB == 2) {
       LAB4D_REQUIRE(a->x && a->aff && a->emb, "mlp_backward: this network needs x, aff and the stored embedding");
     } else {
diff --git a/lab4d_amd/csrc/mlp_kernels.hpp b/lab4d_amd/csrc/mlp_kernels.hpp
--- a/lab4d_amd/csrc/mlp_kernels.hpp
+++ b/lab4d_amd/csrc/mlp_kernels.hpp
@@ -345,6 +345,8 @@
   const int* S_dev;
   const int* frame_idx;
   const float* aff;
+  int head_act;
+  float* inv_norm;
 };
 struct BwdK {
   int S, S_pad, ld, spf, ntiles;
@@ -362,6 +364,9 @@
   const float* x;
   const float* aff;
   float* g_aff;
+  int head_act;
+  const float* y;
+  const float* inv_norm;
 };
 
 template <class Net>
@@ -447,6 +452,69 @@
 
 template <class Net>
 constexpr bool head_staged() { return Net::COUT > 16; }
+
+template <class Net>
+constexpr bool head_sigmoid_ok() { return Net::ID == LAB4D_NET_FG_COLOR || Net::ID == LAB4D_NET_BG_COLOR; }
+template <class Net>
+constexpr bool head_l2norm_ok() { return Net::ID == LAB4D_NET_FEAT; }
+__device__ __forceinline__ float sum_lane_halves(float v) {
+  const auto p = __builtin_amdgcn_permlane32_swap(__float_as_uint(v), __float_as_uint(v), false, false);
+  return __uint_as_float(p[0]) + __uint_as_float(p[1]);
+}
+template <class Net>
+constexpr bool head_act_ok(int act) {
+  return act == LAB4D_HEAD_NONE || (act == LAB4D_HEAD_SIGMOID && head_sigmoid_ok<Net>()) || (act == LAB4D_HEAD_L2NORM && head_l2norm_ok<Net>());
+}
+template <class Net>
+__device__ __forceinline__ float head_fwd_epilogue(int act, f32x16_t& acc) {
+  float inv = 0.f;
+  if constexpr (head_sigmoid_ok<Net>()) {
+    static_assert(Net::COUT <= 4, "colour rows are registers 0..3 of the lane half 0");
+    if (act == LAB4D_HEAD_SIGMOID) {
+#pragma unroll
+      for (int r = 0; r < Net::COUT; ++r) acc[r] = lab4d_head::sigmoid_fwd(acc[r]);
+    }
+  }
+  if constexpr (head_l2norm_ok<Net>()) {
+    static_assert(Net::COUT == 16, "16 channels: registers 0..7 of both lane halves");
+    if (act == LAB4D_HEAD_L2NORM) {
+      float q = 0.f;
+#pragma unroll
+      for (int r = 0; r < 8; ++r) q += acc[r] * acc[r];
+      q = sum_lane_halves(q);
+      inv = lab4d_head::l2_inv_norm(q);
+#pragma unroll
+      for (int r = 0; r < 8; ++r) acc[r] *= inv;
+    }
+  }
+  return inv;
+}
+template <class Net>
+__device__ __forceinline__ void head_bwd_prologue(const BwdK& a, int h, int s, f32x16_t& g) {
+  if constexpr (head_sigmoid_ok<Net>()) {
+    if (a.head_act == LAB4D_HEAD_SIGMOID) {
+#pragma unroll
+      for (int r = 0; r < Net::COUT; ++r) {
+        const float y = (h == 0 && s < a.S) ? ((const GLOBAL_AS float*)a.y)[(size_t)s * Net::COUT + r] : 0.f;
+        g[r] = lab4d_head::sigmoid_bwd(g[r], y);
+      }
+    }
+  }
+  if constexpr (head_l2norm_ok<Net>()) {
+    if (a.head_act == LAB4D_HEAD_L2NORM) {
+      float y[8], d = 0.f;
+#pragma unroll
+      for (int r = 0; r < 8; ++r) {
+        y[r] = s < a.S ? ((const GLOBAL_AS float*)a.y)[(size_t)s * Net::COUT + drow(r, h)] : 0.f;
+        d += g[r] * y[r];
+      }
+      d = sum_lane_halves(d);
+      const float inv = s < a.S ? ((const GLOBAL_AS float*)a.inv_norm)[s] : 0.f;
+#pragma unroll
+      for (int r = 0; r < 8; ++r) g[r] = lab4d_head::l2_bwd(g[r], y[r], d, inv);
+    }
+  }
+}
 
 template <class Net, class P>
 struct Slab {
@@ -881,6 +949,20 @@
           if (a.out) stage_out(stagef, a.out, (long)s0 * Net::COUT, TILE * Net::COUT, (long)S_eff * Net::COUT - 1, lane);
           __builtin_amdgcn_wave_barrier();
         } else {
+          if constexpr ((head_sigmoid_ok<Net>() || head_l2norm_ok<Net>()) && !TAN) {
+#pragma unroll
+            for (int t = 0; t < NT; ++t) {
+              const float inv = head_fwd_epilogue<Net>(a.head_act, acc[t]);
+              if constexpr (head_l2norm_ok<Net>()) {
+                if (a.inv_norm && h == 0 && sidx[t] < S_eff) a.inv_norm[sidx[t]] = inv;
+              }
+#pragma unroll
+              for (int r = 0; r < 16; ++r) {
+                const int f = 32 * mt + drow(r, h);
+                if (f < Net::COUT && sidx[t] < S_eff && a.out) a.out[(size_t)sidx[t] * Net::COUT + f] = acc[t][r];
+              }
+            }
+          } else {
 #pragma unroll
           for (int t = 0; t < NT; ++t)
 #pragma unroll
@@ -888,6 +970,7 @@
               const int f = 32 * mt + drow(r, h);
               if (f < Net::COUT && sidx[t] < S_eff && a.out) a.out[(size_t)sidx[t] * Net::COUT + f] = acc[t][r];
             }
+          }
         }
       };
       auto flush = [&](int mt, const unsigned int (&w)[2][8], unsigned int wbits) {
@@ -1058,6 +1141,8 @@
           const int f = drow(r, h);
           g[t][r] = (f < Net::COUT && sidx[t] < a.S) ? a.d_out[(size_t)sidx[t] * Net::COUT + f] : 0.f;
         }
+#pragma unroll
+      for (int t = 0; t < NT; ++t) head_bwd_prologue<Net>(a, h, sidx[t], g[t]);
       }
       if constexpr (DZ) store_tile<P>((GLOBAL_AS void*)a.dz[NL - 1], pad32(Net::L[NL - 1].mout), s0, 0, lane, g);
 #pragma unroll
diff --git a/lab4d_amd/csrc/mlp_kernels_ws.hpp b/lab4d_amd/csrc/mlp_kernels_ws.hpp
--- a/lab4d_amd/csrc/mlp_kernels_ws.hpp
+++ b/lab4d_amd/csrc/mlp_kernels_ws.hpp
@@ -572,6 +572,10 @@
               for (int q = 0; q < 2; ++q) xout[((2 * b + t) * 16 + 2 * mt + q) * 64 + lane_s] = u[q];
             }
           } else {
+            if constexpr (head_sigmoid_ok<Net>()) {
+#pragma unroll
+              for (int t = 0; t < 2; ++t) head_fwd_epilogue<Net>(a.head_act, acc[t]);
+            }
 #pragma unroll
             for (int t = 0; t < 2; ++t) {
               const int s = s0 + 64 * b + 2 * n + t;
@@ -687,7 +691,12 @@
 
   constexpr bool DPRE = Net::COUT <= 4;
   constexpr int DN = DPRE ? Net::COUT : 1;
-  auto d_fetch = [&](int tile_, float (&d)[2][DN]) {
+  constexpr bool HSIG = head_sigmoid_ok<Net>();
+  static_assert(!HSIG || DPRE, "the sigmoid head prologue rides on the prefetched head gradient");
+  static_assert(!head_l2norm_ok<Net>(), "no weights-stationary net has the L2NORM head");
+  constexpr int YN = HSIG ? DN : 1;
+  const bool hsig = HSIG && a.head_act == LAB4D_HEAD_SIGMOID;
+  auto d_fetch = [&](int tile_, float (&d)[2][DN], float (&y)[2][YN]) {
     if constexpr (DPRE) {
       if (w < 2 && tile_ < ntw) {
 #pragma unroll
@@ -697,20 +706,24 @@
           for (int r = 0; r < DN; ++r) {
             const int f = drow(r, h);
             d[t][r] = (f < Net::COUT && s < a.S) ? a.d_out[(size_t)s * Net::COUT + f] : 0.f;
+            if constexpr (HSIG) y[t][r] = (hsig && f < Net::COUT && s < a.S) ? a.y[(size_t)s * Net::COUT + f] : 0.f;
           }
         }
       }
     }
   };
-  float dcur[2][DN], dnext[2][DN];
-#pragma unroll
-  for (int t = 0; t < 2; ++t)
+  float dcur[2][DN], dnext[2][DN], ycur[2][YN], ynext[2][YN];
+#pragma unroll
+  for (int t = 0; t < 2; ++t) {
 #pragma unroll
     for (int r = 0; r < DN; ++r) dcur[t][r] = dnext[t][r] = 0.f;
-  d_fetch((int)blockIdx.x, dcur);
+#pragma unroll
+    for (int r = 0; r < YN; ++r) ycur[t][r] = ynext[t][r] = 0.f;
+  }
+  d_fetch((int)blockIdx.x, dcur, ycur);
   for (int tile = blockIdx.x; tile < ntw; tile += gridDim.x) {
     const int s0 = tile * WS_TILE;
-    d_fetch(tile + (int)gridDim.x, dnext);
+    d_fetch(tile + (int)gridDim.x, dnext, ynext);
     float dx[2][3];
 #pragma unroll
     for (int t = 0; t < 2; ++t) dx[t][0] = dx[t][1] = dx[t][2] = 0.f;
@@ -726,7 +739,8 @@
 #pragma unroll
         for (int r = 0; r < 16; ++r) {
           const int f = drow(r, h);
-          if constexpr (DPRE) g[t][r] = r < DN ? dcur[t][r < DN ? r : 0] : 0.f;
+          if constexpr (HSIG) g[t][r] = r < DN ? (hsig ? lab4d_head::sigmoid_bwd(dcur[t][r < DN ? r : 0], ycur[t][r < DN ? r : 0]) : dcur[t][r < DN ? r : 0]) : 0.f;
+          else if constexpr (DPRE) g[t][r] = r < DN ? dcur[t][r < DN ? r : 0] : 0.f;
           else g[t][r] = (f < Net::COUT && s < a.S) ? a.d_out[(size_t)s * Net::COUT + f] : 0.f;
         }
       }
@@ -954,7 +968,10 @@
 #pragma unroll
     for (int t = 0; t < 2; ++t)
 #pragma unroll
-      for (int r = 0; r < DN; ++r) dcur[t][r] = dnext[t][r];
+      for (int r = 0; r < DN; ++r) {
+        dcur[t][r] = dnext[t][r];
+        if constexpr (HSIG) ycur[t][r] = ynext[t][r];
+      }
     if (want_dx) {
       if (w < 2 * MTE_ANY) {
 #pragma unroll
diff --git a/lab4d_amd/csrc/pointwise.hip b/lab4d_amd/csrc/pointwise.hip
--- a/lab4d_amd/csrc/pointwise.hip
+++ b/lab4d_amd/csrc/pointwise.hip
@@ -9,7 +9,7 @@
     float q = 0.f;
 #pragma unroll
     for (int c = 0; c < C; ++c) { v[c] = x[s * C + c]; q += v[c] * v[c]; }
-    const float inv = 1.f / sqrtf(q);
+    const float inv = lab4d_head::l2_inv_norm(q);
 #pragma unroll
     for (int c = 0; c < C; ++c) y[s * C + c] = v[c] * inv;
   }
@@ -21,7 +21,7 @@
     float q = 0.f, d = 0.f;
 #pragma unroll
     for (int c = 0; c < C; ++c) { v[c] = x[s * C + c]; gv[c] = g[s * C + c]; q += v[c] * v[c]; d += v[c] * gv[c]; }
-    const float inv = 1.f / sqrtf(q);
+    const float inv = lab4d_head::l2_inv_norm(q);
     const float k = d * inv * inv;
 #pragma unroll
     for (int c = 0; c < C; ++c) gx[s * C + c] = (gv[c] - v[c] * k) * inv;
diff --git a/lab4d_amd/deformable.py b/lab4d_amd/deformable.py
--- a/lab4d_amd/deformable.py
+++ b/lab4d_amd/deformable.py
@@ -176,8 +176,9 @@
     if not with_color:
         return out
     rgb = mlp.run_chain(mlp.NET_FG_COLOR, prec, P, x, spf, conds={0: fr["code_color"], 3: fr["appr_code"]}, ext=feat,
-                        freq_w=posenc_window(alpha, 12, dev), pfs_pre=None if ft is None else {0: ft["pf.color0"], 3: ft["pf.color3"]})
-    return torch.sigmoid(rgb).view(shape[:-1] + (3,)), out
+                        freq_w=posenc_window(alpha, 12, dev), pfs_pre=None if ft is None else {0: ft["pf.color0"], 3: ft["pf.color3"]},
+                        head=mlp.HEAD_SIGMOID)
+    return rgb.view(shape[:-1] + (3,)), out
 
 
 def nerf_forward_bg(P, xyz, dir, codes, prec, get_density=True, alpha=None, prefix="", tap=None):
@@ -196,8 +197,8 @@
     if dir is None:
         return out
     rgb = mlp.run_chain(mlp.NET_BG_COLOR, prec, P, x, spf, conds={0: codes["colorfield"]}, ext=feat, freq_w=posenc_window(alpha, 8, dev),
-                        prefix=prefix, x2=dir.reshape(-1, 3))
-    return torch.sigmoid(rgb).view(shape[:-1] + (3,)), out
+                        prefix=prefix, x2=dir.reshape(-1, 3), head=mlp.HEAD_SIGMOID)
+    return rgb.view(shape[:-1] + (3,)), out
 
 
 def vis_field(P, xyz, fr, prec, ft=None):
@@ -229,8 +230,8 @@
 
 
 def compute_feat(P, xyz, prec):
-    f = mlp.run_chain(mlp.NET_FEAT, prec, P, xyz.reshape(-1, 3), _spf(xyz))
-    return L2Normalize.apply(f).view(xyz.shape[:-1] + (16,))
+    f = mlp.run_chain(mlp.NET_FEAT, prec, P, xyz.reshape(-1, 3), _spf(xyz), head=mlp.HEAD_L2NORM)
+    return f.view(xyz.shape[:-1] + (16,))
 
 
 class GlobalMatch(Function):
diff --git a/lab4d_amd/mlp.py b/lab4d_amd/mlp.py
--- a/lab4d_amd/mlp.py
+++ b/lab4d_amd/mlp.py
@@ -11,6 +11,7 @@
 
 MAXL = 12
 PREC_F32, PREC_BF16 = 0, 1
+HEAD_NONE, HEAD_SIGMOID, HEAD_L2NORM = 0, 1, 2
 vp, ci = ctypes.c_void_p, ctypes.c_int
 
 
@@ -429,7 +430,7 @@
     return out
 
 
-CHAIN_LEAD = ("net", "prec", "spf", "x", "ext", "freq_w", "export_layer", "n_pf", "x2", "tap")
+CHAIN_LEAD = ("net", "prec", "spf", "x", "ext", "freq_w", "export_layer", "n_pf", "x2", "tap", "head")
 
 
 class Wants:
@@ -456,6 +457,7 @@
                  "fused",
                  "x_shape", "has_x2",
                  "aff_in",
+                 "head",
                  "g_aff")
 
     def __init__(self, **kw):
@@ -464,7 +466,7 @@
         assert not kw, kw
 
 
-def chain_forward(net, prec, spf, x, pfs, params, want, ext=None, freq_w=None, export_layer=-1, x2=None, aff=None, tap=None):
+def chain_forward(net, prec, spf, x, pfs, params, want, ext=None, freq_w=None, export_layer=-1, x2=None, aff=None, tap=None, head=HEAD_NONE):
     d = describe(net)
     NL = d.n_layers
     pfs, params = list(pfs), list(params)
@@ -480,7 +482,7 @@
     dev = x.device
     sdt = store_dtype(prec)
     need_grad = want.any
-    fused = bool(need_grad and FUSED_NARROW_BWD and export_layer < 0 and ext is None and x2 is None and tap is None
+    fused = bool(need_grad and FUSED_NARROW_BWD and export_layer < 0 and ext is None and x2 is None and tap is None and head == HEAD_NONE
                  and _lib.lib().lab4d_mlp_fused_backward_supported(net, prec, spf))
     store = need_grad and not fused
     dx_only = bool(store and net in (NET_FG_BASE, NET_BG_BASE) and export_layer < 0 and ext is None and tap is None and not want.beyond_x)
@@ -523,15 +525,20 @@
         a.ext = _lib.dp(ext)
     out = torch.empty(S, d.c_out, device=dev)
     a.out = _lib.dp(out)
-    nbytes = sum(t.numel() * t.element_size() for t in acts + masks + [emb, ext, out, x] if t is not None)
+    inv_norm = torch.empty(S, device=dev) if (head == HEAD_L2NORM and need_grad) else None
+    nbytes = sum(t.numel() * t.element_size() for t in acts + masks + [emb, ext, out, x, inv_norm] if t is not None)
     with _lib.timed(chain_kernel_name("fwd", net, prec, dx_only) + ("" if store else " inference"), (2.0 * S * NET_MACS[net], float(nbytes))):
-        _lib.call("mlp_forward", ctypes.byref(a))
+        if head == HEAD_NONE:
+            _lib.call("mlp_forward", ctypes.byref(a))
+        else:
+            _lib.call("mlp_forward_head", ctypes.byref(a), head, inv_norm)
     if tap is not None and need_grad:
         tap.update(net=net, prec=prec, S=S, S_pad=S_pad, masks=list(masks), emb=emb)
     st = ChainState(net=net, prec=prec, spf=spf, S=S, S_pad=S_pad, want=want, params=params, pf_used=pf_used, acts=acts, masks=masks, emb=emb,
                     ext=ext, dx_only=dx_only, g_aff=None,
                     fused={"x": x, "freq_w": freq_w, "aff": aff, "W": pw_used, "bias": bias_used} if fused else None,
                     x_shape=x.shape if aff is None else (S, d.c_in),
+                    head=(head, out.view(-1), inv_norm) if (head != HEAD_NONE and need_grad) else None,
                     has_x2=x2 is not None,
                     aff_in=(x, aff) if (d.emb_kind == 2 and need_grad) else None)
     return out, (acts[export_layer].view(-1) if export_layer >= 0 else None), st
@@ -560,6 +567,7 @@
         a.ext_gout = _lib.dp(ext_g)
     d_out = d_out.contiguous().float()
     a.d_out = _lib.dp(d_out)
+    head, head_y, head_inv = st.head if st.head is not None else (HEAD_NONE, None, None)
     d_x = d_x2 = g_aff = None
     if st.aff_in is not None:
         xin, aff = st.aff_in
@@ -572,10 +580,14 @@
         if st.has_x2:
             d_x2 = torch.empty(st.x_shape, device=dev)
             a.d_x2 = _lib.dp(d_x2)
-    nbytes = sum(t.numel() * t.element_size() for t in list(dz) + list(st.masks) + [d_out, d_x, ext_g, st.emb if d_x is not None else None, d_export]
+    nbytes = sum(t.numel() * t.element_size() for t in list(dz) + list(st.masks) + [d_out, d_x, ext_g, st.emb if d_x is not None else None, d_export,
+                                                                                    head_y, head_inv]
                  if t is not None)
     with _lib.timed(chain_kernel_name("bwd", net, prec, st.dx_only), (2.0 * S * NET_MACS[net], float(nbytes))):
-        _lib.call("mlp_backward", ctypes.byref(a))
+        if head == HEAD_NONE:
+            _lib.call("mlp_backward", ctypes.byref(a))
+        else:
+            _lib.call("mlp_backward_head", ctypes.byref(a), head, head_y, head_inv)
     need_pf = iter(want.pfs)
     layers = [(dz[l], st.acts[l - 1] if d.layers[l].kin else None, want.params[2 * l], want.params[2 * l + 1],
                bool(d.layers[l].pf_bias) and bool(next(need_pf))) for l in range(NL)]
@@ -585,7 +597,7 @@
 
 
 def _release(st, g_aff):
-    st.acts = st.masks = st.emb = st.ext = st.params = st.aff_in = st.fused = None
+    st.acts = st.masks = st.emb = st.ext = st.params = st.aff_in = st.fused = st.head = None
     st.g_aff = g_aff
 
 
@@ -667,7 +679,8 @@
         want = Wants(need["x"], need["ext"], need["freq_w"], need["x2"], ctx.needs_input_grad[len(CHAIN_LEAD):][:n_pf],
                      ctx.needs_input_grad[len(CHAIN_LEAD):][n_pf:])
         out, exported, ctx.state = chain_forward(lead["net"], lead["prec"], lead["spf"], lead["x"], rest[:n_pf], rest[n_pf:], want, ext=lead["ext"],
-                                                 freq_w=lead["freq_w"], export_layer=lead["export_layer"], x2=lead["x2"], tap=lead["tap"])
+                                                 freq_w=lead["freq_w"], export_layer=lead["export_layer"], x2=lead["x2"], tap=lead["tap"],
+                                                 head=lead["head"])
         return out if exported is None else (out, exported)
 
     @staticmethod
@@ -683,14 +696,14 @@
     return [P[n] for bd in bindings(net, prefix) for n in (bd.wname, bd.bname)]
 
 
-def run_chain(net, prec, P, x, spf, conds=None, ext=None, freq_w=None, export_layer=None, prefix="", x2=None, pfs_pre=None, tap=None):
+def run_chain(net, prec, P, x, spf, conds=None, ext=None, freq_w=None, export_layer=None, prefix="", x2=None, pfs_pre=None, tap=None, head=HEAD_NONE):
     d = describe(net)
     bd = bindings(net, prefix)
     pfs = []
     for l in range(d.n_layers):
         if d.layers[l].pf_bias:
             pfs.append(pfs_pre[l] if pfs_pre is not None and l in pfs_pre else pf_bias_of(net, l, P[bd[l].wname], conds[l]))
-    return MlpChain.apply(net, prec, spf, x, ext, freq_w, -1 if export_layer is None else export_layer, len(pfs), x2, tap, *pfs,
+    return MlpChain.apply(net, prec, spf, x, ext, freq_w, -1 if export_layer is None else export_layer, len(pfs), x2, tap, head, *pfs,
                           *chain_params(net, P, prefix))
 
 
diff --git a/lab4d_amd/warping.py b/lab4d_amd/warping.py
--- a/lab4d_amd/warping.py
+++ b/lab4d_amd/warping.py
@@ -280,7 +280,7 @@
         params += [P[bd[l].wname], P[bd[l].bname]]
     if not FUSE_BONE_COORDS:
         bone = BoneCoords.apply(x, art[0], art[1], gauss, spf)
-        return mlp.MlpChain.apply(net, prec, spf, bone, None, None, -1, 1, None, None, pf, *params), gauss
+        return mlp.MlpChain.apply(net, prec, spf, bone, None, None, -1, 1, None, None, mlp.HEAD_NONE, pf, *params), gauss
     return SkinChain.apply(net, prec, spf, x, art[0], art[1], gauss, 1, pf, *params), gauss
 
 
```

Measured after the change: 758,000, median of 5. About the same (+0.0%).
